# yliess86/TorchBooster

Hardware: AMD Instinct MI355X
Metric: images/sec (whole node) ResNet-50 224px bf16 DDP (higher is better)
Workload: dtype bf16; 1 GPU; model=resnet50, image=224, per_gpu_batch=256, global_batch=256, parallelism=dp1, hip_graph=False, mode=native, pg_world_size=1, optimizer=AdamW lr1e-3 wd1e-2 + clip 1.0 + CycleScheduler, loss=cross_entropy label_smoothing=0.1

## Files before the change

### csrc/bind_conv.cpp

```cpp
#include "bind_common.h"

namespace {
using namespace tbbind;

const auto kNHWC = at::MemoryFormat::ChannelsLast;

Tensor f32_work(int64_t n, const Tensor& like) {
  return n > 0 ? at::empty({n}, like.options().dtype(at::kFloat)) : Tensor();
}

Tensor conv2d_stem_pad(const Tensor& x_) {
  const at::DeviceGuard guard = on_device_of(x_, "x");
  TORCH_CHECK(x_.scalar_type() == at::kBFloat16 && x_.dim() == 4 && x_.size(1) == 3, "conv2d_stem_pad: bf16 [N,3,H,W]");
  Tensor x = nhwc(x_);
  const int N = (int)x.size(0), H = (int)x.size(2), W = (int)x.size(3);
  int P, Q, Hp, Wp;
  tbamd::stem_geometry(H, W, &P, &Q, &Hp, &Wp);
  Tensor xp = at::empty({N, Hp, Wp, 4}, x.options());
  if (N > 0) tbamd::conv_stem_pad(x.data_ptr(), xp.data_ptr(), N, H, W, cur_stream());
  return xp;
}

std::vector<Tensor> conv2d_stem_fwd(const Tensor& xp, const Tensor& wp_, int64_t H, int64_t W, bool want_stats) {
  const at::DeviceGuard guard = on_device_of(xp, "xp");
// ... 67 lines not shown
  const at::DeviceGuard guard = on_device_of(dy_, "dy");
  TORCH_CHECK(dy_.scalar_type() == at::kBFloat16 && wt_.scalar_type() == at::kBFloat16, "conv2d_dgrad_s2: bf16 only");
  const int cs = (int)stride;
  Tensor dy = nhwc(dy_);
  Tensor wt = nhwc(wt_);
  const int N = (int)dy.size(0), Kf = (int)dy.size(1), P = (int)dy.size(2), Q = (int)dy.size(3);
  const int Cf = (int)wt.size(0);
  TORCH_CHECK(wt.dim() == 4 && wt.size(1) == Kf && wt.size(2) == R && wt.size(3) == S,
              "conv2d_dgrad_s2: wt must be the flip-transposed [Cf, Kf, R, S] weight");
  TORCH_CHECK(tbamd::conv_fwd_supported(Kf, Cf) && tbamd::conv_dgrad_s2_supported((int)R, (int)S, cs),
              "conv2d_dgrad_s2: channels % 64, stride 2 or 3, <= 16 taps per phase class");
  TORCH_CHECK(pad >= 0 && P == (H + 2 * pad - R) / cs + 1 && Q == (W + 2 * pad - S) / cs + 1,
              "conv2d_dgrad_s2: geometry");
  Tensor dx = at::empty({N, Cf, H, W}, dy.options().memory_format(kNHWC));
  const int64_t NHW = (int64_t)N * H * W;
  Tensor part;
  Bnb bnb;
  if (bnb_mode != 0) {
    TORCH_CHECK(bnb_mode >= 1 && bnb_mode <= 3, "conv2d_dgrad_s2: bnb_mode");
    bnb = bnb_operands(bnb_mode, bnb_x, bnb_scale, bnb_shift, bnb_mean, bnb_bits, NHW, Cf, "conv2d_dgrad_s2");
    part = at::empty({tbamd::conv_dgrad_s2_tiles(N, (int)H, (int)W, Cf, cs), 2, Cf}, dy.options().dtype(at::kFloat));
  }
  if (NHW > 0)
    tbamd::conv_dgrad_s2(dy.data_ptr(), wt.data_ptr(), dx.data_ptr(), N, P, Q, Kf, Cf, (int)R, (int)S, (int)pad,
                         (int)H, (int)W, cur_stream(), (int)bnb_mode, bnb.x, bnb.scale, bnb.shift, bnb.mean, bnb.bits,
                         f32_or_null(part), cs);
  return {dx, part};
}

std::vector<Tensor> conv2d_fwd(const Tensor& x_, const Tensor& w_, const optional<Tensor>& bias, int64_t stride,
                               int64_t pad, bool relu, bool want_stats, const optional<Tensor>& addend,
                               const optional<Tensor>& addend_mask, int64_t bnb_mode, const optional<Tensor>& bnb_x,
                               const optional<Tensor>& bnb_scale, const optional<Tensor>& bnb_shift,
                               const optional<Tensor>& bnb_mean, const optional<Tensor>& bnb_bits, int64_t big) {
  check_cuda(x_, "x");
  struct BigScope {
    explicit BigScope(int64_t c) { if (c >= 0) tbamd::conv_big_set_call((int)c); }
    ~BigScope() { tbamd::conv_big_set_call(-1); }
  } big_scope(big);
  const at::DeviceGuard guard(x_.device());
  TORCH_CHECK(x_.scalar_type() == at::kBFloat16 && w_.scalar_type() == at::kBFloat16, "conv2d_fwd: bf16 only");
  TORCH_CHECK(x_.dim() == 4 && w_.dim() == 4 && x_.size(1) == w_.size(1), "conv2d_fwd: shape");
  Tensor x = nhwc(x_);
  Tensor w = nhwc(w_);
  ConvGeom g = ConvGeom::of(x, w);
  TORCH_CHECK(tbamd::conv_fwd_supported(g.C, g.K), "conv2d_fwd: needs C % 64 == 0 and K % 64 == 0");
  const auto [N, C, H, W, K, R, S, P, Q] = g.window(stride, pad, 1, false, 0, "conv2d_fwd");
  Tensor y = at::empty({N, K, P, Q}, x.options().memory_format(kNHWC));
  Tensor bf = f32_or_undef(bias);
  Tensor stats;
  const int64_t NPQ = g.NPQ();
  if (want_stats)
    stats = at::empty({tbamd::conv_fwd_stats_rows(NPQ, C, K, R, S, (int)stride, (int)pad), 2, K},
                      x.options().dtype(at::kFloat));
  Tensor add;
  if (given(addend)) {
    TORCH_CHECK(!want_stats && !bf.defined() && !relu, "conv2d_fwd: addend excludes bias / relu / stats");
    TORCH_CHECK(addend->sizes() == y.sizes() && addend->scalar_type() == at::kBFloat16, "conv2d_fwd: addend shape");
    add = nhwc(*addend);
  }
  const uint8_t* amask = nullptr;
  if (given(addend_mask)) {
    TORCH_CHECK(add.defined() && addend_mask->scalar_type() == at::kByte && addend_mask->numel() == NPQ * (K / 8),
                "conv2d_fwd: addend_mask must be [N*P*Q, K/8] bytes");
    amask = addend_mask->data_ptr<uint8_t>();
  }
  Tensor part;
  Bnb bnb;
  if (bnb_mode != 0) {
    TORCH_CHECK(bnb_mode >= 1 && bnb_mode <= 3 && !want_stats && !bf.defined() && !relu, "conv2d_fwd: bnb_mode");
    bnb = bnb_operands(bnb_mode, bnb_x, bnb_scale, bnb_shift, bnb_mean, bnb_bits, NPQ, K, "conv2d_fwd");
    part = at::empty({tbamd::conv_fwd_bnb_rows(NPQ, C, K, R, S, (int)stride, (int)pad), 2, K},
                     x.options().dtype(at::kFloat));
  }
  if (NPQ > 0)
    tbamd::conv_fwd(x.data_ptr(), w.data_ptr(), y.data_ptr(), f32_or_null(bf),
                    want_stats ? stats.data_ptr<float>() : nullptr, ptr_or_null(add), amask, relu, N,
                    H, W, C, K, R, S, P, Q, (int)stride, (int)pad, cur_stream(), (int)bnb_mode, bnb.x, bnb.scale,
                    bnb.shift, bnb.mean, bnb.bits, f32_or_null(part));
  return {y, bnb_mode != 0 ? part : stats};
}

std::vector<Tensor> conv2d_dgrad_gxf(const Tensor& g_, const Tensor& wt_, const optional<Tensor>& addend,
                                     const optional<Tensor>& addend_mask, int64_t bnb_mode,
                                     const optional<Tensor>& bnb_x, const optional<Tensor>& bnb_scale,
                                     const optional<Tensor>& bnb_shift, const optional<Tensor>& bnb_mean,
                                     const optional<Tensor>& bnb_bits, int64_t gxf, const Tensor& gx_x_,
                                     const optional<Tensor>& gx_bits, const optional<Tensor>& gx_scale,
                                     const optional<Tensor>& gx_shift, const Tensor& gx_coef, bool want_dz) {
  const at::DeviceGuard guard = on_device_of(g_, "g");
  TORCH_CHECK(g_.scalar_type() == at::kBFloat16 && wt_.scalar_type() == at::kBFloat16 &&
                  gx_x_.scalar_type() == at::kBFloat16, "conv2d_dgrad_gxf: bf16 only");
  TORCH_CHECK(g_.dim() == 4 && wt_.dim() == 4 && wt_.size(1) == g_.size(1) && wt_.size(2) == 1 && wt_.size(3) == 1,
              "conv2d_dgrad_gxf: 1x1 weight [K, C, 1, 1] over g [N, C, H, W]");
  TORCH_CHECK(gx_x_.sizes() == g_.sizes(), "conv2d_dgrad_gxf: gx_x must have g's shape");
  Tensor g = nhwc(g_);
  Tensor wt = nhwc(wt_);
  Tensor gx_x = nhwc(gx_x_);
  const int N = (int)g.size(0), C = (int)g.size(1), H = (int)g.size(2), W = (int)g.size(3);
  const int K = (int)wt.size(0);
  const int64_t NPQ = (int64_t)N * H * W;
  TORCH_CHECK(tbamd::conv_fwd_supported(C, K), "conv2d_dgrad_gxf: needs C % 64 == 0 and K % 64 == 0");
  TORCH_CHECK(gx_coef.scalar_type() == at::kFloat && gx_coef.is_contiguous() && gx_coef.numel() == 3 * C,
              "conv2d_dgrad_gxf: gx_coef [3, C] f32");
  const uint8_t* gbits = nullptr;
  const float *gsc = nullptr, *gsf = nullptr;
  if (gxf == 2) {
    TORCH_CHECK(gx_bits.has_value() && gx_bits->scalar_type() == at::kByte && gx_bits->numel() == NPQ * (C / 8),
                "conv2d_dgrad_gxf: gx_bits [N*H*W, C/8] bytes");
    gbits = gx_bits->data_ptr<uint8_t>();
  } else {
    TORCH_CHECK(gxf == 1 && gx_scale.has_value() && gx_shift.has_value() && gx_scale->numel() == C &&
                    gx_shift->numel() == C && gx_scale->scalar_type() == at::kFloat &&
                    gx_shift->scalar_type() == at::kFloat && gx_scale->is_contiguous() && gx_shift->is_contiguous(),
                "conv2d_dgrad_gxf: gxf 1 needs f32 [C] scale / shift");
    gsc = gx_scale->data_ptr<float>();
    gsf = gx_shift->data_ptr<float>();
  }
  Tensor y = at::empty({N, K, H, W}, g.options().memory_format(kNHWC));
  Tensor add;
  const uint8_t* amask = nullptr;
  if (given(addend)) {
    TORCH_CHECK(addend->sizes() == y.sizes() && addend->scalar_type() == at::kBFloat16, "conv2d_dgrad_gxf: addend");
    add = nhwc(*addend);
    if (given(addend_mask)) {
      TORCH_CHECK(addend_mask->scalar_type() == at::kByte && addend_mask->numel() == NPQ * (K / 8),
                  "conv2d_dgrad_gxf: addend_mask [N*H*W, K/8] bytes");
      amask = addend_mask->data_ptr<uint8_t>();
    }
  }
  const int add_code = add.defined() ? (amask ? 2 : 1) : 0;
  TORCH_CHECK(tbamd::conv_dgrad_gxf_supported((int)gxf, add_code, (int)bnb_mode),
              "conv2d_dgrad_gxf: unsupported (gxf, addend, bnb_mode) combination");
  Tensor part;
  Bnb bnb;
  if (bnb_mode != 0) {
    bnb = bnb_operands(bnb_mode, bnb_x, bnb_scale, bnb_shift, bnb_mean, bnb_bits, NPQ, K, "conv2d_dgrad_gxf");
    part = at::empty({tbamd::conv_gxf_bnb_rows(NPQ, K), 2, K}, g.options().dtype(at::kFloat));
  }
  Tensor dz;
  if (want_dz) dz = at::empty_like(g);
  if (NPQ > 0)
    tbamd::conv_dgrad_gxf(g.data_ptr(), wt.data_ptr(), y.data_ptr(), ptr_or_null(add), amask,
                          N, H, W, C, K, cur_stream(), (int)bnb_mode, bnb.x, bnb.scale, bnb.shift, bnb.mean, bnb.bits,
                          f32_or_null(part), (int)gxf, gx_x.data_ptr(), gbits, gsc,
                          gsf, gx_coef.data_ptr<float>(), ptr_or_null(dz));
  return {y, part, dz};
}

bool conv_dgrad_gxf_supported(int64_t gxf, int64_t add, int64_t bnb_mode) {
  return tbamd::conv_dgrad_gxf_supported((int)gxf, (int)add, (int)bnb_mode);
}

void check_xf_coeffs(const Tensor& scale, const Tensor& shift, int C, const char* op) {
  TORCH_CHECK(scale.scalar_type() == at::kFloat && shift.scalar_type() == at::kFloat && scale.numel() == C &&
                  shift.numel() == C && scale.is_contiguous() && shift.is_contiguous(),
              op, ": scale / shift [C] f32");
}

std::vector<Tensor> conv2d_fwd_xf(const Tensor& x_, const Tensor& w_, const Tensor& scale, const Tensor& shift,
                                  int64_t stride, int64_t pad, bool want_stats) {
  const at::DeviceGuard guard = on_device_of(x_, "x");
  TORCH_CHECK(x_.scalar_type() == at::kBFloat16 && w_.scalar_type() == at::kBFloat16, "conv2d_fwd_xf: bf16 only");
  Tensor x = nhwc(x_);
  Tensor w = nhwc(w_);
  ConvGeom g = ConvGeom::of(x, w);
  TORCH_CHECK(w.size(1) == g.C && tbamd::conv_fwd_supported(g.C, g.K), "conv2d_fwd_xf: needs C % 64 == 0 and K % 64 == 0");
  TORCH_CHECK(g.C <= tbamd::kXfMaxC, "conv2d_fwd_xf: at most ", tbamd::kXfMaxC, " input channels (coefficients in LDS)");
  check_xf_coeffs(scale, shift, g.C, "conv2d_fwd_xf");
  const auto [N, C, H, W, K, R, S, P, Q] = g.window(stride, pad, 1, false, 0, "conv2d_fwd_xf");
  const int64_t NPQ = g.NPQ();
  TORCH_CHECK(tbamd::conv_fwd_xf_supported(NPQ, C, K, R, S, (int)stride, (int)pad),
              "conv2d_fwd_xf: the persistent 1x1 shapes only (C = 64 / 128, 1x1 stride 1, K % 128, enough pixels)");
  Tensor y = at::empty({N, K, P, Q}, x.options().memory_format(kNHWC));
  Tensor stats;
  if (want_stats)
    stats = at::empty({tbamd::conv_fwd_stats_rows_tiled(NPQ, C, K, R, S, (int)stride, (int)pad), 2, K},
                      x.options().dtype(at::kFloat));
  if (NPQ > 0)
    tbamd::conv_fwd_xf(x.data_ptr(), w.data_ptr(), y.data_ptr(), want_stats ? stats.data_ptr<float>() : nullptr,
                       scale.data_ptr<float>(), shift.data_ptr<float>(), N, H, W, C, K, R, S, P, Q, (int)stride,
                       (int)pad, cur_stream());
  return {y, stats};
}

Tensor conv_flip_weight(const Tensor& w_) {
  const at::DeviceGuard guard(w_.device());
  Tensor w = nhwc(w_);
  const int K = (int)w.size(0), C = (int)w.size(1), R = (int)w.size(2), S = (int)w.size(3);
  Tensor wt = at::empty({C, K, R, S}, w.options().memory_format(kNHWC));
  tbamd::conv_flip_transpose_weight(w.data_ptr(), K, R, S, C, wt.data_ptr(), cur_stream());
  return wt;
}

Tensor dw_slot_or_new(const optional<Tensor>& out, const ConvGeom& g, const Tensor& x, const char* op) {
  if (!given(out)) return at::empty({g.K, g.C, g.R, g.S}, x.options().memory_format(kNHWC));
  TORCH_CHECK(out->dim() == 4 && out->size(0) == g.K && out->size(1) == g.C && out->size(2) == g.R &&
                  out->size(3) == g.S && out->scalar_type() == at::kBFloat16 && out->is_contiguous(kNHWC),
              op, ": out must be a channels_last bf16 [K, C, R, S] tensor");
  return *out;
}

Tensor conv2d_wgrad(const Tensor& dy_, const Tensor& x_, int64_t R_, int64_t S_, int64_t stride, int64_t pad,
                    const optional<Tensor>& out) {
  const at::DeviceGuard guard = on_device_of(x_, "x");
  TORCH_CHECK(x_.scalar_type() == at::kBFloat16 && dy_.scalar_type() == at::kBFloat16, "conv2d_wgrad: bf16 only");
  Tensor x = nhwc(x_);
  Tensor dy = nhwc(dy_);
  ConvGeom g = ConvGeom::of(x, dy, R_, S_);
  const auto [N, C, H, W, K, R, S, P, Q] = g.window(stride, pad, 1, false, 0, "conv2d_wgrad");
  TORCH_CHECK(g.fits(dy), "conv2d_wgrad: dy shape does not match x / kernel / stride / pad");
  const int64_t NPQ = g.NPQ();
  TORCH_CHECK(tbamd::conv_wgrad_supported(C, K, NPQ), "conv2d_wgrad: needs C % 64 == 0 and K % 64 == 0");
  Tensor dw = dw_slot_or_new(out, g, x, "conv2d_wgrad");
  if (NPQ == 0) return dw.zero_();
  Tensor work = f32_work(tbamd::conv_wgrad_workspace(N, H, W, C, K, R, S, P, Q, (int)stride, (int)pad), x);
  tbamd::conv_wgrad(dy.data_ptr(), x.data_ptr(), dw.data_ptr(), f32_or_null(work), N, H, W, C, K, R, S, P, Q,
                    (int)stride, (int)pad, cur_stream());
  return dw;
}

Tensor conv2d_wgrad_xf(const Tensor& dy_, const Tensor& x_, const Tensor& scale, const Tensor& shift, int64_t R_,
                       int64_t S_, int64_t stride, int64_t pad, const optional<Tensor>& out) {
  const at::DeviceGuard guard = on_device_of(x_, "x");
  TORCH_CHECK(x_.scalar_type() == at::kBFloat16 && dy_.scalar_type() == at::kBFloat16, "conv2d_wgrad_xf: bf16 only");
  Tensor x = nhwc(x_);
  Tensor dy = nhwc(dy_);
  ConvGeom g = ConvGeom::of(x, dy, R_, S_);
  TORCH_CHECK(tbamd::conv_wgrad_supported(g.C, g.K, (int64_t)g.N * dy.size(2) * dy.size(3)), "conv2d_wgrad_xf: shape");
  check_xf_coeffs(scale, shift, g.C, "conv2d_wgrad_xf");
  const auto [N, C, H, W, K, R, S, P, Q] = g.window(stride, pad, 1, false, 0, "conv2d_wgrad_xf");
  TORCH_CHECK(dy.size(2) == P && dy.size(3) == Q, "conv2d_wgrad_xf: dy shape");
  Tensor dw = dw_slot_or_new(out, g, x, "conv2d_wgrad_xf");
  Tensor work = f32_work(tbamd::conv_wgrad_workspace(N, H, W, C, K, R, S, P, Q, (int)stride, (int)pad), x);
  tbamd::conv_wgrad_xf(dy.data_ptr(), x.data_ptr(), dw.data_ptr(), f32_or_null(work), scale.data_ptr<float>(),
                       shift.data_ptr<float>(), N, H, W, C, K, R, S, P, Q, (int)stride, (int)pad, cur_stream());
  return dw;
}

Tensor conv2d_wgrad_tinyin(const Tensor& T_, const Tensor& G_) {
  check_cuda(T_, "T");
  check_cuda(G_, "G");
  const at::DeviceGuard guard(T_.device());
  TORCH_CHECK(T_.scalar_type() == at::kBFloat16 && G_.scalar_type() == at::kBFloat16, "conv2d_wgrad_tinyin: bf16");
  TORCH_CHECK(T_.dim() == 4 && G_.dim() == 4 && T_.size(0) == G_.size(0), "conv2d_wgrad_tinyin: NCHW shapes");
  Tensor T = nhwc(T_), G = nhwc(G_);
  const int N = (int)T.size(0), C = (int)T.size(1), H = (int)T.size(2), W = (int)T.size(3);
  const int K = (int)G.size(1), P = (int)G.size(2), Q = (int)G.size(3);
  TORCH_CHECK(tbamd::wgrad_tinyin_supported(C, K, 4, 4, 2, 1, P, Q, H, W),
              "conv2d_wgrad_tinyin: needs C = 3, K = 64, Q = 64, H = 2P, W = 2Q");
  Tensor part = at::empty({(int64_t)tbamd::wgrad_tinyin_parts(N, P) * K * 48}, T.options().dtype(at::kFloat));
  Tensor dw = at::empty({K, C, 4, 4}, T.options().memory_format(kNHWC));
  tbamd::wgrad_tinyin(T.data_ptr(), G.data_ptr(), dw.data_ptr(), part.data_ptr<float>(), N, P, H, W, cur_stream());
  return dw;
}

Tensor conv2d_fwd_virtual(const Tensor& x_, const Tensor& w_, const optional<Tensor>& bias, int64_t stride,
                          int64_t pad, int64_t up, bool reflect) {
  const at::DeviceGuard guard = on_device_of(x_, "x");
  TORCH_CHECK(x_.scalar_type() == at::kBFloat16 && w_.scalar_type() == at::kBFloat16, "conv2d_fwd_virtual: bf16 only");
  TORCH_CHECK(x_.dim() == 4 && w_.dim() == 4 && x_.size(1) == w_.size(1), "conv2d_fwd_virtual: shape");
  TORCH_CHECK(tbamd::conv_fwd_supported((int)x_.size(1), (int)w_.size(0)),
              "conv2d_fwd_virtual: needs C % 64 == 0 and K % 64 == 0");
  TORCH_CHECK(up == 1 || up == 2 || up == 4, "conv2d_fwd_virtual: up must be 1, 2 or 4");
  Tensor x = nhwc(x_);
  Tensor w = nhwc(w_);
  const auto [N, C, H, W, K, R, S, P, Q] = ConvGeom::of(x, w).window(
      stride, pad, up, reflect, ConvGeom::kReflectFits | ConvGeom::kNonEmpty, "conv2d_fwd_virtual");
  Tensor y = at::empty({N, K, P, Q}, x.options().memory_format(kNHWC));
  Tensor bf = f32_or_undef(bias);
  tbamd::conv_fwd_virtual(x.data_ptr(), w.data_ptr(), y.data_ptr(), f32_or_null(bf), N,
                          H, W, C, K, R, S, P, Q, (int)stride, (int)pad, (int)up, reflect ? 1 : 0, cur_stream());
  return y;
}

Tensor conv2d_wgrad_virtual(const Tensor& dy_, const Tensor& x_, int64_t R_, int64_t S_, int64_t stride, int64_t pad,
                            int64_t up, bool reflect) {
  const at::DeviceGuard guard = on_device_of(x_, "x");
  Tensor x = nhwc(x_);
  Tensor dy = nhwc(dy_);
  ConvGeom g = ConvGeom::of(x, dy, R_, S_);
  TORCH_CHECK(dy.scalar_type() == at::kBFloat16 && x.scalar_type() == at::kBFloat16, "conv2d_wgrad_virtual: bf16");
  TORCH_CHECK(g.C % 64 == 0 && g.K % 32 == 0 && (up == 1 || up == 2 || up == 4), "conv2d_wgrad_virtual: channels / up");
  const auto [N, C, H, W, K, R, S, P, Q] = g.window(stride, pad, up, reflect, 0, "conv2d_wgrad_virtual");
  TORCH_CHECK(g.fits(dy), "conv2d_wgrad_virtual: dy shape");
  Tensor dw = at::empty({K, C, R, S}, x.options().memory_format(kNHWC));
  Tensor work = f32_work(tbamd::conv_wgrad_workspace(N, H, W, C, K, R, S, P, Q, (int)stride, (int)pad), x);
  tbamd::conv_wgrad_virtual(dy.data_ptr(), x.data_ptr(), dw.data_ptr(), f32_or_null(work), N, H, W, C, K, R, S, P, Q,
                            (int)stride, (int)pad, (int)up, reflect ? 1 : 0, cur_stream());
  return dw;
}

Tensor conv2d_dgrad_virtual(const Tensor& dy_, const Tensor& wt_, int64_t H, int64_t W, int64_t stride, int64_t pad,
                            int64_t up, bool reflect) {
  const at::DeviceGuard guard = on_device_of(dy_, "dy");
  Tensor dy = nhwc(dy_);
  Tensor wt = nhwc(wt_);
  TORCH_CHECK(dy.scalar_type() == at::kBFloat16 && wt.scalar_type() == at::kBFloat16, "conv2d_dgrad_virtual: bf16");
  const int N = (int)dy.size(0), K = (int)dy.size(1), P = (int)dy.size(2), Q = (int)dy.size(3);
  const int C = (int)wt.size(0), R = (int)wt.size(2), S = (int)wt.size(3);
  TORCH_CHECK(wt.size(1) == K && tbamd::conv_fwd_supported(K, C), "conv2d_dgrad_virtual: wt [C, K, R, S], % 64");
  TORCH_CHECK(stride == 1 || (stride == 2 && tbamd::conv_dgrad_s2_supported(R, S, 2)),
              "conv2d_dgrad_virtual: stride 1, or 2 with <= 16 taps per phase class");
  const int Hp = (int)(H * up + 2 * pad), Wp = (int)(W * up + 2 * pad);
  TORCH_CHECK(P == (Hp - R) / (int)stride + 1 && Q == (Wp - S) / (int)stride + 1, "conv2d_dgrad_virtual: geometry");
  Tensor dxp = at::empty({N, C, Hp, Wp}, dy.options().memory_format(kNHWC));
  if (stride == 1) {
    TORCH_CHECK(R == S, "conv2d_dgrad_virtual: square taps");
    tbamd::conv_fwd(dy.data_ptr(), wt.data_ptr(), dxp.data_ptr(), nullptr, nullptr, nullptr, nullptr, false, N, P, Q, K,
                    C, R, S, Hp, Wp, 1, R - 1, cur_stream());
  } else {
    tbamd::conv_dgrad_s2(dy.data_ptr(), wt.data_ptr(), dxp.data_ptr(), N, P, Q, K, C, R, S, 0, Hp, Wp, cur_stream());
  }
  const tbamd::ConvAnyShape fwd{N, (int)H, (int)W, C, K, R, S, P, Q, (int)stride, (int)pad, (int)up, 1, reflect ? 1 : 0};
  Tensor dx = at::empty({N, C, H, W}, dy.options().memory_format(kNHWC));
  tbamd::conv_any_fold(0, dxp.data_ptr(), Hp, Wp, dx.data_ptr(), fwd, cur_stream());
  return dx;
}

std::vector<Tensor> split_bf16(const Tensor& t_) {
  const at::DeviceGuard guard = on_device_of(t_, "t");
  TORCH_CHECK(t_.scalar_type() == at::kFloat, "split_bf16: fp32");
  const bool cl = t_.dim() == 4 && !t_.is_contiguous() && t_.is_contiguous(kNHWC);
  Tensor t = cl ? t_ : t_.contiguous();
  TORCH_CHECK(t.numel() % 4 == 0, "split_bf16: numel % 4");
  Tensor hi = at::empty_like(t, t.options().dtype(at::kBFloat16));
  Tensor lo = at::empty_like(t, t.options().dtype(at::kBFloat16));
  tbamd::split_bf16(t.data_ptr<float>(), t.numel(), (uint16_t*)hi.data_ptr(), (uint16_t*)lo.data_ptr(), cur_stream());
  return {hi, lo};
}

Tensor bias_k(const optional<Tensor>& bias, int K, const char* op) {
  Tensor b = f32_or_undef(bias);
  TORCH_CHECK(!b.defined() || b.numel() == K, op, ": bias");
  return b;
}

Tensor conv2d_fwd_split32(const Tensor& xh, const Tensor& xl, const Tensor& wh, const Tensor& wl,
                          const optional<Tensor>& bias, int64_t stride, int64_t pad, bool relu) {
  const at::DeviceGuard guard = on_device_of(xh, "xh");
  for (const Tensor* t : {&xh, &xl, &wh, &wl})
    TORCH_CHECK(t->scalar_type() == at::kBFloat16 && t->is_contiguous(kNHWC),
                "conv2d_fwd_split32: bf16 channels_last operands");
  ConvGeom g = ConvGeom::of(xh, wh);
  TORCH_CHECK(wh.size(1) == g.C && g.C % 64 == 0 && g.K % 64 == 0 && xl.sizes() == xh.sizes() &&
                  wl.sizes() == wh.sizes(),
              "conv2d_fwd_split32: shapes");
  const auto [N, C, H, W, K, R, S, P, Q] = g.window(stride, pad, 1, false, 0, "conv2d_fwd_split32");
  Tensor y = at::empty({N, K, P, Q}, xh.options().dtype(at::kFloat).memory_format(kNHWC));
  Tensor b = bias_k(bias, K, "conv2d_fwd_split32");
  const int ns = tbamd::conv_fwd_split32_ksplit(N, C, K, R, S, P, Q);
  Tensor part;
  if (ns > 1) part = at::empty({(int64_t)ns * N * P * Q * K}, y.options().memory_format(at::MemoryFormat::Contiguous));
  tbamd::conv_fwd_split32(xh.data_ptr(), xl.data_ptr(), wh.data_ptr(), wl.data_ptr(), y.data_ptr<float>(),
                          f32_or_null(b), relu, N, H, W, C, K, R, S, P, Q, (int)stride,
                          (int)pad, cur_stream(), ns > 1 ? part.data_ptr<float>() : nullptr);
  return y;
}

Tensor conv2d_fwd_splitk(const Tensor& x_, const Tensor& w_, const optional<Tensor>& bias, int64_t stride, int64_t pad,
                         bool relu) {
  const at::DeviceGuard guard = on_device_of(x_, "x");
  Tensor x = nhwc(x_), w = nhwc(w_);
  TORCH_CHECK(x.scalar_type() == at::kBFloat16 && w.scalar_type() == at::kBFloat16, "conv2d_fwd_splitk: bf16");
  ConvGeom g = ConvGeom::of(x, w);
  TORCH_CHECK(w.size(1) == g.C && g.C % 64 == 0 && g.K % 128 == 0 && stride >= 1 && pad >= 0,
              "conv2d_fwd_splitk: shapes");
  const auto [N, C, H, W, K, R, S, P, Q] = g.window(stride, pad, 1, false, ConvGeom::kNonEmpty, "conv2d_fwd_splitk");
  Tensor y = at::empty({N, K, P, Q}, x.options().memory_format(kNHWC));
  Tensor b = bias_k(bias, K, "conv2d_fwd_splitk");
  const int ns = std::max(1, tbamd::conv_fwd_splitk_bf16_ksplit(N, C, K, R, S, P, Q));
  Tensor part = at::empty({(int64_t)ns * N * P * Q * K}, x.options().dtype(at::kFloat));
  tbamd::conv_fwd_splitk_bf16(x.data_ptr(), w.data_ptr(), y.data_ptr(), f32_or_null(b),
                              relu, N, H, W, C, K, R, S, P, Q, (int)stride, (int)pad, part.data_ptr<float>(), ns,
                              cur_stream());
  return y;
}

Tensor conv2d_wgrad_split32(const Tensor& dy_, const Tensor& x_, int64_t R_, int64_t S_, int64_t stride, int64_t pad,
                            int64_t up, bool reflect) {
  const at::DeviceGuard guard = on_device_of(x_, "x");
  Tensor x = nhwc(x_);
  Tensor dy = nhwc(dy_);
  ConvGeom g = ConvGeom::of(x, dy, R_, S_);
  TORCH_CHECK(dy.scalar_type() == at::kFloat && x.scalar_type() == at::kFloat, "conv2d_wgrad_split32: fp32");
  TORCH_CHECK(g.C % 64 == 0 && g.K % 64 == 0 && (up == 1 || up == 2 || up == 4), "conv2d_wgrad_split32: channels / up");
  const auto [N, C, H, W, K, R, S, P, Q] = g.window(stride, pad, up, reflect, 0, "conv2d_wgrad_split32");
  TORCH_CHECK(g.fits(dy), "conv2d_wgrad_split32: dy shape");
  TORCH_CHECK(g.NPQ() < (1ll << 31), "conv2d_wgrad_split32: too many output pixels");
  Tensor dw = at::empty({K, C, R, S}, x.options().memory_format(kNHWC));
  auto bf = x.options().dtype(at::kBFloat16);
  Tensor dyh = at::empty({dy.numel()}, bf), dyl = at::empty({dy.numel()}, bf);
  Tensor xh = at::empty({x.numel()}, bf), xl = at::empty({x.numel()}, bf);
  Tensor work = at::empty({tbamd::conv_wgrad_split32_workspace(N, H, W, C, K, R, S, P, Q, (int)stride, (int)pad)},
                          x.options());
  tbamd::conv_wgrad_split32(dy.data_ptr<float>(), x.data_ptr<float>(), dw.data_ptr<float>(),
                            (uint16_t*)dyh.data_ptr(), (uint16_t*)dyl.data_ptr(), (uint16_t*)xh.data_ptr(),
                            (uint16_t*)xl.data_ptr(), work.data_ptr<float>(), N, H, W, C, K, R, S, P, Q,
                            (int)stride, (int)pad, (int)up, reflect ? 1 : 0, cur_stream());
  return dw;
}

Tensor im2col(const Tensor& x, int64_t R, int64_t S, int64_t P, int64_t Q, int64_t stride, int64_t pad, int64_t up,
              bool reflect) {
  TORCH_CHECK(x.is_cuda() && x.dtype() == at::kBFloat16 && x.dim() == 4 && x.is_contiguous(kNHWC),
              "im2col: expected bf16 channels_last [N, C, H, W]");
  TORCH_CHECK(up == 1 || up == 2 || up == 4, "im2col: upsample 1, 2 or 4");
  const int64_t N = x.size(0), C = x.size(1), H = x.size(2), W = x.size(3);
  const int64_t KP = (R * S * C + 7) / 8 * 8;
  Tensor col = at::empty({N * P * Q, KP}, x.options().memory_format(at::MemoryFormat::Contiguous));
  tbamd::im2col_nhwc(x.data_ptr(), col.data_ptr(), (int)N, (int)H, (int)W, (int)C, (int)R, (int)S, (int)P, (int)Q,
                     (int)stride, (int)pad, (int)up, reflect ? 1 : 0, (int)KP, cur_stream());
  return col;
}

Tensor col2im(const Tensor& col, int64_t N, int64_t C, int64_t H, int64_t W, int64_t R, int64_t S, int64_t P,
              int64_t Q, int64_t stride, int64_t pad, const optional<Tensor>& bias) {
  TORCH_CHECK(col.is_cuda() && col.dtype() == at::kBFloat16 && col.dim() == 2 && col.is_contiguous(),
              "col2im: expected contiguous bf16 [M, KP]");
  const int64_t KP = col.size(1);
  TORCH_CHECK(col.size(0) == N * P * Q && KP >= R * S * C, "col2im: col shape");
  Tensor b;
  if (given(bias)) {
    b = bias->to(at::kBFloat16).contiguous();
    TORCH_CHECK(b.numel() == C, "col2im: bias size");
  }
  Tensor dx = at::empty({N, C, H, W}, col.options().memory_format(kNHWC));
  tbamd::col2im_nhwc(col.data_ptr(), dx.data_ptr(), ptr_or_null(b), (int)N, (int)H, (int)W,
                     (int)C, (int)R, (int)S, (int)P, (int)Q, (int)stride, (int)pad, (int)KP, cur_stream());
  return dx;
}

}

void register_conv(pybind11::module& m) {
  m.def("conv2d_stem_pad", &conv2d_stem_pad);
  m.def("conv2d_stem_fwd", &conv2d_stem_fwd);
  m.def("conv2d_stem_wgrad", &conv2d_stem_wgrad);
  m.def("conv2d_dgrad_s2", &conv2d_dgrad_s2, py::arg("dy"), py::arg("wt"), py::arg("R"), py::arg("S"), py::arg("pad"),
        py::arg("H"), py::arg("W"), py::arg("bnb_mode") = 0, py::arg("bnb_x") = py::none(),
        py::arg("bnb_scale") = py::none(), py::arg("bnb_shift") = py::none(), py::arg("bnb_mean") = py::none(),
        py::arg("bnb_bits") = py::none(), py::arg("stride") = 2);
  m.def("conv_dgrad_s2_supported", &tbamd::conv_dgrad_s2_supported);
  m.def("conv2d_fwd", &conv2d_fwd, py::arg("x"), py::arg("w"), py::arg("bias"), py::arg("stride"), py::arg("pad"),
        py::arg("relu"), py::arg("want_stats"), py::arg("addend") = py::none(), py::arg("addend_mask") = py::none(),
        py::arg("bnb_mode") = 0, py::arg("bnb_x") = py::none(), py::arg("bnb_scale") = py::none(),
        py::arg("bnb_shift") = py::none(), py::arg("bnb_mean") = py::none(), py::arg("bnb_bits") = py::none(),
        py::arg("big") = -1);
  m.def("conv2d_dgrad_gxf", &conv2d_dgrad_gxf, py::arg("g"), py::arg("wt"), py::arg("addend"),
        py::arg("addend_mask"), py::arg("bnb_mode"), py::arg("bnb_x"), py::arg("bnb_scale"), py::arg("bnb_shift"),
        py::arg("bnb_mean"), py::arg("bnb_bits"), py::arg("gxf"), py::arg("gx_x"), py::arg("gx_bits"),
        py::arg("gx_scale"), py::arg("gx_shift"), py::arg("gx_coef"), py::arg("want_dz"));
  m.def("conv_dgrad_gxf_supported", &conv_dgrad_gxf_supported);
  m.def("conv_fwd_xf_supported", &tbamd::conv_fwd_xf_supported);
  m.def("conv2d_fwd_xf", &conv2d_fwd_xf, py::arg("x"), py::arg("w"), py::arg("scale"), py::arg("shift"),
        py::arg("stride"), py::arg("pad"), py::arg("want_stats") = true);
  m.def("conv_flip_weight", &conv_flip_weight);
  m.def("conv2d_wgrad", &conv2d_wgrad, py::arg("dy"), py::arg("x"), py::arg("R"), py::arg("S"), py::arg("stride"),
        py::arg("pad"), py::arg("out") = py::none());
  m.def("conv2d_wgrad_xf", &conv2d_wgrad_xf, py::arg("dy"), py::arg("x"), py::arg("scale"), py::arg("shift"),
        py::arg("R"), py::arg("S"), py::arg("stride"), py::arg("pad"), py::arg("out") = py::none());
  m.def("conv2d_wgrad_tinyin", &conv2d_wgrad_tinyin, py::arg("T"), py::arg("G"));
  m.def("conv2d_fwd_virtual", &conv2d_fwd_virtual, py::arg("x"), py::arg("w"), py::arg("bias"), py::arg("stride"),
        py::arg("pad"), py::arg("up") = 1, py::arg("reflect") = false);
  m.def("conv2d_wgrad_virtual", &conv2d_wgrad_virtual, py::arg("dy"), py::arg("x"), py::arg("R"), py::arg("S"),
        py::arg("stride"), py::arg("pad"), py::arg("up") = 1, py::arg("reflect") = false);
  m.def("conv2d_dgrad_virtual", &conv2d_dgrad_virtual, py::arg("dy"), py::arg("wt"), py::arg("H"), py::arg("W"),
        py::arg("stride"), py::arg("pad"), py::arg("up") = 1, py::arg("reflect") = false);
  m.def("split_bf16", &split_bf16);
  m.def("conv2d_fwd_split32", &conv2d_fwd_split32, py::arg("xh"), py::arg("xl"), py::arg("wh"), py::arg("wl"),
        py::arg("bias") = py::none(), py::arg("stride") = 1, py::arg("pad") = 0, py::arg("relu") = false);
  m.def("conv2d_fwd_splitk", &conv2d_fwd_splitk, py::arg("x"), py::arg("w"), py::arg("bias") = py::none(),
        py::arg("stride") = 1, py::arg("pad") = 0, py::arg("relu") = false);
  m.def("conv_fwd_splitk_ksplit", [](int64_t N, int64_t C, int64_t K, int64_t R, int64_t S, int64_t P, int64_t Q) {
    return tbamd::conv_fwd_splitk_bf16_ksplit((int)N, (int)C, (int)K, (int)R, (int)S, (int)P, (int)Q);
  });
  m.def("conv2d_wgrad_split32", &conv2d_wgrad_split32);
  m.def("im2col", &im2col);
  m.def("col2im", &col2im, py::arg("col"), py::arg("N"), py::arg("C"), py::arg("H"), py::arg("W"), py::arg("R"),
        py::arg("S"), py::arg("P"), py::arg("Q"), py::arg("stride"), py::arg("pad"), py::arg("bias") = py::none());
  m.def("conv_set_stages", &tbamd::conv_set_stages);
  m.def("conv_set_big", &tbamd::conv_set_big);
  m.def("conv_get_big", &tbamd::conv_get_big);
  m.def("conv_big_encode", &tbamd::conv_big_encode);
  m.def("conv_big_choice", &tbamd::conv_big_choice);
  m.def("conv_set_persistent_1x1", &tbamd::conv_set_persistent_1x1);
  m.def("conv_set_occupancy", &tbamd::conv_set_occupancy);
  m.def("conv_wgrad_set_occupancy", &tbamd::conv_wgrad_set_occupancy);
}
```

### csrc/conv.hip

```cpp
#include <cstdlib>
#include <mutex>
#include <stdexcept>
#include <type_traits>

#include "common.h"
#include "tbamd.h"
#include "xf.h"

namespace tbamd {

typedef __bf16 bf16x8_t __attribute__((ext_vector_type(8)));
typedef float f32x4_t __attribute__((ext_vector_type(4)));

struct ConvGeom {
  int N, H, W, C, K, R, S, P, Q, st, pad;
  int upsh, reflect, Hv, Wv;
};

constexpr int kConvBK = 64;
constexpr int kStemKT = 4;
constexpr int kConvThreads = 256;

__device__ __forceinline__ int swz(int row, int chunk) { return chunk ^ ((row >> 1) & 7); }

__device__ __attribute__((aligned(64))) uint4 g_conv_zero_page[16];

typedef __attribute__((address_space(3))) void lds_void_t;
typedef const __attribute__((address_space(1))) void gbl_void_t;

__device__ __forceinline__ void glds16(const void* src, void* lds_wave_base) {
  __builtin_amdgcn_global_load_lds((gbl_void_t*)src, (lds_void_t*)lds_wave_base, 16, 0, 0);
}

__device__ __forceinline__ uint32_t add_bf16x2(uint32_t a, uint32_t b) {
  const float lo = bf2f((uint16_t)(a & 0xffff)) + bf2f((uint16_t)(b & 0xffff));
  const float hi = bf2f((uint16_t)(a >> 16)) + bf2f((uint16_t)(b >> 16));
  return (uint32_t)f2bf(lo) | ((uint32_t)f2bf(hi) << 16);
}

struct BnBwdEpi {
  const uint16_t* xb;
  const float* scale;
  const float* shift;
  const float* mean;
  const uint8_t* bits;
  float* part;
};

struct GxfArgs {
  const uint16_t* xb;
  const uint8_t* bits;
  const float* scale;
  const float* shift;
  const float* coef;
  uint16_t* out;
};

struct S2Cls {
  int a, b, ntap, st;
  int dr[16], ds[16], wrs[16];
  int H, W;
  int tile_base;
};

constexpr int kS2MaxCls = 9;
struct S2Set {
  int ncls;
  int wg_start[kS2MaxCls + 1];
  ConvGeom g[kS2MaxCls];
  S2Cls c[kS2MaxCls];
};

__device__ __forceinline__ int p_virt_h(int v, const ConvGeom& g) {
  return g.reflect ? (v < 0 ? -v : (v >= g.Hv ? 2 * g.Hv - 2 - v : v)) : v;
}
__device__ __forceinline__ int p_virt_w(int v, const ConvGeom& g) {
  return g.reflect ? (v < 0 ? -v : (v >= g.Wv ? 2 * g.Wv - 2 - v : v)) : v;
}

template <int BM, int BN, bool STATS, bool BIAS, bool RELU, int STAGES, int ADD, int OCC = 2, int BNB = 0,
          bool STEM = false, bool S2D = false, bool VIRT = false, int PRIO = 3, int GXF = 0>
__global__ __launch_bounds__(kConvThreads, OCC) void conv_fwd_k(const uint16_t* __restrict__ x,
                                                              const uint16_t* __restrict__ w,
                                                              uint16_t* __restrict__ y,
                                                              const float* __restrict__ bias,
                                                              float* __restrict__ stats,
                                                              const uint16_t* __restrict__ addend,
                                                              const uint8_t* __restrict__ amask, ConvGeom g_in,
                                                              BnBwdEpi bnb = BnBwdEpi{},
                                                              std::conditional_t<S2D, S2Set, S2Cls> s2arg = {},
                                                              GxfArgs gxa = GxfArgs{}) {
  static_assert(!S2D || (ADD == 0 && !STATS && !STEM), "S2D: dgrad epilogue (optionally BN partials) only");
  static_assert(!VIRT || (!S2D && !STEM), "VIRT: plain forward addressing only");
  static_assert(GXF == 0 || (STAGES == 1 && !S2D && !STEM && !VIRT && !STATS),
                "GXF: single-stage 1x1 dgrad addressing only (host: R = S = 1, stride 1, pad 0)");
  constexpr int BK = kConvBK;
  constexpr int A_PASSES = BM / 32, B_PASSES = BN / 32;
  constexpr int WM = BM / 2, WN = BN / 2;
  constexpr int TM = WM / 16, TN = WN / 16;
  constexpr int STAGE = (BM + BN) * BK / 8;
  constexpr int OUT_U4 = BN * BM / 8 + (STATS ? BM : 0);
  constexpr int LDS_U4 = STAGES * STAGE > OUT_U4 ? STAGES * STAGE : OUT_U4;
  __shared__ __attribute__((aligned(16))) uint4 lds[LDS_U4];

  const int tid = threadIdx.x, lane = tid & 63, wave = tid >> 6;
  const int wm = wave >> 1, wn = wave & 1;
  ConvGeom g = g_in;
  int bid = blockIdx.x;
  int kcls = 0;
  if constexpr (S2D) {
    while (kcls + 1 < s2arg.ncls && bid >= s2arg.wg_start[kcls + 1]) ++kcls;
    bid -= s2arg.wg_start[kcls];
    g = s2arg.g[kcls];
  }
  const S2Cls& cls = [&]() -> const S2Cls& {
    if constexpr (S2D) return s2arg.c[kcls];
    else return s2arg;
  }();
  const int64_t NPQ = (int64_t)g.N * g.P * g.Q;
  const int ntm = g.K / BM;
  const int ntn = (int)((NPQ + BN - 1) / BN);
  {
    const int nwg = ntm * ntn;
    if constexpr (S2D) {
      if (bid >= nwg) return;
    }
    const int q8 = nwg / 8, r8 = nwg % 8, xcd = bid % 8;
    bid = (xcd < r8 ? xcd * (q8 + 1) : r8 * (q8 + 1) + (xcd - r8) * q8) + bid / 8;
  }
  const int tile_m = bid % ntm;
  const int tile_n = bid / ntm;
  const int m0 = tile_m * BM;
  const int64_t n0 = (int64_t)tile_n * BN;

  const int Kred = g.R * g.S * g.C;
  const int cblocks = g.C / BK;
  const int KT = STEM ? kStemKT : (S2D ? cls.ntap * cblocks : g.R * g.S * cblocks);
  const int lrow = wave * 8 + (lane >> 3);
  const int slot = lane & 7;

  int64_t pix_base[B_PASSES];
  int pix_h[B_PASSES], pix_w[B_PASSES], pix_n[B_PASSES];
#pragma unroll
  for (int i = 0; i < B_PASSES; ++i) {
    const int64_t pix = n0 + lrow + 32 * i;
    const bool ok = pix < NPQ;
    const int64_t pp = ok ? pix : 0;
    const int q = (int)(pp % g.Q);
    const int64_t t = pp / g.Q;
    const int p = (int)(t % g.P);
    const int n = (int)(t / g.P);
    pix_n[i] = ok ? n : -1;
    pix_h[i] = ok ? p * g.st - g.pad : -(1 << 20);
    pix_w[i] = q * g.st - g.pad;
    pix_base[i] = (((int64_t)n * g.H + pix_h[i]) * g.W + pix_w[i]) * g.C;
    if constexpr (STEM) pix_base[i] = ok ? (((int64_t)n * g.H + p * g.st) * g.W + q * g.st) * g.C : 0;
  }
  const uint16_t* wsrc0 = w + (int64_t)(m0 + lrow) * Kred + (slot ^ swz(lrow, 0)) * 8;
  const int64_t wpass = (int64_t)32 * Kred;

  const int cbl = STEM ? 1 : cblocks;
  const void* zpage = pin_sgpr(g_conv_zero_page);
  uint4 gx_v[GXF ? B_PASSES : 1];
  uint32_t gx_m[GXF == 2 ? B_PASSES : 1];
  extern __shared__ __attribute__((aligned(16))) float gx_lds[];
  auto issue = [&](int kt, int buf) {
    const int rs = kt / cbl, cb = kt - rs * cbl;
    int r = rs / g.S, s = rs - r * g.S;
    int wofs = kt * BK;
    if constexpr (S2D) {
      r = cls.dr[rs];
      s = cls.ds[rs];
      wofs = (cls.wrs[rs] * cbl + cb) * BK;
    }
    uint4* A = lds + buf * STAGE;
    uint4* B = A + BM * BK / 8;
#pragma unroll
    for (int i = 0; i < A_PASSES; ++i) {
      const uint16_t* wsrc = wsrc0 + i * wpass;
      const bool wok = TB_BOUNDS_OK(wsrc + wofs + 8 <= w + (int64_t)g.K * Kred, kBndConvW);
      glds16(wok ? (const void*)(wsrc + wofs) : zpage, A + (32 * i + wave * 8) * 8);
    }
    if constexpr (STEM) {
#pragma unroll
      for (int i = 0; i < B_PASSES; ++i) {
        const int row = lrow + 32 * i;
        const int lc = slot ^ swz(row, 0);
        const int64_t off = (int64_t)(2 * kt + (lc >> 2)) * g.W * g.C + (lc & 3) * 8;
        const void* src = pix_h[i] >= 0 ? (const void*)(x + pix_base[i] + off) : zpage;
        glds16(src, B + (32 * i + wave * 8) * 8);
      }
    } else if constexpr (VIRT) {
#pragma unroll
      for (int i = 0; i < B_PASSES; ++i) {
        const int row = lrow + 32 * i;
        int vh = p_virt_h(pix_h[i] + r, g), vw = p_virt_w(pix_w[i] + s, g);
        bool ok = pix_n[i] >= 0 && (unsigned)vh < (unsigned)g.Hv && (unsigned)vw < (unsigned)g.Wv;
        const int64_t off = (((int64_t)(ok ? pix_n[i] : 0) * g.H + (vh >> g.upsh)) * g.W + (vw >> g.upsh)) * g.C +
                            cb * BK + (slot ^ swz(row, 0)) * 8;
        ok = ok && TB_BOUNDS_OK(off >= 0 && off + 8 <= (int64_t)g.N * g.H * g.W * g.C, kBndConvSrc);
        glds16(ok ? (const void*)(x + off) : zpage, B + (32 * i + wave * 8) * 8);
      }
    } else {
    const int64_t tap = ((int64_t)r * g.W + s) * g.C + cb * BK;
#pragma unroll
    for (int i = 0; i < B_PASSES; ++i) {
      const int row = lrow + 32 * i;
      const int ih = pix_h[i] + r, iw = pix_w[i] + s;
      bool ok = (unsigned)ih < (unsigned)g.H && (unsigned)iw < (unsigned)g.W;
      const int64_t off = pix_base[i] + tap + (slot ^ swz(row, 0)) * 8;
      ok = ok && TB_BOUNDS_OK(off >= 0 && off + 8 <= (int64_t)g.N * g.H * g.W * g.C, kBndConvSrc);
      const void* src = ok ? (const void*)(x + off) : zpage;
      glds16(src, B + (32 * i + wave * 8) * 8);
      if constexpr (GXF != 0) {
        gx_v[i] = ok ? *reinterpret_cast<const uint4*>(gxa.xb + off) : make_uint4(0u, 0u, 0u, 0u);
        if constexpr (GXF == 2) gx_m[i] = ok ? (uint32_t)gxa.bits[off >> 3] : 0u;
      }
    }
    }
  };
  auto gxf_stage_coef = [&]() {
    if constexpr (GXF != 0) {
      const int C4 = g.C >> 2;
      float4* d = reinterpret_cast<float4*>(gx_lds);
      const float4* cf = reinterpret_cast<const float4*>(gxa.coef);
      for (int i = tid; i < 3 * C4; i += kConvThreads) d[i] = cf[i];
      if constexpr (GXF == 1) {
        const float4* sc = reinterpret_cast<const float4*>(gxa.scale);
        const float4* sf = reinterpret_cast<const float4*>(gxa.shift);
        for (int i = tid; i < C4; i += kConvThreads) {
          d[3 * C4 + i] = sc[i];
          d[4 * C4 + i] = sf[i];
        }
      }
    }
  };
  auto gxf_apply = [&](int kt) {
    if constexpr (GXF != 0) {
      uint4* B = lds + BM * BK / 8;
      const int c0 = kt * BK + (slot ^ swz(lrow, 0)) * 8;
      float ka[8], k0[8], k1[8], sc[8], sf[8];
      auto ld8 = [&](int row, float (&v)[8]) {
        const float4 a = *reinterpret_cast<const float4*>(gx_lds + row * g.C + c0);
        const float4 b = *reinterpret_cast<const float4*>(gx_lds + row * g.C + c0 + 4);
        v[0] = a.x; v[1] = a.y; v[2] = a.z; v[3] = a.w; v[4] = b.x; v[5] = b.y; v[6] = b.z; v[7] = b.w;
      };
      ld8(0, ka);
      ld8(1, k0);
      ld8(2, k1);
      if constexpr (GXF == 1) {
        ld8(3, sc);
        ld8(4, sf);
      }
      const bool wr = gxa.out != nullptr && tile_m == 0;
#pragma unroll
      for (int i = 0; i < B_PASSES; ++i) {
        if (pix_n[i] < 0) continue;
        uint4* p = B + (32 * i + lrow) * 8 + slot;
        const uint4 gv = *p, xv = gx_v[i];
        const uint32_t gw[4] = {gv.x, gv.y, gv.z, gv.w}, xw[4] = {xv.x, xv.y, xv.z, xv.w};
        uint32_t ow[4];
#pragma unroll
        for (int e = 0; e < 4; ++e) {
          float d[2];
#pragma unroll
          for (int h = 0; h < 2; ++h) {
            const int k = 2 * e + h;
            const float xf = bf2f((uint16_t)(xw[e] >> (16 * h)));
            const float gf = bf2f((uint16_t)(gw[e] >> (16 * h)));
            bool keep;
            if constexpr (GXF == 1) keep = __builtin_fmaf(xf, sc[k], sf[k]) > 0.f;
            else keep = (gx_m[i] >> k) & 1u;
            const float dz = keep ? gf : 0.f;
            d[h] = ka[k] * dz + k0[k] + k1[k] * xf;
          }
          ow[e] = (uint32_t)f2bf(d[0]) | ((uint32_t)f2bf(d[1]) << 16);
        }
        const uint4 o = make_uint4(ow[0], ow[1], ow[2], ow[3]);
        *p = o;
        if (wr) *reinterpret_cast<uint4*>(gxa.out + pix_base[i] + c0) = o;
      }
    }
  };
  f32x4_t acc[TM][TN];
#pragma unroll
  for (int i = 0; i < TM; ++i)
#pragma unroll
    for (int j = 0; j < TN; ++j) acc[i][j] = f32x4_t{0.f, 0.f, 0.f, 0.f};

  const int fr = lane & 15, fq = lane >> 4;
  auto compute = [&](int cur) {
    const uint4* A = lds + cur * STAGE;
    const uint4* B = A + BM * BK / 8;
#pragma unroll
    for (int ks = 0; ks < BK / 32; ++ks) {
      bf16x8_t af[TM], bfr[TN];
      const int ch = ks * 4 + fq;
#pragma unroll
      for (int i = 0; i < TM; ++i) {
        const int row = wm * WM + i * 16 + fr;
        af[i] = __builtin_bit_cast(bf16x8_t, A[row * 8 + swz(row, ch)]);
      }
#pragma unroll
      for (int j = 0; j < TN; ++j) {
        const int row = wn * WN + j * 16 + fr;
        bfr[j] = __builtin_bit_cast(bf16x8_t, B[row * 8 + swz(row, ch)]);
      }
#pragma unroll
      for (int i = 0; i < TM; ++i)
#pragma unroll
        for (int j = 0; j < TN; ++j)
          acc[i][j] = __builtin_amdgcn_mfma_f32_16x16x32_bf16(af[i], bfr[j], acc[i][j], 0, 0, 0);
    }
  };

  if constexpr (STAGES >= 2) {
    constexpr int LPT = A_PASSES + B_PASSES;
#pragma unroll
    for (int t = 0; t < STAGES - 1; ++t)
      if (t < KT) issue(t, t);
    int cur = 0, nxt = STAGES - 1;
    for (int kt = 0; kt < KT; ++kt) {
      if (kt + STAGES - 2 < KT) asm volatile("s_waitcnt vmcnt(%0)" ::"n"((STAGES - 2) * LPT) : "memory");
      else asm volatile("s_waitcnt vmcnt(0)" ::: "memory");
      __builtin_amdgcn_s_barrier();
      asm volatile("" ::: "memory");
      if (kt + STAGES - 1 < KT) issue(kt + STAGES - 1, nxt);
      compute(cur);
      cur = cur + 1 == STAGES ? 0 : cur + 1;
      nxt = nxt + 1 == STAGES ? 0 : nxt + 1;
    }
    __syncthreads();
  } else {
  issue(0, 0);
  if constexpr (GXF != 0) {
    gxf_stage_coef();
    asm volatile("s_waitcnt vmcnt(0)" ::: "memory");
    __syncthreads();
    gxf_apply(0);
  } else {
    asm volatile("s_waitcnt vmcnt(0)" ::: "memory");
  }
  __syncthreads();
  for (int kt = 0; kt < KT; ++kt) {
    const int cur = 0;
    const uint4* A = lds + cur * STAGE;
    const uint4* B = A + BM * BK / 8;
    if constexpr (PRIO > 0) __builtin_amdgcn_s_setprio(PRIO);
#pragma unroll
    for (int ks = 0; ks < BK / 32; ++ks) {
      bf16x8_t af[TM], bfr[TN];
      const int ch = ks * 4 + fq;
#pragma unroll
      for (int i = 0; i < TM; ++i) {
        const int row = wm * WM + i * 16 + fr;
        af[i] = __builtin_bit_cast(bf16x8_t, A[row * 8 + swz(row, ch)]);
      }
#pragma unroll
      for (int j = 0; j < TN; ++j) {
        const int row = wn * WN + j * 16 + fr;
        bfr[j] = __builtin_bit_cast(bf16x8_t, B[row * 8 + swz(row, ch)]);
      }
#pragma unroll
      for (int i = 0; i < TM; ++i)
#pragma unroll
        for (int j = 0; j < TN; ++j)
          acc[i][j] = __builtin_amdgcn_mfma_f32_16x16x32_bf16(af[i], bfr[j], acc[i][j], 0, 0, 0);
    }
    if constexpr (PRIO > 0) __builtin_amdgcn_s_setprio(0);
    if (kt + 1 < KT) {
      __syncthreads();
      issue(kt + 1, 0);
    }
    asm volatile("s_waitcnt vmcnt(0)" ::: "memory");
    if constexpr (GXF != 0) {
      if (kt + 1 < KT) gxf_apply(kt + 1);
    }
    __syncthreads();
  }
  }

  constexpr int CPR = BM / 8;
  uint16_t* ot = reinterpret_cast<uint16_t*>(lds);
  float ssum[TM][4], ssq[TM][4];
#pragma unroll
  for (int i = 0; i < TM; ++i)
#pragma unroll
    for (int e = 0; e < 4; ++e) ssum[i][e] = ssq[i][e] = 0.f;
#pragma unroll
  for (int i = 0; i < TM; ++i) {
    const int cl = wm * WM + i * 16 + fq * 4;
    float bv[4] = {0.f, 0.f, 0.f, 0.f};
    if constexpr (BIAS) {
#pragma unroll
      for (int e = 0; e < 4; ++e) bv[e] = bias[m0 + cl + e];
    }
#pragma unroll
    for (int j = 0; j < TN; ++j) {
      const int pl = wn * WN + j * 16 + fr;
      const bool pv = n0 + pl < NPQ;
      uint16_t hv[4];
#pragma unroll
      for (int e = 0; e < 4; ++e) {
        float v = acc[i][j][e] + bv[e];
        if constexpr (RELU) v = fmaxf(v, 0.f);
        hv[e] = f2bf(v);
        if constexpr (STATS) {
          if (pv) {
            const float vr = bf2f(hv[e]);
            ssum[i][e] += vr;
            ssq[i][e] += vr * vr;
          }
        }
      }
      const int chunk = (cl >> 3) ^ (pl & (CPR - 1));
      *reinterpret_cast<uint2*>(ot + pl * BM + chunk * 8 + (cl & 7)) =
          make_uint2((uint32_t)hv[0] | ((uint32_t)hv[1] << 16), (uint32_t)hv[2] | ((uint32_t)hv[3] << 16));
    }
  }
  __syncthreads();
  float bsc[8], bsf[8], bmu[8], bdb[8], bdg[8];
  if constexpr (BNB != 0) {
    const int c0 = m0 + (tid % CPR) * 8;
#pragma unroll
    for (int e = 0; e < 8; ++e) {
      bmu[e] = bnb.mean[c0 + e];
      if constexpr (BNB == 1) {
// ... 643 lines not shown
int conv_fwd_bnb_rows(int64_t NPQ, int C, int K, int R, int S, int stride, int pad) {
  if (const int big = conv_big_choice(NPQ, C, K, R, S, stride, pad)) {
    const int bn = conv_big_pixel_tile(big);
    return (int)((NPQ + bn - 1) / bn);
  }
  return conv_fwd_pixel_tiles(NPQ, K);
}

int conv_fwd_pixel_tiles(int64_t NPQ, int K) {
  const int BN = conv_big_pix(NPQ, K) ? 128 : 64;
  return (int)((NPQ + BN - 1) / BN);
}

static int g_conv_stages = [] {
  const char* e = getenv("TBAMD_CONV_STAGES");
  return e ? atoi(e) : 0;
}();
static int g_conv_occ = 0;
void conv_set_stages(int s) { g_conv_stages = s; }
void conv_set_occupancy(int o) { g_conv_occ = o; }

template <int BM, int BN, bool STATS, bool BIAS, bool RELU, int ADD = 0, int BNB = 0>
static void launch_conv(const uint16_t* x, const uint16_t* w, uint16_t* y, const float* bias, float* stats,
                        const uint16_t* addend, const uint8_t* amask, const ConvGeom& g, hipStream_t st,
                        const BnBwdEpi& bnb = BnBwdEpi{}) {
  const int64_t NPQ = (int64_t)g.N * g.P * g.Q;
  const int ntn = (int)((NPQ + BN - 1) / BN);
  const int ntm = g.K / BM;
  const dim3 grid(ntm * ntn);
  if constexpr (ADD != 0 || BNB != 0) {
    static const int epi_stages = [] {
      const char* e = getenv("TBAMD_CONV_EPI_STAGES");
      return e ? atoi(e) : 1;
    }();
    if (epi_stages == 2)
      conv_fwd_k<BM, BN, STATS, BIAS, RELU, 2, ADD, 2, BNB>
          <<<grid, kConvThreads, 0, st>>>(x, w, y, bias, stats, addend, amask, g, bnb, S2Cls{});
    else if (epi_stages == 3)
      conv_fwd_k<BM, BN, STATS, BIAS, RELU, 3, ADD, 2, BNB>
          <<<grid, kConvThreads, 0, st>>>(x, w, y, bias, stats, addend, amask, g, bnb, S2Cls{});
    else
      conv_fwd_k<BM, BN, STATS, BIAS, RELU, 1, ADD, 4, BNB>
          <<<grid, kConvThreads, 0, st>>>(x, w, y, bias, stats, addend, amask, g, bnb, S2Cls{});
  } else {
    int stages = g_conv_stages;
    if (stages == 0) stages = 1;
    switch (stages) {
      case 1:
        if (g_conv_occ == 2)
          conv_fwd_k<BM, BN, STATS, BIAS, RELU, 1, ADD, 2><<<grid, kConvThreads, 0, st>>>(x, w, y, bias, stats, addend, amask, g, bnb, S2Cls{});
        else if (g_conv_occ == 3)
          conv_fwd_k<BM, BN, STATS, BIAS, RELU, 1, ADD, 3><<<grid, kConvThreads, 0, st>>>(x, w, y, bias, stats, addend, amask, g, bnb, S2Cls{});
        else
          conv_fwd_k<BM, BN, STATS, BIAS, RELU, 1, ADD, 4><<<grid, kConvThreads, 0, st>>>(x, w, y, bias, stats, addend, amask, g, bnb, S2Cls{});
        break;
      case 3:
        conv_fwd_k<BM, BN, STATS, BIAS, RELU, 3, ADD><<<grid, kConvThreads, 0, st>>>(x, w, y, bias, stats, addend, amask, g, bnb, S2Cls{});
        break;
      case 4:
        conv_fwd_k<BM, BN, STATS, BIAS, RELU, 4, ADD><<<grid, kConvThreads, 0, st>>>(x, w, y, bias, stats, addend, amask, g, bnb, S2Cls{});
        break;
      default:
        conv_fwd_k<BM, BN, STATS, BIAS, RELU, 2, ADD><<<grid, kConvThreads, 0, st>>>(x, w, y, bias, stats, addend, amask, g, bnb, S2Cls{});
    }
  }
}

template <int BM, int BN, int ADD>
static void dispatch_bnb(const uint16_t* x, const uint16_t* w, uint16_t* y, const uint16_t* addend,
                         const uint8_t* amask, int bnb_mode, const BnBwdEpi& bnb, const ConvGeom& g,
                         hipStream_t st) {
  switch (bnb_mode) {
    case 1: launch_conv<BM, BN, false, false, false, ADD, 1>(x, w, y, nullptr, nullptr, addend, amask, g, st, bnb); break;
    case 2: launch_conv<BM, BN, false, false, false, ADD, 2>(x, w, y, nullptr, nullptr, addend, amask, g, st, bnb); break;
    default: launch_conv<BM, BN, false, false, false, ADD, 3>(x, w, y, nullptr, nullptr, addend, amask, g, st, bnb);
  }
}

template <int BM, int BN>
static void dispatch_epi(const uint16_t* x, const uint16_t* w, uint16_t* y, const float* bias, float* stats,
                         const uint16_t* addend, const uint8_t* amask, bool relu, const ConvGeom& g,
                         hipStream_t st, int bnb_mode = 0, const BnBwdEpi& bnb = BnBwdEpi{}) {
  if (bnb_mode != 0) {
    if (addend && amask) dispatch_bnb<BM, BN, 2>(x, w, y, addend, amask, bnb_mode, bnb, g, st);
    else if (addend) dispatch_bnb<BM, BN, 1>(x, w, y, addend, nullptr, bnb_mode, bnb, g, st);
    else dispatch_bnb<BM, BN, 0>(x, w, y, nullptr, nullptr, bnb_mode, bnb, g, st);
  } else if (addend) {
    if (amask) launch_conv<BM, BN, false, false, false, 2>(x, w, y, nullptr, nullptr, addend, amask, g, st);
    else launch_conv<BM, BN, false, false, false, 1>(x, w, y, nullptr, nullptr, addend, nullptr, g, st);
  } else if (stats) {
    if (bias) launch_conv<BM, BN, true, true, false>(x, w, y, bias, stats, nullptr, nullptr, g, st, bnb);
    else launch_conv<BM, BN, true, false, false>(x, w, y, bias, stats, nullptr, nullptr, g, st, bnb);
  } else if (bias) {
    if (relu) launch_conv<BM, BN, false, true, true>(x, w, y, bias, stats, nullptr, nullptr, g, st);
    else launch_conv<BM, BN, false, true, false>(x, w, y, bias, stats, nullptr, nullptr, g, st);
  } else {
    if (relu) launch_conv<BM, BN, false, false, true>(x, w, y, bias, stats, nullptr, nullptr, g, st);
    else launch_conv<BM, BN, false, false, false>(x, w, y, bias, stats, nullptr, nullptr, g, st);
  }
}

template <int BM, int BN, int ADD, int BNB, int GXF>
static void launch_gxf(const uint16_t* x, const uint16_t* w, uint16_t* y, const uint16_t* addend,
                       const uint8_t* amask, const ConvGeom& g, hipStream_t st, const BnBwdEpi& bnb,
                       const GxfArgs& gxa) {
  const int64_t NPQ = (int64_t)g.N * g.P * g.Q;
  const dim3 grid((g.K / BM) * (int)((NPQ + BN - 1) / BN));
  const size_t coef_bytes = (size_t)(GXF == 1 ? 5 : 3) * g.C * sizeof(float);
  conv_fwd_k<BM, BN, false, false, false, 1, ADD, 4, BNB, false, false, false, 3, GXF>
      <<<grid, kConvThreads, coef_bytes, st>>>(x, w, y, nullptr, nullptr, addend, amask, g, bnb, S2Cls{}, gxa);
}

template <int BM, int BN>
static bool dispatch_gxf(const uint16_t* x, const uint16_t* w, uint16_t* y, const uint16_t* addend,
                         const uint8_t* amask, const ConvGeom& g, hipStream_t st, int bnb_mode, const BnBwdEpi& bnb,
                         int gxf, const GxfArgs& gxa) {
  const int add = addend ? (amask ? 2 : 1) : 0;
  if (gxf == 2 && add == 0 && bnb_mode == 1) launch_gxf<BM, BN, 0, 1, 2>(x, w, y, addend, amask, g, st, bnb, gxa);
  else if (gxf == 1 && add == 2 && bnb_mode == 2) launch_gxf<BM, BN, 2, 2, 1>(x, w, y, addend, amask, g, st, bnb, gxa);
  else if (gxf == 1 && add == 1 && bnb_mode == 2) launch_gxf<BM, BN, 1, 2, 1>(x, w, y, addend, amask, g, st, bnb, gxa);
  else if (gxf == 1 && add == 1 && bnb_mode == 0) launch_gxf<BM, BN, 1, 0, 1>(x, w, y, addend, amask, g, st, bnb, gxa);
  else return false;
  return true;
}

bool conv_dgrad_gxf_supported(int gxf, int add, int bnb_mode) {
  return (gxf == 2 && add == 0 && bnb_mode == 1) || (gxf == 1 && add == 2 && bnb_mode == 2) ||
         (gxf == 1 && add == 1 && (bnb_mode == 2 || bnb_mode == 0));
}

int conv_gxf_bnb_rows(int64_t NPQ, int K) {
  (void)K;
  return (int)((NPQ + 63) / 64);
}

void conv_dgrad_gxf(const void* x, const void* w, void* y, const void* addend, const uint8_t* amask, int N, int H,
                    int W, int C, int K, hipStream_t st, int bnb_mode, const void* bnb_x, const float* bnb_scale,
                    const float* bnb_shift, const float* bnb_mean, const uint8_t* bnb_bits, float* bnb_part, int gxf,
                    const void* gx_x, const uint8_t* gx_bits, const float* gx_scale, const float* gx_shift,
                    const float* gx_coef, void* gx_out) {
  const BnBwdEpi bnb{(const uint16_t*)bnb_x, bnb_scale, bnb_shift, bnb_mean, bnb_bits, bnb_part};
  const GxfArgs gxa{(const uint16_t*)gx_x, gx_bits, gx_scale, gx_shift, gx_coef, (uint16_t*)gx_out};
  const ConvGeom g{N, H, W, C, K, 1, 1, H, W, 1, 0};
  const uint16_t* xx = (const uint16_t*)x;
  const uint16_t* ww = (const uint16_t*)w;
  uint16_t* yy = (uint16_t*)y;
  const uint16_t* aa = (const uint16_t*)addend;
  bool ok;
  if (K % 128 == 0) ok = dispatch_gxf<128, 64>(xx, ww, yy, aa, amask, g, st, bnb_mode, bnb, gxf, gxa);
  else ok = dispatch_gxf<64, 64>(xx, ww, yy, aa, amask, g, st, bnb_mode, bnb, gxf, gxa);
  if (!ok) throw std::runtime_error("conv_dgrad_gxf: unsupported (gxf, addend, bnb_mode) combination");
}

void conv_fwd(const void* x, const void* w, void* y, const float* bias, float* stats, const void* addend,
              const uint8_t* amask, bool relu, int N, int H, int W, int C, int K, int R, int S, int P, int Q,
              int stride, int pad, hipStream_t st, int bnb_mode, const void* bnb_x, const float* bnb_scale,
              const float* bnb_shift, const float* bnb_mean, const uint8_t* bnb_bits, float* bnb_part) {
  const BnBwdEpi bnb{(const uint16_t*)bnb_x, bnb_scale, bnb_shift, bnb_mean, bnb_bits, bnb_part};
  ConvGeom g{N, H, W, C, K, R, S, P, Q, stride, pad};
  const int64_t NPQ = (int64_t)N * P * Q;
  {
    const int big = bnb_mode != 0 || addend ? conv_big_choice(NPQ, C, K, R, S, stride, pad)
                                            : big_for(NPQ, C, K, R, S, stride, pad);
    if (big) {
      conv_big_fwd(x, w, y, bias, stats, addend, amask, relu, N, H, W, C, K, R, S, P, Q, stride, pad, st, bnb_mode,
                   bnb_x, bnb_scale, bnb_shift, bnb_mean, bnb_bits, bnb_part, big);
      return;
    }
  }

  const bool bigpix = conv_big_pix(NPQ, K);
  const uint16_t* xx = (const uint16_t*)x;
  const uint16_t* ww = (const uint16_t*)w;
  uint16_t* yy = (uint16_t*)y;
  const uint16_t* aa = (const uint16_t*)addend;
  if (!bias && !relu && !addend && bnb_mode == 0 && conv1x1p_eligible(C, K, R, S, stride, pad, NPQ)) {
    const int ns = conv1x1p_streams(NPQ, K, C);
    const dim3 grid((K / 128) * ns);
    if (C == 64) {
      if (stats) conv1x1_fwd_k<64, 128, true><<<grid, kConvThreads, 0, st>>>(xx, ww, yy, stats, NPQ, K, ns);
      else conv1x1_fwd_k<64, 128, false><<<grid, kConvThreads, 0, st>>>(xx, ww, yy, nullptr, NPQ, K, ns);
    } else {
      if (stats) conv1x1_fwd_k<128, 64, true><<<grid, kConvThreads, 0, st>>>(xx, ww, yy, stats, NPQ, K, ns);
      else conv1x1_fwd_k<128, 64, false><<<grid, kConvThreads, 0, st>>>(xx, ww, yy, nullptr, NPQ, K, ns);
    }
    return;
  }
  if (K % 128 == 0) {
    if (bigpix) dispatch_epi<128, 128>(xx, ww, yy, bias, stats, aa, amask, relu, g, st, bnb_mode, bnb);
    else dispatch_epi<128, 64>(xx, ww, yy, bias, stats, aa, amask, relu, g, st, bnb_mode, bnb);
  } else {
    if (bigpix) dispatch_epi<64, 128>(xx, ww, yy, bias, stats, aa, amask, relu, g, st, bnb_mode, bnb);
    else dispatch_epi<64, 64>(xx, ww, yy, bias, stats, aa, amask, relu, g, st, bnb_mode, bnb);
  }
}

bool conv_fwd_xf_supported(int64_t NPQ, int C, int K, int R, int S, int stride, int pad) {
  return conv1x1p_eligible(C, K, R, S, stride, pad, NPQ);
}

template <bool STATS>
static void launch_xf(const uint16_t* x, const uint16_t* w, uint16_t* y, float* stats, const ConvGeom& g,
                      const XfArgs& xf, hipStream_t st) {
  const int64_t NPQ = (int64_t)g.N * g.P * g.Q;
  if (conv1x1p_eligible(g.C, g.K, g.R, g.S, g.st, g.pad, NPQ)) {
    const int ns = conv1x1p_streams(NPQ, g.K, g.C);
    const dim3 grid((g.K / 128) * ns);
    if (g.C == 64)
      conv1x1_fwd_k<64, 128, STATS, true><<<grid, kConvThreads, 0, st>>>(x, w, y, stats, NPQ, g.K, ns, xf);
    else
      conv1x1_fwd_k<128, 64, STATS, true><<<grid, kConvThreads, 0, st>>>(x, w, y, stats, NPQ, g.K, ns, xf);
    return;
  }
  throw std::runtime_error("conv2d_fwd_xf: the BN-in-operand forward runs on the persistent 1x1 kernel only "
                           "(C = 64 / 128, 1x1 stride 1, enough pixels: conv_fwd_xf_supported)");
}

void conv_fwd_xf(const void* x, const void* w, void* y, float* stats, const float* scale, const float* shift, int N,
                 int H, int W, int C, int K, int R, int S, int P, int Q, int stride, int pad, hipStream_t st) {
  const ConvGeom g{N, H, W, C, K, R, S, P, Q, stride, pad};
  const XfArgs xf{scale, shift};
  if (stats) launch_xf<true>((const uint16_t*)x, (const uint16_t*)w, (uint16_t*)y, stats, g, xf, st);
  else launch_xf<false>((const uint16_t*)x, (const uint16_t*)w, (uint16_t*)y, nullptr, g, xf, st);
}

template <int BM, int BN>
static void launch_virt(const uint16_t* x, const uint16_t* w, uint16_t* y, const float* bias, const ConvGeom& g,
                        hipStream_t st) {
  const int64_t NPQ = (int64_t)g.N * g.P * g.Q;
  const dim3 grid((g.K / BM) * (int)((NPQ + BN - 1) / BN));
  if (bias)
    conv_fwd_k<BM, BN, false, true, false, 1, 0, 4, 0, false, false, true>
        <<<grid, kConvThreads, 0, st>>>(x, w, y, bias, nullptr, nullptr, nullptr, g);
  else
    conv_fwd_k<BM, BN, false, false, false, 1, 0, 4, 0, false, false, true>
        <<<grid, kConvThreads, 0, st>>>(x, w, y, nullptr, nullptr, nullptr, nullptr, g);
}

void conv_fwd_virtual(const void* x, const void* w, void* y, const float* bias, int N, int H, int W, int C, int K,
                      int R, int S, int P, int Q, int stride, int pad, int up, int reflect, hipStream_t st) {
  ConvGeom g{N, H, W, C, K, R, S, P, Q, stride, pad, up == 4 ? 2 : (up == 2 ? 1 : 0), reflect ? 1 : 0, H * up, W * up};
  const int64_t NPQ = (int64_t)N * P * Q;
  const bool bigpix = conv_big_pix(NPQ, K);
  const uint16_t* xx = (const uint16_t*)x;
  const uint16_t* ww = (const uint16_t*)w;
  uint16_t* yy = (uint16_t*)y;
  if (K % 128 == 0) {
    if (bigpix) launch_virt<128, 128>(xx, ww, yy, bias, g, st);
    else launch_virt<128, 64>(xx, ww, yy, bias, g, st);
  } else {
    if (bigpix) launch_virt<64, 128>(xx, ww, yy, bias, g, st);
    else launch_virt<64, 64>(xx, ww, yy, bias, g, st);
  }
}

__global__ __launch_bounds__(256) void stem_pad_k(const uint16_t* __restrict__ x, uint16_t* __restrict__ xp, int N,
                                                  int H, int W, int Hp, int Wp, int pad) {
  const int64_t total = (int64_t)N * Hp * Wp;
  for (int64_t i = (int64_t)blockIdx.x * 256 + threadIdx.x; i < total; i += (int64_t)gridDim.x * 256) {
    const int w = (int)(i % Wp);
    const int64_t t = i / Wp;
    const int h = (int)(t % Hp);
    const int n = (int)(t / Hp);
    const int ih = h - pad, iw = w - pad;
    uint32_t lo = 0, hi = 0;
    if ((unsigned)ih < (unsigned)H && (unsigned)iw < (unsigned)W) {
      const uint16_t* s = x + (((int64_t)n * H + ih) * W + iw) * 3;
      lo = (uint32_t)s[0] | ((uint32_t)s[1] << 16);
      hi = (uint32_t)s[2];
    }
    *reinterpret_cast<uint2*>(xp + i * 4) = make_uint2(lo, hi);
  }
}

static void stem_dims(int H, int W, int& P, int& Q, int& Hp, int& Wp) {
  P = (H - 1) / 2 + 1;
  Q = (W - 1) / 2 + 1;
  Hp = 2 * P + 6;
  Wp = 2 * Q + 6;
}

int64_t conv_stem_workspace(int N, int H, int W) {
  int P, Q, Hp, Wp;
  stem_dims(H, W, P, Q, Hp, Wp);
  return (int64_t)N * Hp * Wp * 4;
}

template <int BM, int BN, bool STATS>
static void launch_stem(const uint16_t* xp, const uint16_t* wp, uint16_t* y, float* stats, const ConvGeom& g,
                        hipStream_t st) {
  const int64_t NPQ = (int64_t)g.N * g.P * g.Q;
  const dim3 grid((g.K / BM) * (int)((NPQ + BN - 1) / BN));
  conv_fwd_k<BM, BN, STATS, false, false, 1, 0, 4, 0, true>
      <<<grid, kConvThreads, 0, st>>>(xp, wp, y, nullptr, stats, nullptr, nullptr, g);
}

void conv_stem_pad(const void* x, void* xp, int N, int H, int W, hipStream_t st) {
  int P, Q, Hp, Wp;
  stem_dims(H, W, P, Q, Hp, Wp);
  const int64_t tot = (int64_t)N * Hp * Wp;
  int64_t gs = (tot + 255) / 256;
  if (gs > 8192) gs = 8192;
  stem_pad_k<<<(int)gs, 256, 0, st>>>((const uint16_t*)x, (uint16_t*)xp, N, H, W, Hp, Wp, 3);
}

void stem_geometry(int H, int W, int* P, int* Q, int* Hp, int* Wp) { stem_dims(H, W, *P, *Q, *Hp, *Wp); }
// ... 174 lines not shown
```

### csrc/conv_wgrad.hip

```cpp
#include <algorithm>
#include <cstdlib>
#include <type_traits>

#include "common.h"
#include "tbamd.h"
#include "xf.h"

namespace tbamd {

namespace {

typedef __bf16 bf16x8_t __attribute__((ext_vector_type(8)));
typedef short s16x4_t __attribute__((ext_vector_type(4)));
typedef float f32x4_t __attribute__((ext_vector_type(4)));
typedef __attribute__((address_space(3))) void lds_void_t;
typedef const __attribute__((address_space(1))) void gbl_void_t;
typedef __attribute__((address_space(3))) s16x4_t lds_s16x4_t;

__device__ __attribute__((aligned(64))) uint4 g_wgrad_zero_page[16];

__device__ __forceinline__ void glds16(const void* src, void* lds_wave_base) {
  __builtin_amdgcn_global_load_lds((gbl_void_t*)src, (lds_void_t*)lds_wave_base, 16, 0, 0);
}

struct FastDiv {
  uint32_t mul;
  uint32_t shift;
  uint32_t d;
};

static FastDiv make_fastdiv(uint32_t d) {
  uint32_t l = 0;
  while ((1ull << l) < d) ++l;
  const uint64_t m = ((1ull << 32) * ((1ull << l) - d)) / d + 1;
  return FastDiv{(uint32_t)m, l, d};
}

__device__ __forceinline__ uint32_t fdiv(uint32_t n, const FastDiv& f) {
  return (__umulhi(n, f.mul) + n) >> f.shift;
}

struct WgradGeom {
  int N, H, W, C, K, R, S, P, Q, st, pad;
  int ncol;
  int npq;
  int pix_split;
  int splits;
  FastDiv fq, fp;
  int upsh, reflect, Hv, Wv;
};

template <int ROWB>
__device__ __forceinline__ int wz(int row) {
  if constexpr (ROWB == 256) return ((row & 3) | (((row >> 3) & 1) << 2)) << 1;
  else if constexpr (ROWB == 128) return ((((row >> 1) & 1) | (((row >> 3) & 1) << 1))) << 1;
  else return ((row >> 3) & 1) << 1;
}

template <int ROWB>
__device__ __forceinline__ bf16x8_t tr_frag(const char* base, int ks, int cb, int lane) {
  const int g = lane >> 4, q = (lane >> 2) & 3, p = lane & 3;
  const int lc = (cb >> 3) + (p >> 1);
  const int r0 = ks * 32 + 8 * g + q, r1 = r0 + 4;
  const int o0 = r0 * ROWB + ((lc ^ wz<ROWB>(r0)) << 4) + ((p & 1) << 3);
  const int o1 = r1 * ROWB + ((lc ^ wz<ROWB>(r1)) << 4) + ((p & 1) << 3);
  const s16x4_t v0 = __builtin_amdgcn_ds_read_tr16_b64_v4i16((lds_s16x4_t*)(base + o0));
  const s16x4_t v1 = __builtin_amdgcn_ds_read_tr16_b64_v4i16((lds_s16x4_t*)(base + o1));
  typedef short s16x8_t __attribute__((ext_vector_type(8)));
  const s16x8_t v = __builtin_shufflevector(v0, v1, 0, 1, 2, 3, 4, 5, 6, 7);
  return __builtin_bit_cast(bf16x8_t, v);
}

constexpr int kWgThreads = 256;
constexpr int kWgBK = 64;

template <int BM, int BN, bool FINAL, int OCC = 2, bool STEM = false, bool VIRT = false, bool XF = false>
__global__ __launch_bounds__(kWgThreads, OCC) void conv_wgrad_k(const uint16_t* __restrict__ dy,
                                                              const uint16_t* __restrict__ x,
                                                              float* __restrict__ part,
                                                              uint16_t* __restrict__ dw, WgradGeom g,
                                                              XfArgs xf = XfArgs{}) {
  static_assert(!XF || (!STEM && !VIRT), "XF: plain weight gradient");
  constexpr int BK = kWgBK;
  constexpr int ROWA = BM * 2, ROWB = BN * 2;
  constexpr int CPA = BM / 8, CPB = BN / 8;
  constexpr int A_PASSES = BK * CPA / kWgThreads, B_PASSES = BK * CPB / kWgThreads;
  constexpr int WM = BM / 2, WN = BN / 2, TM = WM / 16, TN = WN / 16;
  constexpr int STAGE = BK * (ROWA + ROWB);
  __shared__ __attribute__((aligned(16))) char lds[STAGE];

  const int tid = threadIdx.x, lane = tid & 63, wave = tid >> 6;
  const int wm = wave >> 1, wn = wave & 1;
  const int ntm = g.K / BM, ntn = g.ncol / BN, ntiles = ntm * ntn;
  const int nwg = ntiles * g.splits;
  int bid = blockIdx.x;
  {
    const int q8 = nwg / 8, r8 = nwg % 8, xcd = bid % 8;
    bid = (xcd < r8 ? xcd * (q8 + 1) : r8 * (q8 + 1) + (xcd - r8) * q8) + bid / 8;
  }
  const int split = bid / ntiles, tile = bid - split * ntiles;
  const int tile_m = tile % ntm, tile_n = tile / ntm;
  const int m0 = tile_m * BM, n0 = tile_n * BN;
  const int pb = split * g.pix_split;
  const int pe = min(pb + g.pix_split, g.npq);
  const int KT = (pe - pb + BK - 1) / BK;

  const uint16_t* asrc[A_PASSES];
  int arow[A_PASSES];
#pragma unroll
  for (int i = 0; i < A_PASSES; ++i) {
    const int row = i * (kWgThreads / CPA) + wave * (64 / CPA) + lane / CPA;
    const int lc = (lane % CPA) ^ wz<ROWA>(row);
    arow[i] = row;
    asrc[i] = dy + m0 + lc * 8;
  }
  int brow[B_PASSES], bdr[B_PASSES], bds[B_PASSES], bc[B_PASSES];
#pragma unroll
  for (int i = 0; i < B_PASSES; ++i) {
    const int row = i * (kWgThreads / CPB) + wave * (64 / CPB) + lane / CPB;
    const int lc = (lane % CPB) ^ wz<ROWB>(row);
    const int col = n0 + lc * 8;
    const int c = col % g.C, rs = col / g.C;
    brow[i] = row;
    bdr[i] = rs / g.S - g.pad;
    bds[i] = rs % g.S - g.pad;
    bc[i] = c;
    if constexpr (STEM) {
      bdr[i] = col >> 5;
      bds[i] = (col & 31) >> 2;
      bc[i] = 0;
    }
  }

  const void* zpage = pin_sgpr(g_wgrad_zero_page);
  uint32_t bvalid = 0u;
  float xsc[XF ? 8 : 1], xsh[XF ? 8 : 1];
  if constexpr (XF) {
    float sc8[8], sh8[8];
    xf_load(xf, bc[0], sc8, sh8);
#pragma unroll
    for (int e = 0; e < 8; ++e) {
      xsc[e] = sc8[e];
      xsh[e] = sh8[e];
    }
  }
  auto issue = [&](int kt, int buf) {
    char* A = lds + buf * STAGE;
    char* B = A + BK * ROWA;
    const int p0 = pb + kt * BK;
#pragma unroll
    for (int i = 0; i < A_PASSES; ++i) {
      const int pix = p0 + arow[i];
      const void* src = pix < pe ? (const void*)(asrc[i] + (int64_t)pix * g.K) : zpage;
      glds16(src, A + (i * kWgThreads + wave * 64) * 16);
    }
#pragma unroll
    for (int i = 0; i < B_PASSES; ++i) {
      const int pix = p0 + brow[i];
      const void* src = zpage;
      if (pix < pe) {
        const uint32_t t = fdiv((uint32_t)pix, g.fq);
        const int q = pix - (int)t * g.Q;
        const uint32_t n = fdiv(t, g.fp);
        const int p = (int)t - (int)n * g.P;
        const int h = p * g.st + bdr[i], w = q * g.st + bds[i];
        if constexpr (STEM) {
          src = x + (((int64_t)n * g.H + h) * g.W + w) * 4;
        } else if constexpr (VIRT) {
          const int vh = g.reflect ? (h < 0 ? -h : (h >= g.Hv ? 2 * g.Hv - 2 - h : h)) : h;
          const int vw = g.reflect ? (w < 0 ? -w : (w >= g.Wv ? 2 * g.Wv - 2 - w : w)) : w;
          if ((unsigned)vh < (unsigned)g.Hv && (unsigned)vw < (unsigned)g.Wv)
            src = x + (((int64_t)n * g.H + (vh >> g.upsh)) * g.W + (vw >> g.upsh)) * g.C + bc[i];
        } else if ((unsigned)h < (unsigned)g.H && (unsigned)w < (unsigned)g.W) {
          src = x + (((int64_t)n * g.H + h) * g.W + w) * g.C + bc[i];
        }
      }
      glds16(src, B + (i * kWgThreads + wave * 64) * 16);
      if constexpr (XF) {
        if (i == 0) bvalid = 0u;
        bvalid |= (uint32_t)(src != zpage) << i;
      }
    }
  };
  auto xform = [&](int buf) {
    if constexpr (XF) {
      char* B = lds + buf * STAGE + BK * ROWA;
      float sc8[8], sh8[8];
#pragma unroll
      for (int e = 0; e < 8; ++e) {
        sc8[e] = xsc[e];
        sh8[e] = xsh[e];
      }
#pragma unroll
      for (int i = 0; i < B_PASSES; ++i) {
        if (!((bvalid >> i) & 1u)) continue;
        uint4* p = reinterpret_cast<uint4*>(B + (i * kWgThreads + wave * 64) * 16) + lane;
        *p = xf_chunk(*p, sc8, sh8);
      }
    }
  };

  f32x4_t acc[TM][TN];
#pragma unroll
  for (int i = 0; i < TM; ++i)
#pragma unroll
    for (int j = 0; j < TN; ++j) acc[i][j] = f32x4_t{0.f, 0.f, 0.f, 0.f};

  for (int kt = 0; kt < KT; ++kt) {
    issue(kt, 0);
    asm volatile("s_waitcnt vmcnt(0)" ::: "memory");
    xform(0);
    __syncthreads();
#pragma unroll
    for (int ks = 0; ks < BK / 32; ++ks) {
      bf16x8_t af[TM], bfr[TN];
#pragma unroll
      for (int i = 0; i < TM; ++i) af[i] = tr_frag<ROWA>(lds, ks, wm * WM + i * 16, lane);
#pragma unroll
      for (int j = 0; j < TN; ++j) bfr[j] = tr_frag<ROWB>(lds + BK * ROWA, ks, wn * WN + j * 16, lane);
#pragma unroll
      for (int i = 0; i < TM; ++i)
#pragma unroll
        for (int j = 0; j < TN; ++j)
          acc[i][j] = __builtin_amdgcn_mfma_f32_16x16x32_bf16(af[i], bfr[j], acc[i][j], 0, 0, 0);
    }
    __syncthreads();
  }

  const int fr = lane & 15, fq = lane >> 4;
#pragma unroll
  for (int i = 0; i < TM; ++i)
#pragma unroll
    for (int e = 0; e < 4; ++e) {
      const int m = m0 + wm * WM + i * 16 + fq * 4 + e;
#pragma unroll
      for (int j = 0; j < TN; ++j) {
        const int n = n0 + wn * WN + j * 16 + fr;
        if constexpr (FINAL) dw[(int64_t)m * g.ncol + n] = f2bf(acc[i][j][e]);
        else part[((int64_t)split * g.K + m) * g.ncol + n] = acc[i][j][e];
      }
    }
}

constexpr int kRedCols = 16, kRedLanes = 16;
template <typename OutT>
__global__ __launch_bounds__(256) void wgrad_reduce_k(const float* __restrict__ part, int splits, int64_t total,
                                                      OutT* __restrict__ dw) {
  __shared__ float4 red[kRedLanes][kRedCols];
  const int tx = threadIdx.x % kRedCols, ty = threadIdx.x / kRedCols;
  const int64_t i4 = ((int64_t)blockIdx.x * kRedCols + tx) * 4;
  float4 s = make_float4(0.f, 0.f, 0.f, 0.f);
  if (i4 < total) {
    int k = ty;
#pragma unroll 1
    for (; k + 3 * kRedLanes < splits; k += 4 * kRedLanes) {
      float4 v[4];
#pragma unroll
      for (int u = 0; u < 4; ++u) v[u] = *reinterpret_cast<const float4*>(part + (int64_t)(k + u * kRedLanes) * total + i4);
#pragma unroll
      for (int u = 0; u < 4; ++u) {
        s.x += v[u].x;
        s.y += v[u].y;
        s.z += v[u].z;
        s.w += v[u].w;
      }
    }
    for (; k < splits; k += kRedLanes) {
      const float4 v = *reinterpret_cast<const float4*>(part + (int64_t)k * total + i4);
      s.x += v.x;
      s.y += v.y;
      s.z += v.z;
      s.w += v.w;
    }
  }
  red[ty][tx] = s;
  __syncthreads();
  if (ty == 0 && i4 < total) {
    for (int j = 1; j < kRedLanes; ++j) {
      const float4 v = red[j][tx];
      s.x += v.x;
      s.y += v.y;
      s.z += v.z;
      s.w += v.w;
    }
    if constexpr (sizeof(OutT) == 4) {
      *reinterpret_cast<float4*>(dw + i4) = s;
    } else {
      const uint32_t lo = (uint32_t)f2bf(s.x) | ((uint32_t)f2bf(s.y) << 16);
      const uint32_t hi = (uint32_t)f2bf(s.z) | ((uint32_t)f2bf(s.w) << 16);
      *reinterpret_cast<uint2*>(dw + i4) = make_uint2(lo, hi);
    }
  }
}

__global__ __launch_bounds__(256) void split_bf16_k(const float* __restrict__ v, int64_t n4, uint16_t* __restrict__ hi,
                                                    uint16_t* __restrict__ lo) {
  for (int64_t i = (int64_t)blockIdx.x * 256 + threadIdx.x; i < n4; i += (int64_t)gridDim.x * 256) {
    const float4 a = reinterpret_cast<const float4*>(v)[i];
    const float f[4] = {a.x, a.y, a.z, a.w};
    uint16_t h[4], l[4];
#pragma unroll
    for (int e = 0; e < 4; ++e) {
      h[e] = f2bf(f[e]);
      l[e] = f2bf(f[e] - bf2f(h[e]));
    }
    reinterpret_cast<uint2*>(hi)[i] = make_uint2((uint32_t)h[0] | ((uint32_t)h[1] << 16), (uint32_t)h[2] | ((uint32_t)h[3] << 16));
    reinterpret_cast<uint2*>(lo)[i] = make_uint2((uint32_t)l[0] | ((uint32_t)l[1] << 16), (uint32_t)l[2] | ((uint32_t)l[3] << 16));
  }
}

int g_wgrad_occ = 0;

template <int BM, int BN, int OCC>
void launch_wgrad_s(const uint16_t* dy, const uint16_t* x, float* part, uint16_t* dw, const WgradGeom& g,
                    hipStream_t st) {
  const int nwg = (g.K / BM) * (g.ncol / BN) * g.splits;
  if (g.splits == 1)
    conv_wgrad_k<BM, BN, true, OCC><<<nwg, kWgThreads, 0, st>>>(dy, x, part, dw, g);
  else
    conv_wgrad_k<BM, BN, false, OCC><<<nwg, kWgThreads, 0, st>>>(dy, x, part, dw, g);
}

template <int BM, int BN>
void launch_wgrad(const uint16_t* dy, const uint16_t* x, float* part, uint16_t* dw, const WgradGeom& g,
                  hipStream_t st) {
  switch (g_wgrad_occ) {
    case 3: launch_wgrad_s<BM, BN, 3>(dy, x, part, dw, g, st); break;
    case 4: launch_wgrad_s<BM, BN, 4>(dy, x, part, dw, g, st); break;
    default: launch_wgrad_s<BM, BN, 2>(dy, x, part, dw, g, st);
  }
}

WgradGeom plan_wgrad(int N, int H, int W, int C, int K, int R, int S, int P, int Q, int stride, int pad) {
  WgradGeom g{};
  g.N = N, g.H = H, g.W = W, g.C = C, g.K = K, g.R = R, g.S = S, g.P = P, g.Q = Q, g.st = stride, g.pad = pad;
  g.ncol = R * S * C;
  g.npq = N * P * Q;
  const int BM = K % 128 == 0 ? 128 : (K % 64 == 0 ? 64 : 32);
  const int BN = g.ncol % 128 == 0 ? 128 : 64;
  const int64_t tiles = (int64_t)(K / BM) * (g.ncol / BN);
  const int bk = kWgBK;
  const int64_t kiters = (g.npq + bk - 1) / bk;
  static const double waves = [] {
    const char* e = getenv("TBAMD_WGRAD_WAVES");
    const double v = e ? atof(e) : 1.0;
    return v > 0.0 && v <= 8.0 ? v : 1.0;
  }();
  const int64_t target = (int64_t)(((BM == 128 && BN == 128) ? 768 : 1024) * waves);
  int64_t splits = (target + tiles - 1) / tiles;
  splits = std::min<int64_t>(splits, std::max<int64_t>(g.npq / 1024, 1));
  static const int64_t cap_mb = [] {
    const char* e = getenv("TBAMD_WGRAD_CAP_MB");
    const int64_t v = e ? atoll(e) : 32;
    return v >= 1 && v <= 1024 ? v : 32;
  }();
  const int64_t cap = (cap_mb << 20) / ((int64_t)K * g.ncol * 4);
  splits = std::max<int64_t>(1, std::min(splits, std::max<int64_t>(cap, 1)));
  const int64_t per = ((kiters + splits - 1) / splits) * bk;
  g.pix_split = (int)per;
  g.splits = (int)((g.npq + per - 1) / per);
  g.fq = make_fastdiv((uint32_t)Q);
  g.fp = make_fastdiv((uint32_t)P);
  return g;
}

}

int64_t conv_stem_wgrad_workspace(int N, int Hp, int Wp, int K, int P, int Q) {
  const WgradGeom g = plan_wgrad(N, Hp, Wp, 4, K, 8, 8, P, Q, 2, 0);
  return g.splits > 1 ? (int64_t)g.splits * K * g.ncol : 0;
}

void conv_stem_wgrad(const void* dy, const void* xp, void* dwp, float* workspace, int N, int Hp, int Wp, int K,
                     int P, int Q, hipStream_t st) {
  const WgradGeom g = plan_wgrad(N, Hp, Wp, 4, K, 8, 8, P, Q, 2, 0);
  const uint16_t* d = (const uint16_t*)dy;
  const uint16_t* xx = (const uint16_t*)xp;
  uint16_t* o = (uint16_t*)dwp;
  const int nwg = (K / (K % 128 == 0 ? 128 : 64)) * (g.ncol / 128) * g.splits;
  if (K % 128 == 0) {
    if (g.splits == 1) conv_wgrad_k<128, 128, true, 3, true><<<nwg, kWgThreads, 0, st>>>(d, xx, workspace, o, g);
    else conv_wgrad_k<128, 128, false, 3, true><<<nwg, kWgThreads, 0, st>>>(d, xx, workspace, o, g);
  } else {
    if (g.splits == 1) conv_wgrad_k<64, 128, true, 3, true><<<nwg, kWgThreads, 0, st>>>(d, xx, workspace, o, g);
    else conv_wgrad_k<64, 128, false, 3, true><<<nwg, kWgThreads, 0, st>>>(d, xx, workspace, o, g);
  }
  if (g.splits > 1) {
    const int64_t total = (int64_t)K * g.ncol;
    wgrad_reduce_k<uint16_t><<<cdiv(total, 4 * kRedCols), kRedCols * kRedLanes, 0, st>>>(workspace, g.splits, total, o);
  }
}

void conv_wgrad_virtual(const void* dy, const void* x, void* dw, float* workspace, int N, int H, int W, int C, int K,
                        int R, int S, int P, int Q, int stride, int pad, int up, int reflect, hipStream_t st) {
  WgradGeom g = plan_wgrad(N, H, W, C, K, R, S, P, Q, stride, pad);
  g.upsh = up == 4 ? 2 : (up == 2 ? 1 : 0);
  g.reflect = reflect ? 1 : 0;
  g.Hv = H * up;
  g.Wv = W * up;
  const uint16_t* d = (const uint16_t*)dy;
  const uint16_t* xx = (const uint16_t*)x;
  uint16_t* o = (uint16_t*)dw;
  auto go = [&](auto bm, auto bn) {
    constexpr int BM = decltype(bm)::value, BN = decltype(bn)::value;
    const int nwg = (g.K / BM) * (g.ncol / BN) * g.splits;
    if (g.splits == 1)
      conv_wgrad_k<BM, BN, true, 3, false, true><<<nwg, kWgThreads, 0, st>>>(d, xx, workspace, o, g);
    else
      conv_wgrad_k<BM, BN, false, 3, false, true><<<nwg, kWgThreads, 0, st>>>(d, xx, workspace, o, g);
  };
  using std::integral_constant;
  const bool bm128 = K % 128 == 0, bn128 = g.ncol % 128 == 0;
  if (K % 64 != 0) go(integral_constant<int, 32>{}, integral_constant<int, 64>{});
  else if (bm128 && bn128) go(integral_constant<int, 128>{}, integral_constant<int, 128>{});
  else if (bm128) go(integral_constant<int, 128>{}, integral_constant<int, 64>{});
  else if (bn128) go(integral_constant<int, 64>{}, integral_constant<int, 128>{});
  else go(integral_constant<int, 64>{}, integral_constant<int, 64>{});
  if (g.splits > 1) {
    const int64_t total = (int64_t)K * g.ncol;
    wgrad_reduce_k<uint16_t><<<cdiv(total, 4 * kRedCols), kRedCols * kRedLanes, 0, st>>>(workspace, g.splits, total, o);
  }
}

void conv_wgrad_xf(const void* dy, const void* x, void* dw, float* workspace, const float* scale, const float* shift,
                   int N, int H, int W, int C, int K, int R, int S, int P, int Q, int stride, int pad,
                   hipStream_t st) {
  const WgradGeom g = plan_wgrad(N, H, W, C, K, R, S, P, Q, stride, pad);
  const XfArgs xf{scale, shift};
  const uint16_t* d = (const uint16_t*)dy;
  const uint16_t* xx = (const uint16_t*)x;
  uint16_t* o = (uint16_t*)dw;
  auto go = [&](auto bm, auto bn) {
    constexpr int BM = decltype(bm)::value, BN = decltype(bn)::value;
    const int nwg = (g.K / BM) * (g.ncol / BN) * g.splits;
    if (g_wgrad_occ == 3) {
      if (g.splits == 1)
        conv_wgrad_k<BM, BN, true, 3, false, false, true><<<nwg, kWgThreads, 0, st>>>(d, xx, workspace, o, g, xf);
      else
        conv_wgrad_k<BM, BN, false, 3, false, false, true><<<nwg, kWgThreads, 0, st>>>(d, xx, workspace, o, g, xf);
    } else if (g.splits == 1) {
      conv_wgrad_k<BM, BN, true, 2, false, false, true><<<nwg, kWgThreads, 0, st>>>(d, xx, workspace, o, g, xf);
    } else {
      conv_wgrad_k<BM, BN, false, 2, false, false, true><<<nwg, kWgThreads, 0, st>>>(d, xx, workspace, o, g, xf);
    }
  };
  using std::integral_constant;
  const bool bm128 = K % 128 == 0, bn128 = g.ncol % 128 == 0;
  if (bm128 && bn128) go(integral_constant<int, 128>{}, integral_constant<int, 128>{});
  else if (bm128) go(integral_constant<int, 128>{}, integral_constant<int, 64>{});
  else if (bn128) go(integral_constant<int, 64>{}, integral_constant<int, 128>{});
  else go(integral_constant<int, 64>{}, integral_constant<int, 64>{});
  if (g.splits > 1) {
    const int64_t total = (int64_t)K * g.ncol;
    wgrad_reduce_k<uint16_t><<<cdiv(total, 4 * kRedCols), kRedCols * kRedLanes, 0, st>>>(workspace, g.splits, total, o);
  }
}

void conv_wgrad_set_occupancy(int o) { g_wgrad_occ = o; }

int64_t conv_wgrad_split32_workspace(int N, int H, int W, int C, int K, int R, int S, int P, int Q, int stride,
                                     int pad) {
  const WgradGeom g = plan_wgrad(N, H, W, C, K, R, S, P, Q, stride, pad);
  return 3ll * g.splits * K * g.ncol;
}

void conv_wgrad_split32(const float* dy, const float* x, float* dw, uint16_t* dyh, uint16_t* dyl, uint16_t* xh,
                        uint16_t* xl, float* part, int N, int H, int W, int C, int K, int R, int S, int P, int Q,
                        int stride, int pad, int up, int reflect, hipStream_t st) {
  const int64_t ndy = (int64_t)N * P * Q * K, nx = (int64_t)N * H * W * C;
  auto grid4 = [](int64_t n4) { return (int)std::min<int64_t>((n4 + 255) / 256, 8192); };
  split_bf16_k<<<grid4(ndy / 4), 256, 0, st>>>(dy, ndy / 4, dyh, dyl);
  split_bf16_k<<<grid4(nx / 4), 256, 0, st>>>(x, nx / 4, xh, xl);
  WgradGeom g = plan_wgrad(N, H, W, C, K, R, S, P, Q, stride, pad);
  const bool virt = up != 1 || reflect;
  g.upsh = up == 4 ? 2 : (up == 2 ? 1 : 0);
  g.reflect = reflect ? 1 : 0;
  g.Hv = H * up;
  g.Wv = W * up;
  const int64_t slab = (int64_t)g.splits * K * g.ncol;
  const uint16_t* A[3] = {dyh, dyh, dyl};
  const uint16_t* B[3] = {xh, xl, xh};
  auto go = [&](auto bm, auto bn) {
    constexpr int BM = decltype(bm)::value, BN = decltype(bn)::value;
    const int nwg = (g.K / BM) * (g.ncol / BN) * g.splits;
    for (int t = 0; t < 3; ++t) {
      if (virt)
        conv_wgrad_k<BM, BN, false, 3, false, true><<<nwg, kWgThreads, 0, st>>>(A[t], B[t], part + t * slab, nullptr, g);
      else
        conv_wgrad_k<BM, BN, false, 3><<<nwg, kWgThreads, 0, st>>>(A[t], B[t], part + t * slab, nullptr, g);
    }
  };
  using std::integral_constant;
  const bool bm128 = K % 128 == 0, bn128 = g.ncol % 128 == 0;
  if (bm128 && bn128) go(integral_constant<int, 128>{}, integral_constant<int, 128>{});
  else if (bm128) go(integral_constant<int, 128>{}, integral_constant<int, 64>{});
  else if (bn128) go(integral_constant<int, 64>{}, integral_constant<int, 128>{});
  else go(integral_constant<int, 64>{}, integral_constant<int, 64>{});
  const int64_t total = (int64_t)K * g.ncol;
  wgrad_reduce_k<float><<<cdiv(total, 4 * kRedCols), kRedCols * kRedLanes, 0, st>>>(part, 3 * g.splits, total, dw);
}

void split_bf16(const float* v, int64_t n, uint16_t* hi, uint16_t* lo, hipStream_t st) {
  const int64_t n4 = n / 4;
  if (n4 == 0) return;
  split_bf16_k<<<(int)std::min<int64_t>((n4 + 255) / 256, 8192), 256, 0, st>>>(v, n4, hi, lo);
}

int conv_wgrad_supported(int C, int K, int64_t NPQ) {
  return C % 64 == 0 && K % 64 == 0 && NPQ < (1ll << 31);
}

int64_t conv_wgrad_workspace(int N, int H, int W, int C, int K, int R, int S, int P, int Q, int stride, int pad) {
  const WgradGeom g = plan_wgrad(N, H, W, C, K, R, S, P, Q, stride, pad);
  return g.splits > 1 ? (int64_t)g.splits * K * g.ncol : 0;
}

void conv_wgrad(const void* dy, const void* x, void* dw, float* workspace, int N, int H, int W, int C, int K, int R,
                int S, int P, int Q, int stride, int pad, hipStream_t st) {
  const WgradGeom g = plan_wgrad(N, H, W, C, K, R, S, P, Q, stride, pad);
  const uint16_t* d = (const uint16_t*)dy;
  const uint16_t* xx = (const uint16_t*)x;
  uint16_t* o = (uint16_t*)dw;
  const bool bm128 = K % 128 == 0, bn128 = g.ncol % 128 == 0;
  if (bm128 && bn128) launch_wgrad<128, 128>(d, xx, workspace, o, g, st);
  else if (bm128) launch_wgrad<128, 64>(d, xx, workspace, o, g, st);
  else if (bn128) launch_wgrad<64, 128>(d, xx, workspace, o, g, st);
  else launch_wgrad<64, 64>(d, xx, workspace, o, g, st);
  if (g.splits > 1) {
    const int64_t total = (int64_t)K * g.ncol;
    wgrad_reduce_k<uint16_t><<<cdiv(total, 4 * kRedCols), kRedCols * kRedLanes, 0, st>>>(workspace, g.splits, total, o);
  }
}

}
```

### csrc/tbamd.h

```cpp
#pragma once
#include <hip/hip_runtime.h>
#include <stdint.h>

#include <string>
#include <vector>


namespace tbamd {

enum DTypeCode : int { kF32 = 0, kBF16 = 1, kF16 = 2 };

int64_t conv_wgrad_split32_workspace(int N, int H, int W, int C, int K, int R, int S, int P, int Q, int stride,
                                     int pad);
void conv_wgrad_split32(const float* dy, const float* x, float* dw, uint16_t* dyh, uint16_t* dyl, uint16_t* xh,
                        uint16_t* xl, float* part, int N, int H, int W, int C, int K, int R, int S, int P, int Q,
                        int stride, int pad, int up, int reflect, hipStream_t st);

void split_bf16(const float* v, int64_t n, uint16_t* hi, uint16_t* lo, hipStream_t st);
void conv_fwd_split32(const void* xh, const void* xl, const void* wh, const void* wl, float* y, const float* bias,
                      bool relu, int N, int H, int W, int C, int K, int R, int S, int P, int Q, int stride, int pad,
                      hipStream_t st, float* part = nullptr);
int conv_fwd_splitk_bf16_ksplit(int N, int C, int K, int R, int S, int P, int Q);
void conv_fwd_splitk_bf16(const void* x, const void* w, void* y, const float* bias, bool relu, int N, int H, int W,
                          int C, int K, int R, int S, int P, int Q, int stride, int pad, float* part, int ns,
                          hipStream_t st);
int conv_fwd_split32_ksplit(int N, int C, int K, int R, int S, int P, int Q);

void act_forward(int dt, int act, const void* x, void* y, int64_t n, float slope, hipStream_t st);
void act_backward(int dt, int act, const void* x, const void* dy, void* dx, int64_t n, float slope, hipStream_t st);

int64_t stop_event_arm();
bool stop_event_disarm();
void stream_wait_stop_event(hipStream_t st, int64_t id);

int bn_partial_blocks(int64_t M, int C);
int bn_stats_rows(int dt, int nblk);
void bn_forward_train(int dt, const void* x, int64_t M, int C, const float* gamma, const float* beta,
                      float* running_mean, float* running_var, int64_t* nbt, float momentum, float eps,
                      float* psum, float* psq, int nblk, double* fin_ws, float* mean, float* invstd, float* scale,
                      float* shift, hipStream_t st);
int64_t colsum_workspace(int nrows, int C);
bool bn_backward_pool_ok(int H, int W, int C, int k, int s, int pad);
int bn_backward_pool_blocks(int N, int H, int W, int C);
void bn_backward_pool(int dt, const void* dyp, const uint8_t* idx, const void* x, int N, int H, int W, int C, int k,
                      int s, int pad, int act, float slope, const float* gamma, const float* mean,
                      const float* invstd, const float* scale, const float* shift, int training, float* pdb,
                      float* pdg, int nblk, double* fin_ws, float* coef, float* dgamma, float* dbeta, void* dx,
                      hipStream_t st);
void bn_backward_from_partials(int dt, const void* dy, const void* y, const void* x, int64_t M, int C, int act,
                               float slope, const float* gamma, const float* mean, const float* invstd,
                               const float* scale, const float* shift, int training, const float* part, int nrows,
                               double* fin_ws, float* coef, float* dgamma, float* dbeta, void* dx,
                               const uint8_t* maskin, hipStream_t st,
                               void* dres = nullptr,
                               const void* xds = nullptr, const float* mean_ds = nullptr, float* pds = nullptr);
void bn_backward_coef(const float* part, int nrows, int64_t M, int C, const float* gamma, const float* mean,
                      const float* invstd, int training, double* fin_ws, float* coef, float* dgamma, float* dbeta,
                      hipStream_t st);
void bn_backward_apply_coef(int dt, const void* dy, const void* x, int64_t M, int C, int act, float slope,
                            const float* scale, const float* shift, const float* coef, void* dx,
                            const uint8_t* maskin, hipStream_t st);
int bn_bwd_dsp_rows(int64_t M, int C);
void bn_eval_coeffs(int C, const float* gamma, const float* beta, const float* rm, const float* rv,
                    float eps, float* mean, float* invstd, float* scale, float* shift, hipStream_t st);
void bn_apply(int dt, const void* x, const void* res, const float* scale, const float* shift, int64_t M,
              int C, int act, float slope, void* y, uint8_t* mask, hipStream_t st, const float* rsc = nullptr,
              const float* rsh = nullptr);
void bn_backward(int dt, const void* dy, const void* y, const void* x, const void* res, int64_t M, int C,
                 int act, float slope, const float* gamma, const float* mean, const float* invstd,
                 const float* scale, const float* shift, int training, float* pdb, float* pdg, int nblk,
                 double* fin_ws, float* coef, float* dgamma, float* dbeta, void* dres, void* dx,
                 const uint8_t* maskin, hipStream_t st);

int norm_partial_blocks(int64_t M, int C, int S);
void norm_apply(int dt, const void* x, const void* res, const float* scale, const float* shift, int S,
                int64_t M, int C, int act, float slope, void* y, hipStream_t st);
void gn_forward_stats(int dt, const void* x, int N, int64_t HW, int C, int G, const float* gamma,
                      const float* beta, float eps, float* psum, float* psq, float* row0, int nblk, float* mean,
                      float* invstd, float* scale, float* shift, hipStream_t st);
void gn_backward(int dt, const void* dy, const void* y, const void* x, const void* res, int N, int64_t HW, int C,
                 int G, int act, float slope, const float* gamma, const float* mean, const float* invstd,
                 const float* scale, const float* shift, float* pdb, float* pdg, int nblk, float* coef,
                 float* dg_nc, float* db_nc, float* dgamma, float* dbeta, void* dres, void* dx, hipStream_t st);

int ln_bwd_blocks(int64_t M);
void ln_forward(int dt, const void* x, const void* res, const float* gamma, const float* beta, int64_t M, int C,
                float eps, void* y, void* xsum, float* mean, float* rstd, hipStream_t st);
void ln_backward(int dt, const void* dy, const void* x, const void* dadd, const float* gamma, const float* mean,
                 const float* rstd, int64_t M, int C, void* dx, float* pdg, float* pdb, int nblk, float* dgamma,
                 float* dbeta, hipStream_t st);
void rms_forward(int dt, const void* x, const void* res, const float* gamma, int64_t M, int C, float eps, void* y,
                 void* xsum, float* rstd, hipStream_t st);
void rms_backward(int dt, const void* dy, const void* x, const void* dadd, const float* gamma, const float* rstd,
                  int64_t M, int C, void* dx, float* pdg, int nblk, float* dgamma, hipStream_t st);

void swiglu_forward(int dt, const void* gu, int64_t sgu, int64_t M, int F, void* y, hipStream_t st);
void swiglu_backward(int dt, const void* gu, int64_t sgu, const void* dy, int64_t M, int F, void* dgu,
                     hipStream_t st);

void adamw_mt(int pdt, int gdt, bool master, bool ema, bool amsgrad, const void* chunks, int nchunks,
              const int64_t* table, float lr, float beta1, float beta2, float eps, float wd, float bc1,
              float bc2_sqrt, float ema_decay, const float* clip_coef, const float* inv_scale,
              const float* found_inf, hipStream_t st, const float* hyper = nullptr);
void sgd_mt(int pdt, int gdt, bool master, float momentum, float dampening, bool nesterov, float wd,
            float lr, int first_step, const void* chunks, int nchunks, const int64_t* table,
            const float* clip_coef, const float* inv_scale, const float* found_inf, hipStream_t st,
            const float* hyper = nullptr);
void grad_norm_mt(int gdt, const void* chunks, int nchunks, const int64_t* table, float max_norm,
                  const float* inv_scale, float* partial, float* out3, hipStream_t st);
void grad_norm_multi(int ngroups, const int* gdts, const void* const* chunks, const int* nchunks,
                     const int64_t* const* tables, float max_norm, const float* inv_scale, float* partial,
                     float* out3, hipStream_t st);
void scale_mt(int gdt, const void* chunks, int nchunks, const int64_t* table, const float* s,
              hipStream_t st);

void ce_forward(int dt, const void* logits, const int64_t* labels, int64_t N, int K, float smoothing,
                int64_t ignore_index, float* row_loss, float* row_lse, float* row_ok, float* out3,
                hipStream_t st);
void ce_backward(int dt, const void* logits, const int64_t* labels, const float* row_lse, const float* gout,
                 const float* stats3, int64_t N, int K, float smoothing, int64_t ignore_index,
                 void* dlogits, hipStream_t st);

int conv_fwd_supported(int C, int K);
void conv_set_stages(int s);
void conv_set_occupancy(int o);
int conv_fwd_pixel_tiles(int64_t NPQ, int K);
int conv_fwd_bnb_rows(int64_t NPQ, int C, int K, int R, int S, int stride, int pad);
bool conv_dgrad_gxf_supported(int gxf, int add, int bnb_mode);
int conv_gxf_bnb_rows(int64_t NPQ, int K);
void conv_dgrad_gxf(const void* x, const void* w, void* y, const void* addend, const uint8_t* amask, int N, int H,
                    int W, int C, int K, hipStream_t st, int bnb_mode, const void* bnb_x, const float* bnb_scale,
                    const float* bnb_shift, const float* bnb_mean, const uint8_t* bnb_bits, float* bnb_part, int gxf,
                    const void* gx_x, const uint8_t* gx_bits, const float* gx_scale, const float* gx_shift,
                    const float* gx_coef, void* gx_out);
int conv_big_choice(int64_t NPQ, int C, int K, int R, int S, int stride, int pad);
int conv_big_encode(int bm, int bn, int mf, int stages);
int conv_big_pixel_tile(int code);
void conv_set_big(int mode);
int conv_get_big();
void conv_big_set_call(int code);
int conv_big_mode_now();
void conv_big_fwd(const void* x, const void* w, void* y, const float* bias, float* stats, const void* addend,
                  const uint8_t* amask, bool relu, int N, int H, int W, int C, int K, int R, int S, int P, int Q,
                  int stride, int pad, hipStream_t st, int bnb_mode, const void* bnb_x, const float* bnb_scale,
                  const float* bnb_shift, const float* bnb_mean, const uint8_t* bnb_bits, float* bnb_part,
                  int code);
void conv_set_persistent_1x1(bool on);
int conv_fwd_stats_rows(int64_t NPQ, int C, int K, int R, int S, int stride, int pad);
int conv_fwd_stats_rows_tiled(int64_t NPQ, int C, int K, int R, int S, int stride, int pad);
int64_t conv_stem_workspace(int N, int H, int W);
void stem_geometry(int H, int W, int* P, int* Q, int* Hp, int* Wp);
void conv_stem_pad(const void* x, void* xp, int N, int H, int W, hipStream_t st);
void conv_stem_fwd(const void* xp, const void* wp, void* y, float* stats, int N, int H, int W, int K,
                   hipStream_t st);
int64_t conv_stem_wgrad_workspace(int N, int Hp, int Wp, int K, int P, int Q);
void conv_stem_wgrad(const void* dy, const void* xp, void* dwp, float* workspace, int N, int Hp, int Wp, int K,
                     int P, int Q, hipStream_t st);
void conv_dgrad_s2(const void* dy, const void* wt, void* dx, int N, int P, int Q, int Kf, int Cf, int R, int S,
                   int pad, int H, int W, hipStream_t st, int bnb_mode = 0, const void* bnb_x = nullptr,
                   const float* bnb_scale = nullptr, const float* bnb_shift = nullptr,
                   const float* bnb_mean = nullptr, const uint8_t* bnb_bits = nullptr, float* bnb_part = nullptr,
                   int cs = 2);
int conv_dgrad_s2_tiles(int N, int H, int W, int Cf, int st = 2);
bool conv_dgrad_s2_supported(int R, int S, int st);
constexpr int kXfMaxC = 512;
bool wgrad_tinyin_supported(int C, int K, int R, int S, int stride, int pad, int P, int Q, int H, int W);
int wgrad_tinyin_parts(int N, int P);
void wgrad_tinyin(const void* T, const void* G, void* dw, float* part, int N, int P, int H, int W, hipStream_t st);
void conv_wgrad_xf(const void* dy, const void* x, void* dw, float* workspace, const float* scale, const float* shift,
                   int N, int H, int W, int C, int K, int R, int S, int P, int Q, int stride, int pad,
                   hipStream_t st);
bool conv_fwd_xf_supported(int64_t NPQ, int C, int K, int R, int S, int stride, int pad);
void conv_fwd_xf(const void* x, const void* w, void* y, float* stats, const float* scale, const float* shift, int N,
                 int H, int W, int C, int K, int R, int S, int P, int Q, int stride, int pad, hipStream_t st);
void conv_fwd(const void* x, const void* w, void* y, const float* bias, float* stats, const void* addend,
              const uint8_t* addend_mask, bool relu, int N, int H, int W, int C, int K, int R, int S, int P, int Q,
              int stride, int pad, hipStream_t st, int bnb_mode = 0, const void* bnb_x = nullptr,
              const float* bnb_scale = nullptr, const float* bnb_shift = nullptr, const float* bnb_mean = nullptr,
              const uint8_t* bnb_bits = nullptr, float* bnb_part = nullptr);
void bn_finalize_from_conv(const float* part, int nblk, int64_t M, int C, const float* gamma, const float* beta,
                           float* running_mean, float* running_var, int64_t* nbt, float momentum, float eps,
                           double* fin_ws, float* mean, float* invstd, float* scale, float* shift, hipStream_t st);
void conv_flip_transpose_weights_mt(const void* chunks, int nchunks, const int64_t* table, hipStream_t st);
void conv_flip_transpose_weight(const void* w, int K, int R, int S, int C, void* wt, hipStream_t st);
int conv_wgrad_supported(int C, int K, int64_t NPQ);
void conv_wgrad_set_occupancy(int o);
int64_t conv_wgrad_workspace(int N, int H, int W, int C, int K, int R, int S, int P, int Q, int stride, int pad);
void conv_fwd_virtual(const void* x, const void* w, void* y, const float* bias, int N, int H, int W, int C, int K,
                      int R, int S, int P, int Q, int stride, int pad, int up, int reflect, hipStream_t st);
void conv_wgrad_virtual(const void* dy, const void* x, void* dw, float* workspace, int N, int H, int W, int C, int K,
                        int R, int S, int P, int Q, int stride, int pad, int up, int reflect, hipStream_t st);
void conv_wgrad(const void* dy, const void* x, void* dw, float* workspace, int N, int H, int W, int C, int K, int R,
                int S, int P, int Q, int stride, int pad, hipStream_t st);

struct AttnArgs {
  const uint16_t* q;
  const uint16_t* k;
  const uint16_t* v;
  uint16_t* o;
  float* lse;
  int B, H, N;
  float scale;
  int64_t sq[3], sk[3], sv[3], so[3];
  const uint16_t* dout;
  int64_t sdo[3];
  uint16_t* dq;
  uint16_t* dk;
  uint16_t* dv;
  int64_t sdq[3], sdk[3], sdv[3];
  float* delta;
  int causal;
  const int* klen;
  int window;
};
// ... 248 lines not shown
```

### torchbooster_amd/models/resnet.py

```python
from __future__ import annotations

import os
from typing import Tuple, Callable, List, Optional, Sequence, Type, Union

import torch
from torch import Tensor, nn

from torchbooster_amd.ops.conv import (conv2d_bn_stats, conv2d_xf_bn_stats, conv_stem, native_supported,
                                       stem_supported)
from torchbooster_amd.ops import _ext
from torchbooster_amd.ops._ext import native, use_native
from torchbooster_amd.ops.norm import BatchNormAct2d, BnBwdLink, BnGradXf, LazyAct, ResidualGradLink, gxf_enabled
from torchbooster_amd.ops.linear import Linear

__all__ = [
    "ConvBNAct",
    "conv_bn_act",
    "global_avgpool_flatten",
    "BasicBlock",
    "Bottleneck",
    "ResNet",
    "resnet18",
    "resnet34",
    "resnet50",
    "resnet101",
    "resnet152",
]


class ConvBNAct(nn.Module):

    def __init__(
        self,
        in_ch: int,
        out_ch: int,
        kernel_size: int,
        stride: int = 1,
        padding: Optional[int] = None,
        act: str = "relu",
        groups: int = 1,
    ) -> None:
        super().__init__()
        if padding is None:
            padding = kernel_size // 2
        self.conv = nn.Conv2d(in_ch, out_ch, kernel_size, stride, padding, groups=groups, bias=False)
        self.bn = BatchNormAct2d(out_ch, act=act)

    def native_ok(self, x: Tensor) -> bool:
        c = self.conv
        return (x.is_cuda and use_native(x) and
                native_supported(x, c.weight, c.stride, c.padding, c.dilation, c.groups))

    def forward(self, x: Tensor, residual: Optional[Tensor] = None, passthrough: bool = False,
                pool: Optional[Tuple[int, int, int]] = None, link: Optional[ResidualGradLink] = None,
                bn_in: Optional[BnBwdLink] = None, bn_out: Optional[BnBwdLink] = None,
                lazy_in: Optional[LazyAct] = None, lazy_out: Optional[LazyAct] = None, gx: Optional[BnGradXf] = None):
        return conv_bn_act(self.conv, self.bn, x, None, residual, passthrough, pool, link, bn_in, bn_out, lazy_in,
                           lazy_out, gx)


def conv_bn_act(conv: nn.Conv2d, bn: BatchNormAct2d, x: Tensor, act: Optional[str] = None,
                residual: Optional[Tensor] = None, passthrough: bool = False,
                pool: Optional[Tuple[int, int, int]] = None, link: Optional[ResidualGradLink] = None,
                bn_in: Optional[BnBwdLink] = None, bn_out: Optional[BnBwdLink] = None,
                lazy_in: Optional[LazyAct] = None, lazy_out: Optional[LazyAct] = None, gx: Optional[BnGradXf] = None):
    c = conv
    if lazy_in is not None and lazy_in.ready(x):
        assert not passthrough and pool is None
        y, stats = conv2d_xf_bn_stats(x, lazy_in.y, lazy_in.scale, lazy_in.shift, c.weight, c.stride[0],
                                      c.padding[0], bn_in, gx)
        outs = (y, stats, x)
    elif x.is_cuda and c.bias is None and native_supported(x, c.weight, c.stride, c.padding, c.dilation, c.groups):
        outs = conv2d_bn_stats(x, c.weight, c.stride[0], c.padding[0], passthrough,
                               link if passthrough else None, bn_in, gx)
        y, stats = outs[0], outs[1]
    elif x.is_cuda and c.bias is None and stem_supported(x, c.weight, c.stride, c.padding, c.dilation, c.groups):
        y, stats = conv_stem(x, c.weight)
        outs = (y, stats, x)
    else:
        y, stats = c(x), None
        outs = (y, None, x)
    if pool is not None:
        assert residual is None and not passthrough
        return bn.forward_maxpool(y, *pool, stats=stats, act=act)
    bn_link = link if residual is not None or (link is not None and link.carrier and not passthrough) else None
    y = bn(y, residual, stats, bn_link, bn_out, act=act, lazy=lazy_out, gx=gx if stats is not None else None)
    return (y, outs[2]) if passthrough else y


_LAZY_BN = os.environ.get("TBAMD_BN_XF", "1") != "0"
_RES_CARRIER = os.environ.get("TBAMD_RES_CARRIER", "1") != "0"
_LAZY_DS = os.environ.get("TBAMD_LAZY_DS", "1") != "0"


def _no_hooks(mods) -> bool:
    from torch.nn.modules import module as _mod

    if _mod._global_forward_hooks or _mod._global_forward_pre_hooks:
        return False
    return not any(m._forward_hooks or m._forward_pre_hooks for m in mods)


def _lazy_ds_ok(training: bool, down: Sequence[nn.Module], watch: Sequence[nn.Module]) -> bool:
    return _LAZY_DS and training and torch.is_grad_enabled() and _no_hooks(tuple(down) + tuple(watch))


def _lazy_ok(training: bool, convs: Sequence[nn.Conv2d], bns: Sequence[nn.Module],
             acts: Sequence[str], watch: Sequence[nn.Module]) -> bool:
    if not (_LAZY_BN and training and torch.is_grad_enabled()):
        return False
    if not _no_hooks((bns[0], convs[1], bns[1], convs[2]) + tuple(watch)):
        return False
    for i in (0, 1):
        if acts[i] != "relu" or convs[i].weight.dtype != torch.bfloat16 or convs[i].out_channels % 64:
            return False
    c2, c3 = convs[1], convs[2]
    return (c2.in_channels % 64 == 0 and c2.in_channels <= 512 and c3.in_channels <= 512 and c3.out_channels % 64 == 0
            and c2.groups == 1 and c3.groups == 1)


def _gxf_ok(training: bool, convs: Sequence[Optional[nn.Conv2d]], bns: Sequence[Optional[nn.Module]],
            watch: Sequence[nn.Module]) -> bool:
    if not (gxf_enabled() and training and torch.is_grad_enabled()):
        return False
    return _no_hooks(tuple(m for m in tuple(convs[:3]) + tuple(bns[:3]) if m is not None) + tuple(watch))


def _gxf_pair_ok(conv: nn.Conv2d, act: str) -> bool:
    return (act == "relu" and conv.bias is None and conv.kernel_size == (1, 1) and conv.stride == (1, 1)
            and conv.padding == (0, 0) and conv.groups == 1 and conv.weight.dtype == torch.bfloat16
            and conv.in_channels % 64 == 0 and conv.out_channels % 64 == 0)


def bottleneck_linked(x: Tensor, convs: Sequence[Optional[nn.Conv2d]], bns: Sequence[Optional[nn.Module]],
                      run: Callable, training: bool, bn_in: Optional[BnBwdLink] = None,
                      watch: Sequence[nn.Module] = (), acts: Sequence[str] = ("relu", "relu", "relu", "none")):
    c1 = convs[0]
    has_down = convs[3] is not None
    native = (x.is_cuda and use_native(x) and c1.bias is None and
              native_supported(x, c1.weight, c1.stride, c1.padding, c1.dilation, c1.groups))
    link = None
    if (native and _RES_CARRIER and has_down and convs[2].out_channels % 8 == 0
            and torch.is_grad_enabled() and bns[2].training and bns[3].training):
        link = ResidualGradLink(carrier=True)
    elif native and not has_down:
        link = ResidualGradLink()
    l1, l2, l3 = (BnBwdLink(), BnBwdLink(), BnBwdLink()) if native else (None, None, None)
    z2 = None
    if native and _lazy_ok(training, convs, bns, acts, watch):
        st = convs[1].stride[0]
        npq = x.shape[0] * (-(-x.shape[2] // st)) * (-(-x.shape[3] // st))
        c3 = convs[2]
        if _ext.native().conv_fwd_xf_supported(npq, c3.in_channels, c3.out_channels, 1, 1, 1, 0):
            z2 = LazyAct()
    g1 = g3 = None
    if native and _gxf_ok(training, convs, bns, watch):
        g1 = BnGradXf() if _gxf_pair_ok(convs[0], acts[0]) else None
        g3 = BnGradXf() if not has_down and link is not None and _gxf_pair_ok(convs[2], "relu") else None
    h, xp = run(0, x, passthrough=True, link=link if not has_down else None,
                bn_in=bn_in if native else None, bn_out=l1, gx=g1)
    if has_down:
        lz = LazyAct() if native and _lazy_ds_ok(training, (convs[3], bns[3]), watch) else None
        identity = run(3, xp, link=link, lazy_out=lz)
    else:
        identity = xp
    h = run(1, h, bn_in=l1, bn_out=l2, lazy_out=z2)
    return run(2, h, residual=identity, link=link, bn_in=l2, bn_out=l3, lazy_in=z2, gx=g3), l3


class BasicBlock(nn.Module):
    expansion = 1

    def __init__(self, in_ch: int, ch: int, stride: int = 1) -> None:
        super().__init__()
        out_ch = ch * self.expansion
        self.c1 = ConvBNAct(in_ch, ch, 3, stride)
        self.c2 = ConvBNAct(ch, out_ch, 3, 1, act="relu")
        self.down = None
        if stride != 1 or in_ch != out_ch:
            self.down = ConvBNAct(in_ch, out_ch, 1, stride, 0, act="none")

    def forward(self, x: Tensor) -> Tensor:
        h, xp = self.c1(x, passthrough=True)
        identity = xp if self.down is None else self.down(xp)
        return self.c2(h, identity)


class Bottleneck(nn.Module):
    expansion = 4

    def __init__(self, in_ch: int, ch: int, stride: int = 1) -> None:
        super().__init__()
        out_ch = ch * self.expansion
        self.c1 = ConvBNAct(in_ch, ch, 1, 1, 0)
        self.c2 = ConvBNAct(ch, ch, 3, stride)
        self.c3 = ConvBNAct(ch, out_ch, 1, 1, 0, act="relu")
        self.down = None
        if stride != 1 or in_ch != out_ch:
            self.down = ConvBNAct(in_ch, out_ch, 1, stride, 0, act="none")

    def forward(self, x: Tensor) -> Tensor:
        return self.forward_linked(x)[0]

    def forward_linked(self, x: Tensor, bn_in: Optional[BnBwdLink] = None):
        mods = (self.c1, self.c2, self.c3, self.down)

        def run(i, t, residual=None, **kw):
            return mods[i](t, residual, **kw)

        d = self.down
        return bottleneck_linked(
            x, tuple(m.conv if m is not None else None for m in mods),
            tuple(m.bn if m is not None else None for m in mods), run, self.training, bn_in,
            watch=(self.c2, self.c3) + ((d,) if d is not None else ()),
            acts=tuple(m.bn.act if m is not None else "none" for m in mods))


Block = Union[Type[BasicBlock], Type[Bottleneck]]


class ResNet(nn.Module):

    def __init__(
        self,
        block: Block,
        layers: Sequence[int],
        num_classes: int = 1000,
        in_ch: int = 3,
        small_input: bool = False,
        zero_init_residual: bool = False,
    ) -> None:
        super().__init__()
        self.block = block
        if small_input:
            self.stem = ConvBNAct(in_ch, 64, 3, 1, 1)
            self.pool = nn.Identity()
        else:
            self.stem = ConvBNAct(in_ch, 64, 7, 2, 3)
            self.pool = nn.MaxPool2d(3, 2, 1)
        ch = 64
        stages: List[nn.Module] = []
        for i, n in enumerate(layers):
            width = 64 * 2**i
            blocks = []
            for j in range(n):
                stride = 2 if (j == 0 and i > 0) else 1
                blocks.append(block(ch, width, stride))
                ch = width * block.expansion
            stages.append(nn.Sequential(*blocks))
        self.layer1, self.layer2, self.layer3, self.layer4 = stages
        self.avgpool = nn.AdaptiveAvgPool2d(1)
        self.fc = Linear(ch, num_classes)
        self.reset_parameters(zero_init_residual)

    def reset_parameters(self, zero_init_residual: bool = False) -> None:
        for m in self.modules():
            if isinstance(m, nn.Conv2d):
                nn.init.kaiming_normal_(m.weight, mode="fan_out", nonlinearity="relu")
            elif isinstance(m, BatchNormAct2d):
                nn.init.ones_(m.weight)
                nn.init.zeros_(m.bias)
        if zero_init_residual:
            for m in self.modules():
                if isinstance(m, Bottleneck):
                    nn.init.zeros_(m.c3.bn.weight)
                elif isinstance(m, BasicBlock):
                    nn.init.zeros_(m.c2.bn.weight)

    def features(self, x: Tensor) -> Tensor:
        if isinstance(self.pool, nn.MaxPool2d):
            p = self.pool
            x = self.stem(x, pool=(p.kernel_size, p.stride, p.padding))
        else:
            x = self.pool(self.stem(x))
        link = None
        for stage in (self.layer1, self.layer2, self.layer3, self.layer4):
            for blk in stage:
                if isinstance(blk, Bottleneck):
                    x, link = blk.forward_linked(x, link)
                else:
                    x, link = blk(x), None
        return x

    def forward(self, x: Tensor) -> Tensor:
        x = self.features(x)
        return self.fc(global_avgpool_flatten(x, self.avgpool))


def global_avgpool_flatten(x: Tensor, avgpool: nn.Module) -> Tensor:
    if x.is_cuda and x.is_contiguous(memory_format=torch.channels_last):
        return _GlobalAvgPoolNHWC.apply(x)
    return torch.flatten(avgpool(x), 1)


class _GlobalAvgPoolNHWC(torch.autograd.Function):

    @staticmethod
    def forward(ctx, x):
        ctx.shape = x.shape
        if x.shape[1] % 8 == 0:
            return native().global_avgpool(x)
        return x.mean((2, 3))

    @staticmethod
    def backward(ctx, dy):
        N, C, H, W = ctx.shape
        if C % 8 == 0:
            return native().global_avgpool_backward(dy.contiguous(), H, W)
        g = (dy * (1.0 / (H * W))).view(N, 1, 1, C).expand(N, H, W, C).contiguous()
        return g.permute(0, 3, 1, 2)

# ... 20 lines not shown
```

### torchbooster_amd/ops/conv.py

```python
from __future__ import annotations

import math
import os
from typing import Callable, Dict, Optional, Tuple

from torchbooster_amd.ops import conv_route as RT
from torchbooster_amd.ops import convgemm as CG
from torchbooster_amd.ops import streams

import torch
from torch.autograd.function import once_differentiable
import torch.nn.functional as F
from torch import Tensor

from torchbooster_amd.ops._ext import native, slot_alias, slot_in_use, take_slot, use_native
from torchbooster_amd.ops.conv_route import (_FORCE, _ROUTE_NAMES, _route, autotune_table,
                                             load_routes, save_routes)
from torchbooster_amd.ops.flipcache import _FLIP_CACHE, _FlipCache, _flipped, transposed_linear_weight

__all__ = ["conv2d_any", "conv_any_supported", "PadConv2d", "conv2d", "conv2d_bn_stats", "conv_stem", "stem_supported", "native_supported", "conv2d_forward", "conv2d_wgrad", "autotune_table",
           "Conv2d", "ConvTranspose2d", "conv_transpose2d", "conv_transpose_supported"]

_DIAG_SKIP_WGRAD = os.environ.get("TBAMD_DIAG_SKIP_WGRAD", "0") == "1"
_DISABLE_T = os.environ.get("TBAMD_NATIVE_CONVT", "1") == "0"
# ... 118 lines not shown
    return _route("fwd", key, cands)


def _add_residual(dx: Optional[Tensor], addend: Optional[Tensor], amask: Optional[Tensor],
                  inplace: bool = False) -> Optional[Tensor]:
    if addend is None:
        return dx
    if amask is not None:
        from torchbooster_amd.ops.norm import unpack_mask

        addend = addend * unpack_mask(amask, addend)
    if dx is None:
        return addend
    return dx.add_(addend) if inplace else dx + addend


def _dgrad(dy: Tensor, x: Tensor, w: Tensor, stride: int, pad: int, addend: Optional[Tensor],
           amask: Optional[Tensor] = None, bn_in=None, wparam: Optional[Tensor] = None) -> Tensor:
    R = w.shape[2]
    if addend is not None:
        addend = addend.contiguous(memory_format=torch.channels_last)
    use_bnb = bn_in is not None and bn_in.ready()

    def mio():
        return _add_residual(_miopen_bwd(dy, x, w, stride, pad, 0), addend, amask, inplace=True)

    if stride in (2, 3) and amask is None and native().conv_dgrad_s2_supported(R, w.shape[3], stride):
        bnb_ok = use_bnb and addend is None

        def nat_s2():
            wt = _flipped(w, wparam)
            if bnb_ok:
                b = bn_in
                dx, part = native().conv2d_dgrad_s2(dy, wt, R, w.shape[3], pad, x.shape[2], x.shape[3], b.mode, b.xb,
                                                    b.scale, b.shift, b.mean, b.bits, stride=stride)
                b.part, b.dx_ptr = part, dx.data_ptr()
                return dx
            dx = native().conv2d_dgrad_s2(dy, wt, R, w.shape[3], pad, x.shape[2], x.shape[3], stride=stride)[0]
            return _add_residual(dx, addend, None, inplace=True)

        pen = 2 * x.numel() * x.element_size() / _STATS_PASS_BW * 1e3 if bnb_ok else 0.0
        key = (tuple(x.shape), tuple(w.shape), stride, pad, addend is not None, False, bnb_ok)
        cands = [("native", nat_s2, 0.0), ("miopen", mio, pen)]
        return _route("dgrad", key, cands)
    if not (stride == 1 and pad <= R - 1):
        def gen():
            dx = native().conv_any_dgrad(dy, w, x.shape[2], x.shape[3], stride, pad, 1, False, _dgrad_weight(w, wparam))
            return _add_residual(dx, addend, amask, inplace=True)

        key = ("generic", tuple(x.shape), tuple(w.shape), stride, pad, addend is not None, amask is not None)
        return _route("dgrad", key, [("native", gen, 0.0), ("miopen", mio, 0.0)])

    def nat(big=-1):
        wt = _flipped(w, wparam)
        if use_bnb:
            b = bn_in
            dx, part = native().conv2d_fwd(dy, wt, None, 1, R - 1 - pad, False, False, addend, amask, b.mode, b.xb,
                                           b.scale, b.shift, b.mean, b.bits, big=big)
            b.part, b.dx_ptr = part, dx.data_ptr()
            return dx
        return native().conv2d_fwd(dy, wt, None, 1, R - 1 - pad, False, False, addend, amask, big=big)[0]

    pen = 2 * x.numel() * x.element_size() / _STATS_PASS_BW * 1e3 if use_bnb else 0.0
    key = (tuple(x.shape), tuple(w.shape), stride, pad, addend is not None, amask is not None, use_bnb)
    cands = [("native", nat, 0.0), ("miopen", mio, pen)]
    cands += _big_cands(x.shape[1], w.shape[0], lambda code: lambda: nat(big=code))
    return _route("dgrad", key, cands)


def _wgrad(dy: Tensor, x: Tensor, w: Tensor, stride: int, pad: int, slot: Optional[Tensor] = None) -> Tensor:
    R = w.shape[2]

    def nat():
        if slot is not None:
            native().conv2d_wgrad(dy, x, R, R, stride, pad, slot)
            return slot_alias(slot)
        return native().conv2d_wgrad(dy, x, R, R, stride, pad)

    def mio():
        return _miopen_bwd(dy, x, w, stride, pad, 1)

    cands = [("native", nat, 0.0), ("miopen", mio, 0.0)]
    K, C = w.shape[0], w.shape[1]
    if (R == 1 and w.shape[3] == 1 and stride == 1 and pad == 0 and K % 8 == 0 and C % 8 == 0
            and dy.is_contiguous(memory_format=torch.channels_last)
            and x.is_contiguous(memory_format=torch.channels_last)):
        def gemm():
            from torchbooster_amd.ops.gemm import mm_tn

            d2 = dy.permute(0, 2, 3, 1).reshape(-1, K)
            x2 = x.permute(0, 2, 3, 1).reshape(-1, C)
            if slot is not None:
                mm_tn(d2, x2, out=slot.permute(0, 2, 3, 1).reshape(K, C))
                return slot_alias(slot)
            return mm_tn(d2, x2).view(K, 1, 1, C).permute(0, 3, 1, 2)

        cands.insert(1, ("gemm", gemm, 0.0))
    key = (tuple(x.shape), tuple(w.shape), stride, pad)
    return _route("wgrad", key, cands)


def _gxf_conv_ok(x: Tensor, w: Tensor, stride: int, pad: int) -> bool:
    return (w.shape[2] == 1 and w.shape[3] == 1 and stride == 1 and pad == 0 and x.dtype == torch.bfloat16
            and w.dtype == torch.bfloat16 and x.dim() == 4 and w.shape[0] % 64 == 0 and w.shape[1] % 64 == 0
            and not f32_exact())


def _dgrad_gxf(gx, w: Tensor, wparam: Optional[Tensor], addend: Optional[Tensor], amask: Optional[Tensor], bn_in,
               want_dz: bool):
    g, xb, bits, scale, shift, coef, mode = gx.take()
    wt = _flipped(w, wparam)
    if addend is not None:
        addend = addend.contiguous(memory_format=torch.channels_last)
    b = bn_in
    dx, part, dz = native().conv2d_dgrad_gxf(
        g, wt, addend, amask, b.mode if b is not None else 0, b.xb if b is not None else None,
        b.scale if b is not None else None, b.shift if b is not None else None, b.mean if b is not None else None,
        b.bits if b is not None else None, mode, xb, bits, scale, shift, coef, want_dz)
    if b is not None:
        b.part, b.dx_ptr = part, dx.data_ptr()
    return dx, (dz if want_dz else None)


def _cl_slot(wparam: Tensor, w: Tensor) -> Optional[Tensor]:
    slot = take_slot(wparam)
    if slot is not None and (slot.dtype != w.dtype or not slot.is_contiguous(memory_format=torch.channels_last)):
        return None
    return slot


def _wgrad_side(wparam: Tensor, w: Tensor, run: Callable[[Tensor, Optional[Tensor]], Tensor], reads,
                after: Optional[Tensor]) -> Tensor:
    dy = reads[0]
    slot = _cl_slot(wparam, w)
    if slot is not None and _DIAG_SKIP_WGRAD:
        return slot_alias(slot)
    if slot is not None and streams.usable(dy):
        side = streams.fork(dy.device, after)
        with torch.cuda.stream(side):
            dw = run(dy, slot)
            if dw.data_ptr() != slot.data_ptr():
                slot.copy_(dw)
                dw.record_stream(side)
                dw = slot_alias(slot)
        for t in reads:
            t.record_stream(side)
        return dw
    dw = run(dy, slot)
    if slot is None and slot_in_use(wparam) and streams.pending(dy.device):
        torch.cuda.current_stream(dy.device).wait_stream(streams.side_stream(dy.device))
    return dw


def _deferred_apply(ctx, dy: Tensor, x: Tensor, w: Tensor, stride: int, pad: int, ok: bool,
                    addend: Optional[Tensor], amask: Optional[Tensor], want_dw: bool,
                    wgrad: Callable[[Tensor, Optional[Tensor]], Tensor], reads: tuple):
    gx, ctx.gx = ctx.gx, None
    if gx is None:
        return dy
    if not gx.ready(dy):
        return gx.materialize() if gx.mode else dy
    b = ctx.bn_in if (ctx.bn_in is not None and ctx.bn_in.ready()) else None
    add = 0 if addend is None else (2 if amask is not None else 1)
    if not (ctx.needs_input_grad[0] and ok and _gxf_conv_ok(x, w, stride, pad)
            and native().conv_dgrad_gxf_supported(gx.mode, add, b.mode if b is not None else 0)):
        return gx.materialize()
    dx, dz = _dgrad_gxf(gx, w, ctx.wparam, addend, amask, b, want_dz=want_dw)
    dw = _wgrad_side(ctx.wparam, w, wgrad, (dz,) + reads, None) if want_dw else None
    return dx, dw


def _recompute_grads(ctx, has_bias: bool, dy: Tensor, conv: Callable) -> list:
    needs = (ctx.needs_input_grad[0], ctx.needs_input_grad[1], has_bias and ctx.needs_input_grad[2])
    operands = (*ctx.saved_tensors[:2], ctx.bias_ref if has_bias else None)
    ins = [t for t, need in zip(operands, needs) if need]
    out = [None, None, None]
    if ins:
        y = conv(*operands)
        got = list(torch.autograd.grad(y, ins, dy.to(y.dtype), create_graph=True, allow_unused=True))
        for i, need in enumerate(needs):
            if need:
                out[i] = got.pop(0)
    return out


class _ConvFn(torch.autograd.Function):
    @staticmethod
    def forward(ctx, x, w, bias, stride, pad, want_stats, passthrough, link=None, bn_in=None, relu=False, gx=None):
        assert not (relu and (want_stats or passthrough)), "fused ReLU excludes stats / passthrough"
        y, stats = _fwd(x, w, bias, stride, pad, want_stats, relu)
        ctx.set_materialize_grads(False)
        ctx.relu = relu
        if relu:
            ctx.save_for_backward(x, w, y)
        else:
            ctx.save_for_backward(x, w)
        ctx.cfg = (stride, pad, bias is not None)
        ctx.wparam = w
        ctx.bias_ref = bias
        ctx.link = link
        ctx.bn_in = bn_in
        ctx.gx = gx
        if stats is not None:
            ctx.mark_non_differentiable(stats)
        if passthrough:
            return y, stats, x.view_as(x)
        return y, stats

    @staticmethod
    def backward(ctx, dy, dstats, dpass=None):
        if ctx.relu and dy is not None:
            dy = dy * (ctx.saved_tensors[2] > 0).to(dy.dtype)
        if torch.is_grad_enabled():
            return _ConvFn._backward_differentiable(ctx, dy, dpass)
        with torch.no_grad():
            return _ConvFn._backward_native(ctx, dy, dpass)

    @staticmethod
    def _backward_differentiable(ctx, dy, dpass):
        stride, pad, has_bias = ctx.cfg
        if ctx.link is not None:
            dpass = _add_residual(dpass, *ctx.link.take())
        ctx.gx = None
        grads = [None, None, None]
        if dy is not None:
            grads = _recompute_grads(ctx, has_bias, dy, lambda x, w, b: F.conv2d(x, w, b, stride, pad))
        grads[0] = _add_residual(grads[0], dpass, None)
        return (*grads, None, None, None, None, None, None, None, None)

    @staticmethod
    def _backward_native(ctx, dy, dpass):
        x, w = ctx.saved_tensors[:2]
        stride, pad, has_bias = ctx.cfg
        amask = None
        if ctx.link is not None:
            ldy, lmask = ctx.link.take()
            if ldy is not None and dpass is not None:
                dpass = _add_residual(dpass, ldy, lmask)
            elif ldy is not None:
                dpass, amask = ldy, lmask
        if dy is None:
            return _add_residual(None, dpass, amask), None, None, None, None, None, None, None, None, None, None

        def wgrad(g, slot):
            return _wgrad(g, x, w, stride, pad, slot)

        dy = _deferred_apply(ctx, dy, x, w, stride, pad, not has_bias and not ctx.relu, dpass, amask,
                             ctx.needs_input_grad[1], wgrad, (x,))
        if isinstance(dy, tuple):
            return (*dy, None, None, None, None, None, None, None, None, None)
        dy_in = dy
        dy = dy.contiguous(memory_format=torch.channels_last)
        dx = dw = db = None
        if ctx.needs_input_grad[1]:
            dw = _wgrad_side(ctx.wparam, w, wgrad, (dy, x), dy if dy is dy_in else None)
        if ctx.needs_input_grad[0]:
            dx = _dgrad(dy, x, w, stride, pad, dpass, amask, ctx.bn_in, ctx.wparam)
        if has_bias and ctx.needs_input_grad[2]:
            db = _bias_grad(dy, w.dtype)
        return dx, dw, db, None, None, None, None, None, None, None, None


class _ConvXfFn(torch.autograd.Function):

    @staticmethod
    def forward(ctx, a_ph, y, scale, shift, w, stride, pad, bn_in=None, gx=None):
        out, stats = native().conv2d_fwd_xf(y, w, scale, shift, stride, pad, True)
        ctx.set_materialize_grads(False)
        ctx.save_for_backward(y, scale, shift, w)
        ctx.cfg = (stride, pad)
        ctx.wparam = w
        ctx.bn_in = bn_in
        ctx.gx = gx
        ctx.mark_non_differentiable(stats)
        return out, stats

    @staticmethod
    @once_differentiable
    def backward(ctx, dy, dstats):
        if dy is None:
            return (None,) * 9
        y, scale, shift, w = ctx.saved_tensors
        stride, pad = ctx.cfg
        R = w.shape[2]

        def wgrad(g, slot):
            if slot is not None:
                native().conv2d_wgrad_xf(g, y, scale, shift, R, R, stride, pad, slot)
                return slot_alias(slot)
            return native().conv2d_wgrad_xf(g, y, scale, shift, R, R, stride, pad)

        dy = _deferred_apply(ctx, dy, y, w, stride, pad, True, None, None, ctx.needs_input_grad[4], wgrad,
                             (y, scale, shift))
        if isinstance(dy, tuple):
            return dy[0], None, None, None, dy[1], None, None, None, None
        dy_in = dy
        dy = dy.contiguous(memory_format=torch.channels_last)
        da = dw = None
        if ctx.needs_input_grad[4]:
            dw = _wgrad_side(ctx.wparam, w, wgrad, (dy, y, scale, shift), dy if dy is dy_in else None)
        if ctx.needs_input_grad[0]:
            da = _dgrad(dy, y, w, stride, pad, None, None, ctx.bn_in, ctx.wparam)
        return da, None, None, None, dw, None, None, None, None


def xf_supported(y: Tensor, w: Tensor, stride, padding) -> bool:
    return (y.is_cuda and y.dim() == 4 and y.dtype == torch.bfloat16 and w.dtype == torch.bfloat16
            and y.shape[1] % 64 == 0 and y.shape[1] <= 512 and w.shape[0] % 64 == 0 and w.shape[1] == y.shape[1]
            and w.shape[2] == w.shape[3] and _pair(stride) >= 1 and _pair(padding) >= 0 and not RT._DISABLE
            and use_native(y))


def conv2d_xf_bn_stats(a_ph: Tensor, y: Tensor, scale: Tensor, shift: Tensor, w: Tensor, stride: int, padding: int,
                       bn_in=None, gx=None):
    w = w.contiguous(memory_format=torch.channels_last)
    return _ConvXfFn.apply(a_ph, y.contiguous(memory_format=torch.channels_last), scale, shift, w, _pair(stride),
                           _pair(padding), bn_in, gx)


def conv2d(x: Tensor, w: Tensor, bias: Optional[Tensor] = None, stride=1, padding=0, dilation=1,
           groups=1, relu: bool = False) -> Tensor:
    if use_native(x) and native_supported(x, w, stride, padding, dilation, groups):
        x = x.contiguous(memory_format=torch.channels_last)
        w = w.contiguous(memory_format=torch.channels_last)
        return _ConvFn.apply(x, w, bias, _pair(stride), _pair(padding), False, False, None, None, relu)[0]
    y = F.conv2d(x, w, bias, stride, padding, dilation, groups)
    return F.relu(y) if relu else y


def stem_supported(x: Tensor, w: Tensor, stride, padding, dilation=1, groups=1) -> bool:
    return (x.is_cuda and x.dim() == 4 and x.shape[1] == 3 and x.dtype == torch.bfloat16
            and w.dtype == torch.bfloat16 and tuple(w.shape[1:]) == (3, 7, 7) and w.shape[0] % 64 == 0
            and _pair(stride) == 2 and _pair(padding) == 3 and _pair(dilation) == 1 and groups == 1
            and not RT._DISABLE and use_native(x))


def _pack_stem_w(w: Tensor) -> Tensor:
    K = w.shape[0]
    wp = w.new_zeros(K, 8, 8, 4)
    wp[:, :7, :7, :3] = w.permute(0, 2, 3, 1)
    return wp.reshape(K, 256)


class _StemConvFn(torch.autograd.Function):

    @staticmethod
    def forward(ctx, x, w, want_stats):
        H, W = x.shape[2], x.shape[3]
        keep = {}

        def nat():
            xp = native().conv2d_stem_pad(x)
            keep["xp"] = xp
            y, st = native().conv2d_stem_fwd(xp, _pack_stem_w(w), H, W, want_stats)
            return y, (st if want_stats else None)

        def mio():
            return F.conv2d(x, w, None, 2, 3).contiguous(memory_format=torch.channels_last), None

        pen = 0.0
        if want_stats:
            p, q = _out_hw(H, W, 7, 7, 2, 3)
            pen = x.shape[0] * p * q * w.shape[0] * 2 / _STATS_PASS_BW * 1e3
        y, stats = _route("fwd", ("stem", tuple(x.shape), tuple(w.shape), want_stats),
                          [("native", nat, 0.0), ("miopen", mio, pen)])
        ctx.set_materialize_grads(False)
        ctx.save_for_backward(x, w)
        ctx.xp = keep.get("xp")
        if stats is not None:
            ctx.mark_non_differentiable(stats)
        return y, stats

    @staticmethod
    @once_differentiable
    def backward(ctx, dy, dstats):
        x, w = ctx.saved_tensors
        dx = dw = None
        if dy is None:
            return None, None, None
        if ctx.needs_input_grad[0]:
            dx = _miopen_bwd(dy, x, w, 2, 3, 0)
        if ctx.needs_input_grad[1]:
            K, H, W = w.shape[0], x.shape[2], x.shape[3]
            cl = w.is_contiguous(memory_format=torch.channels_last)

            def nat():
                xp = ctx.xp if ctx.xp is not None else native().conv2d_stem_pad(x)
                g = native().conv2d_stem_wgrad(dy, xp, H, W).view(K, 8, 8, 4)[:, :7, :7, :3].permute(0, 3, 1, 2)
                return g.contiguous(memory_format=torch.channels_last if cl else torch.contiguous_format)

            def mio():
                return _miopen_bwd(dy, x, w, 2, 3, 1)

            dw = _route("wgrad", ("stem", tuple(x.shape), tuple(w.shape)), [("native", nat, 0.0), ("miopen", mio, 0.0)])
        ctx.xp = None
        return dx, dw, None


def conv_stem(x: Tensor, w: Tensor, want_stats: bool = True):
    x = x.contiguous(memory_format=torch.channels_last)
    return _StemConvFn.apply(x, w, want_stats)


def conv2d_bn_stats(x: Tensor, w: Tensor, stride: int, padding: int, passthrough: bool = False, link=None,
                    bn_in=None, gx=None):
    if use_native(x) and native_supported(x, w, stride, padding):
        x = x.contiguous(memory_format=torch.channels_last)
        w = w.contiguous(memory_format=torch.channels_last)
        return _ConvFn.apply(x, w, None, _pair(stride), _pair(padding), True, passthrough, link, bn_in, False, gx)
    y = F.conv2d(x, w, None, stride, padding)
    return (y, None, x) if passthrough else (y, None)


def conv_any_supported(x: Tensor, w: Tensor, stride, padding, dilation=1, groups=1) -> bool:
    if RT._DISABLE or not x.is_cuda or x.dim() != 4 or x.dtype not in (torch.bfloat16, torch.float32):
        return False
    if w.dtype != x.dtype or groups != 1 or _pair(dilation) != 1 or w.shape[2] != w.shape[3]:
        return False
    return _pair(stride) >= 1 and _pair(padding) >= 0 and use_native(x)


def _virtual(x: Tensor, pad: int, up: int, reflect: bool) -> Tensor:
    if up > 1:
        x = F.interpolate(x, scale_factor=up, mode="nearest")
    if pad:
        x = F.pad(x, (pad,) * 4, mode="reflect" if reflect else "constant")
    return x


def _bias_grad(dy: Tensor, dtype: torch.dtype) -> Tensor:
    C = dy.shape[1]
    rows = dy.permute(0, 2, 3, 1)
    if dy.is_cuda and rows.is_contiguous() and dy.dtype in (torch.bfloat16, torch.float32) and not RT._DISABLE:
        G = 8 // math.gcd(C, 8)
        M = rows.numel() // C
        if M % G == 0 and M > 0:
            s = native().colsum(rows.reshape(M // G, G * C), None)
            return (s.view(G, C).float().sum(0) if G > 1 else s).to(dtype)
    return dy.float().sum(dim=(0, 2, 3)).to(dtype)


def _dgrad_weight(w: Tensor, owner: Optional[Tensor]) -> Optional[Tensor]:
    if w.dtype != torch.bfloat16 or not w.is_contiguous(memory_format=torch.channels_last):
        return None
    return _flipped(w, owner)

# ... 444 lines not shown
```

### torchbooster_amd/ops/norm.py

```python
from __future__ import annotations

import os
import weakref
from typing import Optional

import torch
from torch.autograd.function import once_differentiable
import torch.nn.functional as F
from torch import Tensor, nn

from torchbooster_amd.ops import streams
from torchbooster_amd.ops._ext import DTYPE_CODE, slot_alias, take_slot, native, use_native

ACT_CODES = {"none": 0, "identity": 0, None: 0, "relu": 1, "gelu": 2, "silu": 3, "leaky_relu": 4}


def act_ref(z: Tensor, act: str, slope: float = 0.01) -> Tensor:
    if act in ("none", "identity", None):
        return z
    if act == "relu":
        return F.relu(z)
    if act == "gelu":
        return F.gelu(z)
    if act == "silu":
        return F.silu(z)
    if act == "leaky_relu":
        return F.leaky_relu(z, slope)
    raise ValueError(f"unknown activation {act}")


def _to_rows(x: Tensor):
    if x.dim() == 2:
        return x.contiguous(), lambda r: r
    N, C = x.shape[0], x.shape[1]
    if x.dim() == 4:
        xc = x.contiguous(memory_format=torch.channels_last)
        H, W = x.shape[2], x.shape[3]
        rows = xc.permute(0, 2, 3, 1).reshape(N * H * W, C)
        return rows, lambda r: r.view(N, H, W, C).permute(0, 3, 1, 2)
    spatial = x.shape[2:]
    perm = [0] + list(range(2, x.dim())) + [1]
    rows = x.permute(*perm).contiguous().reshape(-1, C)
    inv = [0, x.dim() - 1] + list(range(1, x.dim() - 1))
    return rows, lambda r: r.view(N, *spatial, C).permute(*inv)


class ResidualGradLink:

    __slots__ = ("dy", "mask", "carrier", "ver", "ds_x", "ds_mean", "ds_part")

    def __init__(self, carrier: bool = False) -> None:
        self.dy: Optional[Tensor] = None
        self.mask: Optional[Tensor] = None
        self.carrier = carrier
        self.ver = None
        self.ds_x = self.ds_mean = self.ds_part = None

    def put(self, dy: Tensor, mask: Tensor) -> None:
        self.dy, self.mask, self.ver = dy, mask, dy._version

    def take(self):
        out = (self.dy, self.mask)
        self.dy = self.mask = self.ver = None
        return out

    def take_carried(self, g: Tensor):
        dy, mask, ver, part = self.dy, self.mask, self.ver, self.ds_part
        self.dy = self.mask = self.ver = self.ds_part = self.ds_x = self.ds_mean = None
        if dy is None or mask is None or g.data_ptr() != dy.data_ptr() or g._version != ver or g.shape != dy.shape:
            raise RuntimeError("ResidualGradLink(carrier): the downsample branch received a gradient other than "
                               "the block output's dy (tensor hook or second consumer); build the block without "
                               "the carrier link for this use")
        return mask, part


class BnBwdLink:

    __slots__ = ("xb", "mean", "scale", "shift", "bits", "mode", "part", "dx_ptr")

    def __init__(self) -> None:
        self.mode = 0
        self.xb = self.mean = self.scale = self.shift = self.bits = self.part = None
        self.dx_ptr = None

    def ready(self) -> bool:
        return self.mode != 0 and self.xb is not None

    def take(self, dy: Tensor):
        part, ptr = self.part, self.dx_ptr
        self.part = self.dx_ptr = None
        if part is None or ptr != dy.data_ptr():
            return None
        return part


class BnGradXf:

    __slots__ = ("g", "xb", "bits", "scale", "shift", "coef", "mode", "ph", "restore", "__weakref__")

    def __init__(self) -> None:
        self.g = self.xb = self.bits = self.scale = self.shift = self.coef = self.ph = self.restore = None
        self.mode = 0

    def ready(self, dy: Optional[Tensor]) -> bool:
        return (self.mode != 0 and dy is not None and self.ph is not None and dy.data_ptr() == self.ph.data_ptr()
                and dy.shape == self.ph.shape and dy.stride() == self.ph.stride())

    def take(self):
        out = (self.g, self.xb, self.bits, self.scale, self.shift, self.coef, self.mode)
        self.g = self.xb = self.bits = self.scale = self.shift = self.coef = self.ph = self.restore = None
        self.mode = 0
        return out

    def materialize(self) -> Tensor:
        restore = self.restore
        g, xb, bits, scale, shift, coef, mode = self.take()
        dx = native().bn_backward_apply_coef(_to_rows(g)[0], _to_rows(xb)[0], coef, scale, shift, 1, 0.0,
                                             bits if mode == 2 else None)
        return restore(dx)


_GXF = os.environ.get("TBAMD_BN_GXF", "0") == "1"


def gxf_enabled() -> bool:
    return _GXF


class LazyAct:

    __slots__ = ("y", "scale", "shift", "ph", "__weakref__")

    def __init__(self) -> None:
        self.y = self.scale = self.shift = self.ph = None

    def ready(self, a: Tensor) -> bool:
        return self.y is not None and a is self.ph


def unpack_mask(mask: Tensor, shape_like: Tensor) -> Tensor:
    bits = (mask.unsqueeze(-1) >> torch.arange(8, device=mask.device, dtype=torch.uint8)) & 1
    rows, restore = _to_rows(shape_like)
    return restore(bits.reshape(rows.shape).bool())


class _BNActFn(torch.autograd.Function):
    @staticmethod
    def forward(ctx, x, weight, bias, running_mean, running_var, residual, training, momentum, eps, act,
                slope, stats=None, nbt=None, link=None, bn_out=None, lazy=None, gx=None):
        C = native()
        rows, restore = _to_rows(x)
        ctx.gx = gx if (gx is not None and training and x.dim() == 4) else None
        if (lazy is not None and training and stats is not None and residual is None and ACT_CODES[act] == 0
                and bn_out is None and x.dim() == 4 and rows.shape[1] % 8 == 0):
            mean, invstd, scale, shift = C.bn_stats(rows, stats, weight, bias, running_mean, running_var, True,
                                                    momentum, eps, nbt)
            ctx.save_for_backward(rows, None, None, weight, mean, invstd, scale, shift, None)
            ctx.link = None
            ctx.carried = link if link is not None and link.carrier else None
            if ctx.carried is not None:
                link.ds_x, link.ds_mean = rows, mean
            ctx.bn_out = None
            ctx.cfg = (training, 0, slope, False, x.dim(), x.shape)
            ctx.restore = restore
            ctx.w_dtype = weight.dtype if weight is not None else None
            ctx.params = (weight, bias)
            ctx.orig = (x, None, eps)
            lazy.y, lazy.scale, lazy.shift = x, scale.contiguous(), shift.contiguous()
            lazy.ph = x.new_empty(1).as_strided(tuple(x.shape), (0,) * x.dim())
            lazy.ph._tb_lazy_affine = weakref.ref(lazy)
            return lazy.ph
        if (lazy is not None and training and stats is not None and residual is None and ACT_CODES[act] == 1
                and bn_out is not None and x.dim() == 4 and rows.shape[1] % 8 == 0):
            mean, invstd, scale, shift = C.bn_stats(rows, stats, weight, bias, running_mean, running_var, True,
                                                    momentum, eps, nbt)
            ctx.save_for_backward(rows, None, None, weight, mean, invstd, scale, shift, None)
            ctx.link = None
            ctx.carried = None
            bn_out.mode, bn_out.xb, bn_out.mean, bn_out.scale, bn_out.shift = 1, rows, mean, scale, shift
            bn_out.bits = None
            ctx.bn_out = bn_out
            ctx.cfg = (training, 1, slope, False, x.dim(), x.shape)
            ctx.restore = restore
            ctx.w_dtype = weight.dtype if weight is not None else None
            ctx.params = (weight, bias)
            ctx.orig = (x, None, eps)
            lazy.y, lazy.scale, lazy.shift = x, scale.contiguous(), shift.contiguous()
            lazy.ph = x.new_empty(1).as_strided(tuple(x.shape), (0,) * x.dim())
            return lazy.ph
        code = ACT_CODES[act]
        if link is not None and link.carrier and residual is not None and link.ds_x is None:
            link = None
        want_mask = ((link is not None or (bn_out is not None and training)) and residual is not None and code == 1
                     and rows.shape[1] % 8 == 0)
        res_rows = res_aff = None
        if residual is not None:
            lz = getattr(residual, "_tb_lazy_affine", None)
            lz = lz() if lz is not None else None
            if lz is not None and lz.ready(residual):
                lrows, _ = _to_rows(lz.y)
                if stats is not None and training and want_mask and lrows.dtype == x.dtype:
                    res_rows, res_aff = lrows, (lz.scale, lz.shift)
                else:
                    coeff = torch.stack([lz.scale, lz.scale, lz.scale, lz.shift]).contiguous()
                    res_rows = C.bn_apply_coeff(lrows, coeff, None, 0, 0.0, False)[0].to(x.dtype)
            else:
                res_rows, _ = _to_rows(residual.to(x.dtype))
        if stats is not None and training:
            y, mean, invstd, scale, shift, mask = C.bn_forward_from_stats(
                rows, stats, weight, bias, running_mean, running_var, momentum, eps, res_rows, code, slope, nbt,
                want_mask, *(res_aff if res_aff is not None else (None, None)))
        else:
            y, mean, invstd, scale, shift, mask = C.bn_forward(rows, weight, bias, running_mean, running_var,
                                                               training, momentum, eps, res_rows, code, slope,
                                                               nbt if training else None, want_mask)
        keep_res = res_rows if (residual is not None and code not in (0, 1)) else None
        ctx.save_for_backward(rows, y, keep_res, weight, mean, invstd, scale, shift, mask)
        ctx.link = link if mask is not None else None
        ctx.carried = (link if link is not None and link.carrier and residual is None and code == 0 and training
                       and rows.shape[1] % 8 == 0 and x.dim() == 4 else None)
        if ctx.carried is not None:
            link.ds_x, link.ds_mean = rows, mean
        ctx.bn_out = None
        if bn_out is not None and training and rows.shape[1] % 8 == 0 and x.dim() == 4:
            mode = 0
            if code == 1 and residual is None:
                mode = 1
            elif code == 1 and mask is not None and residual is not None:
                mode = 2
            elif code == 0 and residual is None:
                mode = 3
            if mode:
                bn_out.mode, bn_out.xb, bn_out.mean, bn_out.scale, bn_out.shift = mode, rows, mean, scale, shift
                bn_out.bits = mask if mode == 2 else None
                ctx.bn_out = bn_out
        ctx.cfg = (training, code, slope, residual is not None, x.dim(), x.shape)
        ctx.restore = restore
        ctx.w_dtype = weight.dtype if weight is not None else None
        ctx.params = (weight, bias)
        ctx.orig = (x, residual, eps)
        out = restore(y)
        if not (code == 1 and residual is not None) and out._base is not None:
            out = out.new_empty(0).set_(y.untyped_storage(), out.storage_offset(), out.size(), out.stride())
        return out

    @staticmethod
    def backward(ctx, dy):
        if torch.is_grad_enabled():
            return _BNActFn._backward_differentiable(ctx, dy)
        with torch.no_grad():
            return _BNActFn._backward_native(ctx, dy)

    @staticmethod
    def _backward_differentiable(ctx, dy):
        rows, y, res_rows, weight, mean, invstd, scale, shift, mask = ctx.saved_tensors
        training, code, slope, has_res, _, _ = ctx.cfg
        x, residual, eps = ctx.orig
        wp, bp = ctx.params
        if ctx.link is not None:
            ctx.link = None
        if ctx.carried is not None:
            raise RuntimeError("ResidualGradLink(carrier) under create_graph: build the model without it")
        if ctx.bn_out is not None:
            ctx.bn_out.take(dy)
        shp = [1, -1] + [1] * (x.dim() - 2)
        xf = x.float()
        if training:
            dims = [0] + list(range(2, x.dim()))
            mu = xf.mean(dim=dims, keepdim=True)
            var = xf.var(dim=dims, unbiased=False, keepdim=True)
            xh = (xf - mu) * torch.rsqrt(var + eps)
        else:
            xh = (xf - mean.view(shp)) * invstd.view(shp)
        z = xh * (wp.float().view(shp) if wp is not None else 1.0) + (bp.float().view(shp) if bp is not None else 0.0)
        if residual is not None:
            z = z + residual.float()
        out = act_ref(z, {v: k for k, v in ACT_CODES.items() if isinstance(k, str)}[code], slope).to(x.dtype)
        want = [(x, ctx.needs_input_grad[0]), (wp, wp is not None and ctx.needs_input_grad[1]),
                (bp, bp is not None and ctx.needs_input_grad[2]), (residual, has_res and ctx.needs_input_grad[5])]
        ins = [t for t, need in want if need]
        grads = [None] * 17
        if ins:
            got = list(torch.autograd.grad(out, ins, dy.to(out.dtype), create_graph=True, allow_unused=True))
            for i, (t, need) in zip((0, 1, 2, 5), want):
                if need:
                    grads[i] = got.pop(0)
        return tuple(grads)

    @staticmethod
    def _backward_native(ctx, dy):
        C = native()
        rows, y, res_rows, weight, mean, invstd, scale, shift, mask = ctx.saved_tensors
        training, code, slope, has_res, _, _ = ctx.cfg
        if dy.dim() == 4:
            dy = dy.contiguous(memory_format=torch.channels_last)
        dy_rows, _ = _to_rows(dy)
        wp, bp = ctx.params
        f32 = ctx.w_dtype == torch.float32
        link = ctx.link
        part = ctx.bn_out.take(dy) if ctx.bn_out is not None else None
        gs = take_slot(wp) if f32 and ctx.needs_input_grad[1] else None
        bs = take_slot(bp) if f32 and ctx.needs_input_grad[2] else None
        ev = streams.arm(dy)
        if part is not None and _DIAG_SKIP_BN_BWD and (not has_res or _DIAG_SKIP_BN_BWD == "all"):
            dx = torch.empty_like(rows)
            dg = torch.zeros_like(mean) if weight is not None else None
            db = torch.zeros_like(mean) if weight is not None else None
            dx = ctx.restore(dx)
            dres_out = None
            if link is not None:
                link.put(dy, mask)
                dres_out = dy if link.carrier else None
            elif has_res:
                dres_out = dx
            dw = dg.to(ctx.w_dtype) if weight is not None and ctx.needs_input_grad[1] else None
            dbias = db.to(ctx.w_dtype) if weight is not None and ctx.needs_input_grad[2] else None
            return dx, dw, dbias, None, None, dres_out, None, None, None, None, None, None, None, None, None, None, None
        gx, ctx.gx = ctx.gx, None
        if part is not None and gx is not None and code == 1 and rows.shape[1] % 64 == 0:
            gmode = 0
            if not has_res and mask is None:
                gmode = 1
            elif has_res and mask is not None and link is not None and not link.carrier:
                gmode = 2
            if gmode:
                coef, dg, db = C.bn_backward_coef(part, weight, mean, invstd, rows.shape[0], training, gs, bs)
                gx.g, gx.xb, gx.bits = dy, ctx.restore(rows), (mask if gmode == 2 else None)
                gx.scale, gx.shift, gx.coef, gx.mode, gx.restore = scale, shift, coef, gmode, ctx.restore
                gx.ph = rows.new_empty(1).view(1, 1, 1, 1).expand(ctx.cfg[5])
                streams.tag(gx.ph, ev)
                if link is not None:
                    link.put(dy, mask)
                dw = dbias = None
                if weight is not None and ctx.needs_input_grad[1]:
                    dw = slot_alias(gs) if gs is not None else dg.to(ctx.w_dtype)
                if weight is not None and ctx.needs_input_grad[2]:
                    dbias = slot_alias(bs) if bs is not None else db.to(ctx.w_dtype)
                return (gx.ph, dw, dbias, None, None, None, None, None, None, None, None, None, None, None, None, None,
                        None)
        if part is not None:
            own_dres = link is None and has_res
            dsx = (link.ds_x if _DS_PARTIALS and link is not None and link.carrier and link.ds_x is not None
                   and link.ds_x.shape == rows.shape and link.ds_x.dtype == rows.dtype else None)
            dx, dg, db, dres, dsp = C.bn_backward_from_partials(
                dy_rows, rows, part, weight, mean, invstd, scale, shift, training, code, slope, gs, bs,
                mask if (link is not None or own_dres) else None, own_dres,
                dsx, link.ds_mean if dsx is not None else None)
            if dsx is not None:
                link.ds_part = dsp
            if not own_dres:
                dres = None
        else:
            if y is None and code == 0:
                y = rows
            elif y is None:
                y, _ = C.bn_apply_coeff(rows, torch.stack([mean, invstd, scale, shift]).contiguous(), None, code,
                                        slope, False)
            dsp = None
            if ctx.carried is not None:
                maskin, dsp = ctx.carried.take_carried(dy)
            else:
                maskin = mask if link is not None else None
            if dsp is not None:
                dx, dg, db, dres, _ = C.bn_backward_from_partials(dy_rows, rows, dsp, weight, mean, invstd, scale,
                                                                  shift, training, code, slope, gs, bs, maskin,
                                                                  False)
            else:
                dx, dg, db, dres = C.bn_backward(dy_rows, y, rows, res_rows, weight, mean, invstd, scale, shift,
                                                 training, code, slope, has_res, gs, bs, maskin)
        dx = ctx.restore(dx)
        streams.tag(dx, ev)
        if link is not None:
            link.put(dy, mask)
            dres_out = dy if link.carrier else None
        else:
            dres_out = ctx.restore(dres) if has_res else None
        dw = dbias = None
        if weight is not None and ctx.needs_input_grad[1]:
            dw = slot_alias(gs) if gs is not None else dg.to(ctx.w_dtype)
        if weight is not None and ctx.needs_input_grad[2]:
            dbias = slot_alias(bs) if bs is not None else db.to(ctx.w_dtype)
        return dx, dw, dbias, None, None, dres_out, None, None, None, None, None, None, None, None, None, None, None


_DIAG_SKIP_BN_BWD = os.environ.get("TBAMD_DIAG_SKIP_BN_BWD", "")

_DS_PARTIALS = os.environ.get("TBAMD_DS_PARTIALS", "1") == "1"

_POOL_FUSED_BWD = os.environ.get("TBAMD_POOL_FUSED_BWD", "1") == "1"


class _BNActPoolFn(torch.autograd.Function):

    @staticmethod
    def forward(ctx, x, weight, bias, running_mean, running_var, training, momentum, eps, act, slope, stats, nbt,
                k, s, p):
        C = native()
        rows, _ = _to_rows(x)
        code = ACT_CODES[act]
        mean, invstd, scale, shift = C.bn_stats(rows, stats if training else None, weight, bias, running_mean,
                                                running_var, training, momentum, eps, nbt if training else None)
        y, idx = C.bn_act_maxpool(x, scale, shift, code, slope, k, s, p)
        ctx.save_for_backward(rows, idx, weight, mean, invstd, scale, shift)
        ctx.cfg = (training, code, slope, k, s, p, x.shape[2], x.shape[3])
        ctx.w_dtype = weight.dtype if weight is not None else None
        ctx.params = (weight, bias)
        return y

    @staticmethod
    @once_differentiable
    def backward(ctx, dy):
        C = native()
        rows, idx, weight, mean, invstd, scale, shift = ctx.saved_tensors
        training, code, slope, k, s, p, H, W = ctx.cfg
        wp, bp = ctx.params
        f32 = ctx.w_dtype == torch.float32
        gs = take_slot(wp) if f32 and ctx.needs_input_grad[1] else None
        bs = take_slot(bp) if f32 and ctx.needs_input_grad[2] else None
        if _POOL_FUSED_BWD and C.bn_backward_pool_ok(H, W, rows.shape[1], k, s, p):
            N = dy.shape[0]
            dx, dg, db = C.bn_backward_pool(dy, idx, rows, N, H, W, k, s, p, weight, mean, invstd, scale, shift,
                                            training, code, slope, gs, bs)
            Cc = rows.shape[1]

            def restore(r):
                return r.view(N, H, W, Cc).permute(0, 3, 1, 2)
        else:
            dz = C.maxpool_backward(dy, idx, H, W, k, s, p)
            dz_rows, restore = _to_rows(dz)
            dx, dg, db, _ = C.bn_backward(dz_rows, rows, rows, None, weight, mean, invstd, scale, shift, training,
                                          code, slope, False, gs, bs)
        dw = dbias = None
        if weight is not None and ctx.needs_input_grad[1]:
            dw = slot_alias(gs) if gs is not None else dg.to(ctx.w_dtype)
        if weight is not None and ctx.needs_input_grad[2]:
            dbias = slot_alias(bs) if bs is not None else db.to(ctx.w_dtype)
        return (restore(dx), dw, dbias) + (None,) * 12


def batch_norm_act(
    x: Tensor,
    weight: Optional[Tensor],
    bias: Optional[Tensor],
    running_mean: Optional[Tensor],
    running_var: Optional[Tensor],
    training: bool,
    momentum: float = 0.1,
    eps: float = 1e-5,
    residual: Optional[Tensor] = None,
    act: str = "relu",
    slope: float = 0.01,
    stats: Optional[Tensor] = None,
    num_batches_tracked: Optional[Tensor] = None,
    link: Optional[ResidualGradLink] = None,
    bn_out: Optional[BnBwdLink] = None,
    lazy: Optional[LazyAct] = None,
    gx: Optional[BnGradXf] = None,
) -> Tensor:
    if use_native(x):
        return _BNActFn.apply(x, weight, bias, running_mean, running_var, residual, training, momentum, eps,
                              act, slope, stats, num_batches_tracked, link, bn_out, lazy, gx)
    if num_batches_tracked is not None and training:
        num_batches_tracked.add_(1)
    if running_mean is not None and running_mean.dtype != x.dtype and x.dtype != torch.float32:
        z = F.batch_norm(x.float(), running_mean, running_var, None if weight is None else weight.float(),
                         None if bias is None else bias.float(), training, momentum, eps).to(x.dtype)
    else:
        z = F.batch_norm(x, running_mean, running_var, weight, bias, training, momentum, eps)
    if residual is not None:
        z = z + residual
    return act_ref(z, act, slope)


class BatchNormAct2d(nn.BatchNorm2d):
# ... 300 lines not shown
```

Baseline: 13550 images/s.

## Fold BatchNorm backward input-term into 1x1 conv dgrad and wgrad via precomputed matrix

Adds a fold path for the bottleneck's third 1x1 conv followed by BN+residual. The BN backward's x-dependent term is folded algebraically: dgrad gets an extra reduction over K using a precomputed C×C matrix (W^T diag(c1) W) applied to the conv input, and wgrad gets a fused kernel. The aim is to avoid materializing the BN backward dx tensor and the separate pass over it. The cost is extra MMA work (a longer K reduction), a small per-step fold-matrix kernel, and a bf16 rounding of the folded matrix. It is enabled by default through TBAMD_BN_FOLD=1, for C≤128.

Result: no change. 13750 images/s, median of 6 (+1.4%).

```diff
diff --git a/csrc/bind_conv.cpp b/csrc/bind_conv.cpp
--- a/csrc/bind_conv.cpp
+++ b/csrc/bind_conv.cpp
@@ -243,6 +243,114 @@
   return tbamd::conv_dgrad_gxf_supported((int)gxf, (int)add, (int)bnb_mode);
 }
 
+void check_xf_coeffs(const Tensor& scale, const Tensor& shift, int C, const char* op);
+Tensor dw_slot_or_new(const optional<Tensor>& out, const ConvGeom& g, const Tensor& x, const char* op);
+
+struct FoldOps {
+  Tensor g, a;
+  int N, C, K, H, W;
+  int64_t NPQ;
+  const float *asc = nullptr, *ash = nullptr;
+};
+
+FoldOps fold_operands(const Tensor& g_, const Tensor& bits, const Tensor& coef, const Tensor& a_,
+                      const optional<Tensor>& a_scale, const optional<Tensor>& a_shift, const char* op) {
+  TORCH_CHECK(g_.scalar_type() == at::kBFloat16 && a_.scalar_type() == at::kBFloat16, op, ": bf16 only");
+  TORCH_CHECK(g_.dim() == 4 && a_.dim() == 4 && a_.size(0) == g_.size(0) && a_.size(2) == g_.size(2) &&
+                  a_.size(3) == g_.size(3), op, ": g [N, K, H, W], a [N, C, H, W]");
+  FoldOps f;
+  f.g = nhwc(g_), f.a = nhwc(a_);
+  f.N = (int)g_.size(0), f.K = (int)g_.size(1), f.H = (int)g_.size(2), f.W = (int)g_.size(3), f.C = (int)a_.size(1);
+  f.NPQ = (int64_t)f.N * f.H * f.W;
+  TORCH_CHECK(f.C % 64 == 0 && f.K % 128 == 0 && f.NPQ < (1ll << 31), op, ": needs C % 64 == 0 and K % 128 == 0");
+  TORCH_CHECK(coef.scalar_type() == at::kFloat && coef.is_contiguous() && coef.numel() == 3 * f.K, op,
+              ": coef [3, K] f32");
+  TORCH_CHECK(bits.scalar_type() == at::kByte && bits.is_contiguous() && bits.numel() == f.NPQ * (f.K / 8), op,
+              ": bits [N*H*W, K/8] bytes");
+  TORCH_CHECK(given(a_scale) == given(a_shift), op, ": a_scale and a_shift go together");
+  if (given(a_scale)) {
+    check_xf_coeffs(*a_scale, *a_shift, f.C, op);
+    f.asc = a_scale->data_ptr<float>();
+    f.ash = a_shift->data_ptr<float>();
+  }
+  return f;
+}
+
+Tensor conv_bn_fold_m(const Tensor& w_, const Tensor& coef) {
+  const at::DeviceGuard guard = on_device_of(w_, "w");
+  TORCH_CHECK(w_.scalar_type() == at::kBFloat16 && w_.dim() == 4 && w_.size(2) == 1 && w_.size(3) == 1,
+              "conv_bn_fold_m: w [K, C, 1, 1] bf16");
+  Tensor w = nhwc(w_);
+  const int K = (int)w.size(0), C = (int)w.size(1);
+  TORCH_CHECK(C % 16 == 0 && coef.scalar_type() == at::kFloat && coef.is_contiguous() && coef.numel() == 3 * K,
+              "conv_bn_fold_m: C % 16 == 0, coef [3, K] f32");
+  Tensor m = at::empty({C, C}, w.options());
+  tbamd::conv_bn_fold_m(w.data_ptr(), coef.data_ptr<float>(), K, C, m.data_ptr(), cur_stream());
+  return m;
+}
+
+std::vector<Tensor> conv2d_dgrad_fold(const Tensor& g_, const Tensor& wt_, const Tensor& wm, const Tensor& bits,
+                                      const Tensor& coef, const Tensor& a_, const optional<Tensor>& a_scale,
+                                      const optional<Tensor>& a_shift, const optional<Tensor>& addend,
+                                      const optional<Tensor>& addend_mask, int64_t bnb_mode,
+                                      const optional<Tensor>& bnb_x, const optional<Tensor>& bnb_scale,
+                                      const optional<Tensor>& bnb_shift, const optional<Tensor>& bnb_mean) {
+  const at::DeviceGuard guard = on_device_of(g_, "g");
+  TORCH_CHECK(wt_.dim() == 4 && wt_.size(0) == a_.size(1) && wt_.size(1) == g_.size(1) && wt_.size(2) == 1 &&
+                  wt_.size(3) == 1, "conv2d_dgrad_fold: wt [C, K, 1, 1]");
+  const FoldOps f = fold_operands(g_, bits, coef, a_, a_scale, a_shift, "conv2d_dgrad_fold");
+  Tensor wt = nhwc(wt_);
+  TORCH_CHECK(wt.scalar_type() == at::kBFloat16 && wm.scalar_type() == at::kBFloat16 && wm.is_contiguous() &&
+                  wm.numel() == (int64_t)f.C * f.C, "conv2d_dgrad_fold: wm [C, C] bf16");
+  Tensor y = at::empty({f.N, f.C, f.H, f.W}, f.g.options().memory_format(kNHWC));
+  Tensor add;
+  const uint8_t* amask = nullptr;
+  if (given(addend)) {
+    TORCH_CHECK(addend->sizes() == y.sizes() && addend->scalar_type() == at::kBFloat16, "conv2d_dgrad_fold: addend");
+    add = nhwc(*addend);
+    if (given(addend_mask)) {
+      TORCH_CHECK(addend_mask->scalar_type() == at::kByte && addend_mask->numel() == f.NPQ * (f.C / 8),
+                  "conv2d_dgrad_fold: addend_mask [N*H*W, C/8] bytes");
+      amask = addend_mask->data_ptr<uint8_t>();
+    }
+  }
+  const int add_code = add.defined() ? (amask ? 2 : 1) : 0;
+  TORCH_CHECK(tbamd::conv_dgrad_fold_combo_supported(add_code, (int)bnb_mode),
+              "conv2d_dgrad_fold: unsupported (addend, bnb_mode) combination");
+  Tensor part;
+  Bnb bnb;
+  if (bnb_mode != 0) {
+    bnb = bnb_operands(bnb_mode, bnb_x, bnb_scale, bnb_shift, bnb_mean, optional<Tensor>(), f.NPQ, f.C,
+                       "conv2d_dgrad_fold");
+    part = at::empty({tbamd::conv_fold_bnb_rows(f.NPQ, f.C), 2, f.C}, f.g.options().dtype(at::kFloat));
+  }
+  if (f.NPQ > 0)
+    tbamd::conv_dgrad_fold(f.g.data_ptr(), wt.data_ptr(), wm.data_ptr(), y.data_ptr(), ptr_or_null(add), amask, f.N,
+                           f.H, f.W, f.K, f.C, cur_stream(), (int)bnb_mode, bnb.x, bnb.scale, bnb.shift, bnb.mean,
+                           f32_or_null(part), bits.data_ptr<uint8_t>(), coef.data_ptr<float>(), f.a.data_ptr(), f.asc,
+                           f.ash);
+  return {y, part};
+}
+
+std::vector<Tensor> conv2d_wgrad_fold(const Tensor& g_, const Tensor& bits, const Tensor& coef, const Tensor& a_,
+                                      const optional<Tensor>& a_scale, const optional<Tensor>& a_shift,
+                                      const Tensor& w_, const optional<Tensor>& out) {
+  const at::DeviceGuard guard = on_device_of(g_, "g");
+  TORCH_CHECK(w_.scalar_type() == at::kBFloat16 && w_.dim() == 4 && w_.size(0) == g_.size(1) &&
+                  w_.size(1) == a_.size(1) && w_.size(2) == 1 && w_.size(3) == 1, "conv2d_wgrad_fold: w [K, C, 1, 1]");
+  const FoldOps f = fold_operands(g_, bits, coef, a_, a_scale, a_shift, "conv2d_wgrad_fold");
+  Tensor w = nhwc(w_);
+  ConvGeom cg = ConvGeom::of(f.a, f.g, 1, 1);
+  Tensor dw = dw_slot_or_new(out, cg, f.a, "conv2d_wgrad_fold");
+  if (f.NPQ == 0) return {dw.zero_(), Tensor()};
+  const int64_t rows = tbamd::conv_wgrad_fold_rows(f.C, f.K);
+  Tensor work = f32_work(tbamd::conv_wgrad_fold_workspace(f.N, f.H, f.W, f.C, f.K), f.a);
+  tbamd::conv_wgrad_fold(f.g.data_ptr(), bits.data_ptr<uint8_t>(), coef.data_ptr<float>(), f.a.data_ptr(), f.asc,
+                         f.ash, w.data_ptr(), dw.data_ptr(), work.data_ptr<float>(), f.N, f.H, f.W, f.C, f.K,
+                         cur_stream());
+  return {dw, work.slice(0, work.numel() - rows * f.C).view({rows, (int64_t)f.C})};
+}
+
 void check_xf_coeffs(const Tensor& scale, const Tensor& shift, int C, const char* op) {
   TORCH_CHECK(scale.scalar_type() == at::kFloat && shift.scalar_type() == at::kFloat && scale.numel() == C &&
                   shift.numel() == C && scale.is_contiguous() && shift.is_contiguous(),
@@ -543,6 +651,20 @@
         py::arg("bnb_mean"), py::arg("bnb_bits"), py::arg("gxf"), py::arg("gx_x"), py::arg("gx_bits"),
         py::arg("gx_scale"), py::arg("gx_shift"), py::arg("gx_coef"), py::arg("want_dz"));
   m.def("conv_dgrad_gxf_supported", &conv_dgrad_gxf_supported);
+  m.def("conv_bwd_fold_supported", [](int64_t NPQ, int64_t C, int64_t K, bool xf) {
+    return tbamd::conv_bwd_fold_supported(NPQ, (int)C, (int)K, xf);
+  });
+  m.def("conv_dgrad_fold_combo_supported", [](int64_t add, int64_t bnb_mode) {
+    return tbamd::conv_dgrad_fold_combo_supported((int)add, (int)bnb_mode);
+  });
+  m.def("conv_bn_fold_m", &conv_bn_fold_m, py::arg("w"), py::arg("coef"));
+  m.def("conv2d_dgrad_fold", &conv2d_dgrad_fold, py::arg("g"), py::arg("wt"), py::arg("wm"), py::arg("bits"),
+        py::arg("coef"), py::arg("a"), py::arg("a_scale") = py::none(), py::arg("a_shift") = py::none(),
+        py::arg("addend") = py::none(), py::arg("addend_mask") = py::none(), py::arg("bnb_mode") = 0,
+        py::arg("bnb_x") = py::none(), py::arg("bnb_scale") = py::none(), py::arg("bnb_shift") = py::none(),
+        py::arg("bnb_mean") = py::none());
+  m.def("conv2d_wgrad_fold", &conv2d_wgrad_fold, py::arg("g"), py::arg("bits"), py::arg("coef"), py::arg("a"),
+        py::arg("a_scale"), py::arg("a_shift"), py::arg("w"), py::arg("out") = py::none());
   m.def("conv_fwd_xf_supported", &tbamd::conv_fwd_xf_supported);
   m.def("conv2d_fwd_xf", &conv2d_fwd_xf, py::arg("x"), py::arg("w"), py::arg("scale"), py::arg("shift"),
         py::arg("stride"), py::arg("pad"), py::arg("want_stats") = true);
diff --git a/csrc/conv.hip b/csrc/conv.hip
--- a/csrc/conv.hip
+++ b/csrc/conv.hip
@@ -54,6 +54,7 @@
   const float* shift;
   const float* coef;
   uint16_t* out;
+  const uint16_t* wm = nullptr;
 };
 
 struct S2Cls {
@@ -94,6 +95,7 @@
   static_assert(!VIRT || (!S2D && !STEM), "VIRT: plain forward addressing only");
   static_assert(GXF == 0 || (STAGES == 1 && !S2D && !STEM && !VIRT && !STATS),
                 "GXF: single-stage 1x1 dgrad addressing only (host: R = S = 1, stride 1, pad 0)");
+  constexpr bool FOLD = GXF == 3;
   constexpr int BK = kConvBK;
   constexpr int A_PASSES = BM / 32, B_PASSES = BN / 32;
   constexpr int WM = BM / 2, WN = BN / 2;
@@ -135,7 +137,7 @@
 
   const int Kred = g.R * g.S * g.C;
   const int cblocks = g.C / BK;
-  const int KT = STEM ? kStemKT : (S2D ? cls.ntap * cblocks : g.R * g.S * cblocks);
+  const int KT = STEM ? kStemKT : (S2D ? cls.ntap * cblocks : g.R * g.S * cblocks) + (FOLD ? g.K / BK : 0);
   const int lrow = wave * 8 + (lane >> 3);
   const int slot = lane & 7;
 
@@ -158,11 +160,12 @@
   }
   const uint16_t* wsrc0 = w + (int64_t)(m0 + lrow) * Kred + (slot ^ swz(lrow, 0)) * 8;
   const int64_t wpass = (int64_t)32 * Kred;
+  const uint16_t* msrc0 = FOLD ? gxa.wm + (int64_t)(m0 + lrow) * g.K + (slot ^ swz(lrow, 0)) * 8 : nullptr;
 
   const int cbl = STEM ? 1 : cblocks;
   const void* zpage = pin_sgpr(g_conv_zero_page);
-  uint4 gx_v[GXF ? B_PASSES : 1];
-  uint32_t gx_m[GXF == 2 ? B_PASSES : 1];
+  uint4 gx_v[(GXF == 1 || GXF == 2) ? B_PASSES : 1];
+  uint32_t gx_m[GXF >= 2 ? B_PASSES : 1];
   extern __shared__ __attribute__((aligned(16))) float gx_lds[];
   auto issue = [&](int kt, int buf) {
     const int rs = kt / cbl, cb = kt - rs * cbl;
@@ -175,6 +178,25 @@
     }
     uint4* A = lds + buf * STAGE;
     uint4* B = A + BM * BK / 8;
+    if constexpr (FOLD) {
+      if (kt >= cblocks) {
+        const int ko = (kt - cblocks) * BK;
+#pragma unroll
+        for (int i = 0; i < A_PASSES; ++i) {
+          const uint16_t* msrc = msrc0 + (int64_t)i * 32 * g.K + ko;
+          const bool wok = TB_BOUNDS_OK(msrc + 8 <= gxa.wm + (int64_t)g.K * g.K, kBndConvW);
+          glds16(wok ? (const void*)msrc : zpage, A + (32 * i + wave * 8) * 8);
+        }
+#pragma unroll
+        for (int i = 0; i < B_PASSES; ++i) {
+          const int row = lrow + 32 * i;
+          const int64_t off = (n0 + row) * g.K + ko + (slot ^ swz(row, 0)) * 8;
+          const bool ok = pix_n[i] >= 0 && TB_BOUNDS_OK(off + 8 <= NPQ * g.K, kBndConvSrc);
+          glds16(ok ? (const void*)(gxa.xb + off) : zpage, B + (32 * i + wave * 8) * 8);
+        }
+        return;
+      }
+    }
 #pragma unroll
     for (int i = 0; i < A_PASSES; ++i) {
       const uint16_t* wsrc = wsrc0 + i * wpass;
@@ -213,8 +235,8 @@
       const void* src = ok ? (const void*)(x + off) : zpage;
       glds16(src, B + (32 * i + wave * 8) * 8);
       if constexpr (GXF != 0) {
-        gx_v[i] = ok ? *reinterpret_cast<const uint4*>(gxa.xb + off) : make_uint4(0u, 0u, 0u, 0u);
-        if constexpr (GXF == 2) gx_m[i] = ok ? (uint32_t)gxa.bits[off >> 3] : 0u;
+        if constexpr (!FOLD) gx_v[i] = ok ? *reinterpret_cast<const uint4*>(gxa.xb + off) : make_uint4(0u, 0u, 0u, 0u);
+        if constexpr (GXF >= 2) gx_m[i] = ok ? (uint32_t)gxa.bits[off >> 3] : 0u;
       }
     }
     }
@@ -224,6 +246,19 @@
       const int C4 = g.C >> 2;
       float4* d = reinterpret_cast<float4*>(gx_lds);
       const float4* cf = reinterpret_cast<const float4*>(gxa.coef);
+      if constexpr (FOLD) {
+        for (int i = tid; i < 2 * C4; i += kConvThreads) d[i] = cf[i];
+        if (gxa.scale != nullptr) {
+          const int K4 = g.K >> 2;
+          const float4* sc = reinterpret_cast<const float4*>(gxa.scale);
+          const float4* sf = reinterpret_cast<const float4*>(gxa.shift);
+          for (int i = tid; i < K4; i += kConvThreads) {
+            d[2 * C4 + i] = sc[i];
+            d[2 * C4 + K4 + i] = sf[i];
+          }
+        }
+        return;
+      }
       for (int i = tid; i < 3 * C4; i += kConvThreads) d[i] = cf[i];
       if constexpr (GXF == 1) {
         const float4* sc = reinterpret_cast<const float4*>(gxa.scale);
@@ -238,6 +273,26 @@
   auto gxf_apply = [&](int kt) {
     if constexpr (GXF != 0) {
       uint4* B = lds + BM * BK / 8;
+      if constexpr (FOLD) {
+        if (kt >= cblocks) {
+          if (gxa.scale == nullptr) return;
+          const int ca = (kt - cblocks) * BK + (slot ^ swz(lrow, 0)) * 8;
+          const float* sp = gx_lds + 2 * g.C + ca;
+          float s8[8], h8[8];
+#pragma unroll
+          for (int e = 0; e < 8; ++e) {
+            s8[e] = sp[e];
+            h8[e] = sp[g.K + e];
+          }
+#pragma unroll
+          for (int i = 0; i < B_PASSES; ++i) {
+            if (pix_n[i] < 0) continue;
+            uint4* p = B + (32 * i + lrow) * 8 + slot;
+            *p = xf_chunk(*p, s8, h8);
+          }
+          return;
+        }
+      }
       const int c0 = kt * BK + (slot ^ swz(lrow, 0)) * 8;
       float ka[8], k0[8], k1[8], sc[8], sf[8];
       auto ld8 = [&](int row, float (&v)[8]) {
@@ -247,17 +302,17 @@
       };
       ld8(0, ka);
       ld8(1, k0);
-      ld8(2, k1);
+      if constexpr (!FOLD) ld8(2, k1);
       if constexpr (GXF == 1) {
         ld8(3, sc);
         ld8(4, sf);
       }
-      const bool wr = gxa.out != nullptr && tile_m == 0;
+      const bool wr = !FOLD && gxa.out != nullptr && tile_m == 0;
 #pragma unroll
       for (int i = 0; i < B_PASSES; ++i) {
         if (pix_n[i] < 0) continue;
         uint4* p = B + (32 * i + lrow) * 8 + slot;
-        const uint4 gv = *p, xv = gx_v[i];
+        const uint4 gv = *p, xv = FOLD ? make_uint4(0u, 0u, 0u, 0u) : gx_v[FOLD ? 0 : i];
         const uint32_t gw[4] = {gv.x, gv.y, gv.z, gv.w}, xw[4] = {xv.x, xv.y, xv.z, xv.w};
         uint32_t ow[4];
 #pragma unroll
@@ -272,7 +327,8 @@
             if constexpr (GXF == 1) keep = __builtin_fmaf(xf, sc[k], sf[k]) > 0.f;
             else keep = (gx_m[i] >> k) & 1u;
             const float dz = keep ? gf : 0.f;
-            d[h] = ka[k] * dz + k0[k] + k1[k] * xf;
+            if constexpr (FOLD) d[h] = ka[k] * dz + k0[k];
+            else d[h] = ka[k] * dz + k0[k] + k1[k] * xf;
           }
           ow[e] = (uint32_t)f2bf(d[0]) | ((uint32_t)f2bf(d[1]) << 16);
         }
@@ -1222,6 +1278,88 @@
   if (!ok) throw std::runtime_error("conv_dgrad_gxf: unsupported (gxf, addend, bnb_mode) combination");
 }
 
+constexpr int kFoldT = 16, kFoldKS = 256;
+__global__ __launch_bounds__(kFoldT * kFoldT) void conv_bn_fold_m_k(const uint16_t* __restrict__ w,
+                                                                   const float* __restrict__ c1, int K, int C,
+                                                                   uint16_t* __restrict__ m) {
+  __shared__ float sa[kFoldKS][kFoldT + 1], sb[kFoldKS][kFoldT + 1];
+  const int tx = threadIdx.x % kFoldT, ty = threadIdx.x / kFoldT;
+  const int ca = blockIdx.y * kFoldT, cb = blockIdx.x * kFoldT;
+  float acc = 0.f;
+  for (int k0 = 0; k0 < K; k0 += kFoldKS) {
+    for (int r = ty; r < kFoldKS; r += kFoldT) {
+      const int k = k0 + r;
+      const bool ok = k < K;
+      sa[r][tx] = ok ? bf2f(w[(int64_t)k * C + ca + tx]) * c1[k] : 0.f;
+      sb[r][tx] = ok ? bf2f(w[(int64_t)k * C + cb + tx]) : 0.f;
+    }
+    __syncthreads();
+#pragma unroll 16
+    for (int r = 0; r < kFoldKS; ++r) acc = __builtin_fmaf(sa[r][ty], sb[r][tx], acc);
+    __syncthreads();
+  }
+  m[(int64_t)(ca + ty) * C + cb + tx] = f2bf(acc);
+}
+
+void conv_bn_fold_m(const void* w, const float* coef, int K, int C, void* m, hipStream_t st) {
+  conv_bn_fold_m_k<<<dim3(C / kFoldT, C / kFoldT), kFoldT * kFoldT, 0, st>>>((const uint16_t*)w, coef + 2 * (int64_t)K, K,
+                                                                           C, (uint16_t*)m);
+}
+
+bool conv_bwd_fold_supported(int64_t NPQ, int C, int K, bool xf) {
+  (void)xf;
+  return C % 64 == 0 && K % 64 == 0 && C <= 128 && NPQ > 0 && NPQ < (1ll << 31);
+}
+
+static int fold_pix_tile(int C) { return C % 128 == 0 ? 64 : 128; }
+
+int conv_fold_bnb_rows(int64_t NPQ, int C) {
+  const int bn = fold_pix_tile(C);
+  return (int)((NPQ + bn - 1) / bn);
+}
+
+template <int BM, int BN, int ADD, int BNB>
+static void launch_fold(const uint16_t* x, const uint16_t* w, uint16_t* y, const uint16_t* addend,
+                        const uint8_t* amask, const ConvGeom& g, hipStream_t st, const BnBwdEpi& bnb,
+                        const GxfArgs& gxa) {
+  const int64_t NPQ = (int64_t)g.N * g.P * g.Q;
+  const dim3 grid((g.K / BM) * (int)((NPQ + BN - 1) / BN));
+  const size_t coef_bytes = (size_t)(2 * g.C + 2 * g.K) * sizeof(float);
+  conv_fwd_k<BM, BN, false, false, false, 1, ADD, 4, BNB, false, false, false, 3, 3>
+      <<<grid, kConvThreads, coef_bytes, st>>>(x, w, y, nullptr, nullptr, addend, amask, g, bnb, S2Cls{}, gxa);
+}
+
+bool conv_dgrad_fold_combo_supported(int add, int bnb_mode) {
+  return (add == 0 || add == 2) && (bnb_mode == 0 || bnb_mode == 1);
+}
+
+void conv_dgrad_fold(const void* g_, const void* wt, const void* wm, void* y, const void* addend, const uint8_t* amask,
+                     int N, int H, int W, int K, int C, hipStream_t st, int bnb_mode, const void* bnb_x,
+                     const float* bnb_scale, const float* bnb_shift, const float* bnb_mean, float* bnb_part,
+                     const uint8_t* bits, const float* coef, const void* a, const float* a_scale,
+                     const float* a_shift) {
+  const BnBwdEpi bnb{(const uint16_t*)bnb_x, bnb_scale, bnb_shift, bnb_mean, nullptr, bnb_part};
+  const GxfArgs gxa{(const uint16_t*)a, bits, a_scale, a_shift, coef, nullptr, (const uint16_t*)wm};
+  const ConvGeom g{N, H, W, K, C, 1, 1, H, W, 1, 0};
+  const uint16_t* xx = (const uint16_t*)g_;
+  const uint16_t* ww = (const uint16_t*)wt;
+  uint16_t* yy = (uint16_t*)y;
+  const uint16_t* aa = (const uint16_t*)addend;
+  const int add = addend ? (amask ? 2 : 1) : 0;
+  if (!conv_dgrad_fold_combo_supported(add, bnb_mode))
+    throw std::runtime_error("conv_dgrad_fold: unsupported (addend, bnb_mode) combination");
+  auto go = [&](auto bm, auto bn) {
+    constexpr int BM = decltype(bm)::value, BN = decltype(bn)::value;
+    if (add == 0 && bnb_mode == 1) launch_fold<BM, BN, 0, 1>(xx, ww, yy, aa, amask, g, st, bnb, gxa);
+    else if (add == 0) launch_fold<BM, BN, 0, 0>(xx, ww, yy, aa, amask, g, st, bnb, gxa);
+    else if (bnb_mode == 1) launch_fold<BM, BN, 2, 1>(xx, ww, yy, aa, amask, g, st, bnb, gxa);
+    else launch_fold<BM, BN, 2, 0>(xx, ww, yy, aa, amask, g, st, bnb, gxa);
+  };
+  using std::integral_constant;
+  if (fold_pix_tile(C) == 64) go(integral_constant<int, 128>{}, integral_constant<int, 64>{});
+  else go(integral_constant<int, 64>{}, integral_constant<int, 128>{});
+}
+
 void conv_fwd(const void* x, const void* w, void* y, const float* bias, float* stats, const void* addend,
               const uint8_t* amask, bool relu, int N, int H, int W, int C, int K, int R, int S, int P, int Q,
               int stride, int pad, hipStream_t st, int bnb_mode, const void* bnb_x, const float* bnb_scale,
diff --git a/csrc/conv_wgrad.hip b/csrc/conv_wgrad.hip
--- a/csrc/conv_wgrad.hip
+++ b/csrc/conv_wgrad.hip
@@ -74,13 +74,20 @@
 constexpr int kWgThreads = 256;
 constexpr int kWgBK = 64;
 
-template <int BM, int BN, bool FINAL, int OCC = 2, bool STEM = false, bool VIRT = false, bool XF = false>
+struct FoldArgs {
+  const uint8_t* bits;
+  const float* coef;
+};
+
+template <int BM, int BN, bool FINAL, int OCC = 2, bool STEM = false, bool VIRT = false, bool XF = false,
+          bool FOLD = false>
 __global__ __launch_bounds__(kWgThreads, OCC) void conv_wgrad_k(const uint16_t* __restrict__ dy,
                                                               const uint16_t* __restrict__ x,
                                                               float* __restrict__ part,
                                                               uint16_t* __restrict__ dw, WgradGeom g,
-                                                              XfArgs xf = XfArgs{}) {
+                                                              XfArgs xf = XfArgs{}, FoldArgs fo = FoldArgs{}) {
   static_assert(!XF || (!STEM && !VIRT), "XF: plain weight gradient");
+  static_assert(!FOLD || (!STEM && !VIRT && !FINAL), "FOLD: plain 1x1 weight gradient into partials");
   constexpr int BK = kWgBK;
   constexpr int ROWA = BM * 2, ROWB = BN * 2;
   constexpr int CPA = BM / 8, CPB = BN / 8;
@@ -91,7 +98,8 @@
 
   const int tid = threadIdx.x, lane = tid & 63, wave = tid >> 6;
   const int wm = wave >> 1, wn = wave & 1;
-  const int ntm = g.K / BM, ntn = g.ncol / BN, ntiles = ntm * ntn;
+  const int ntk = g.K / BM;
+  const int ntm = ntk + (FOLD ? (g.C + BM - 1) / BM : 0), ntn = g.ncol / BN, ntiles = ntm * ntn;
   const int nwg = ntiles * g.splits;
   int bid = blockIdx.x;
   {
@@ -107,12 +115,24 @@
 
   const uint16_t* asrc[A_PASSES];
   int arow[A_PASSES];
+  const bool gtile = FOLD && tile_m >= ntk;
+  const int astride = gtile ? g.C : g.K;
+  bool acol_ok = true;
+  int achan = 0;
 #pragma unroll
   for (int i = 0; i < A_PASSES; ++i) {
     const int row = i * (kWgThreads / CPA) + wave * (64 / CPA) + lane / CPA;
     const int lc = (lane % CPA) ^ wz<ROWA>(row);
     arow[i] = row;
     asrc[i] = dy + m0 + lc * 8;
+    if constexpr (FOLD) {
+      achan = m0 + lc * 8;
+      if (gtile) {
+        achan -= g.K;
+        acol_ok = achan < g.C;
+        asrc[i] = x + (acol_ok ? achan : 0);
+      }
+    }
   }
   int brow[B_PASSES], bdr[B_PASSES], bds[B_PASSES], bc[B_PASSES];
 #pragma unroll
@@ -144,6 +164,19 @@
       xsh[e] = sh8[e];
     }
   }
+  float fta[FOLD ? 8 : 1], ftb[FOLD ? 8 : 1];
+  uint32_t amask[FOLD ? A_PASSES : 1];
+  uint32_t avalid = 0u;
+  if constexpr (FOLD) {
+    const float* ra = gtile ? xf.scale : fo.coef;
+    const float* rb = gtile ? xf.shift : fo.coef + g.K;
+    const bool have = (!gtile || XF) && acol_ok;
+#pragma unroll
+    for (int e = 0; e < 8; ++e) {
+      fta[e] = have ? ra[achan + e] : 0.f;
+      ftb[e] = have ? rb[achan + e] : 0.f;
+    }
+  }
   auto issue = [&](int kt, int buf) {
     char* A = lds + buf * STAGE;
     char* B = A + BK * ROWA;
@@ -151,8 +184,14 @@
 #pragma unroll
     for (int i = 0; i < A_PASSES; ++i) {
       const int pix = p0 + arow[i];
-      const void* src = pix < pe ? (const void*)(asrc[i] + (int64_t)pix * g.K) : zpage;
+      const bool aok = pix < pe && (!FOLD || acol_ok);
+      const void* src = aok ? (const void*)(asrc[i] + (int64_t)pix * (FOLD ? astride : g.K)) : zpage;
       glds16(src, A + (i * kWgThreads + wave * 64) * 16);
+      if constexpr (FOLD) {
+        if (i == 0) avalid = 0u;
+        avalid |= (uint32_t)aok << i;
+        amask[i] = (aok && !gtile) ? (uint32_t)fo.bits[(int64_t)pix * (g.K >> 3) + (achan >> 3)] : 0u;
+      }
     }
 #pragma unroll
     for (int i = 0; i < B_PASSES; ++i) {
@@ -183,6 +222,45 @@
     }
   };
   auto xform = [&](int buf) {
+    if constexpr (FOLD) {
+      char* A = lds + buf * STAGE;
+      if (!gtile) {
+#pragma unroll
+        for (int i = 0; i < A_PASSES; ++i) {
+          if (!((avalid >> i) & 1u)) continue;
+          uint4* p = reinterpret_cast<uint4*>(A + (i * kWgThreads + wave * 64) * 16) + lane;
+          const uint4 gv = *p;
+          const uint32_t gw[4] = {gv.x, gv.y, gv.z, gv.w};
+          uint32_t ow[4];
+#pragma unroll
+          for (int e = 0; e < 4; ++e) {
+            float d[2];
+#pragma unroll
+            for (int h = 0; h < 2; ++h) {
+              const int k = 2 * e + h;
+              const float gf = bf2f((uint16_t)(gw[e] >> (16 * h)));
+              const float dz = ((amask[i] >> k) & 1u) ? gf : 0.f;
+              d[h] = fta[k] * dz + ftb[k];
+            }
+            ow[e] = (uint32_t)f2bf(d[0]) | ((uint32_t)f2bf(d[1]) << 16);
+          }
+          *p = make_uint4(ow[0], ow[1], ow[2], ow[3]);
+        }
+      } else if constexpr (XF) {
+        float sc8[8], sh8[8];
+#pragma unroll
+        for (int e = 0; e < 8; ++e) {
+          sc8[e] = fta[e];
+          sh8[e] = ftb[e];
+        }
+#pragma unroll
+        for (int i = 0; i < A_PASSES; ++i) {
+          if (!((avalid >> i) & 1u)) continue;
+          uint4* p = reinterpret_cast<uint4*>(A + (i * kWgThreads + wave * 64) * 16) + lane;
+          *p = xf_chunk(*p, sc8, sh8);
+        }
+      }
+    }
     if constexpr (XF) {
       char* B = lds + buf * STAGE + BK * ROWA;
       float sc8[8], sh8[8];
@@ -237,7 +315,7 @@
       for (int j = 0; j < TN; ++j) {
         const int n = n0 + wn * WN + j * 16 + fr;
         if constexpr (FINAL) dw[(int64_t)m * g.ncol + n] = f2bf(acc[i][j][e]);
-        else part[((int64_t)split * g.K + m) * g.ncol + n] = acc[i][j][e];
+        else part[((int64_t)split * (FOLD ? ntm * BM : g.K) + m) * g.ncol + n] = acc[i][j][e];
       }
     }
 }
@@ -456,6 +534,62 @@
   }
 }
 
+__global__ __launch_bounds__(256) void wgrad_fold_finish_k(const float* __restrict__ sums,
+                                                           const uint16_t* __restrict__ w,
+                                                           const float* __restrict__ c1, int K, int C,
+                                                           uint16_t* __restrict__ dw) {
+  const int64_t idx = (int64_t)blockIdx.x * 256 + threadIdx.x;
+  if (idx >= (int64_t)K * C) return;
+  const int k = (int)(idx / C), c = (int)(idx - (int64_t)k * C);
+  const float* G = sums + (int64_t)K * C;
+  const uint16_t* wr = w + (int64_t)k * C;
+  float acc = 0.f;
+#pragma unroll 8
+  for (int j = 0; j < C; ++j) acc = __builtin_fmaf(bf2f(wr[j]), G[(int64_t)j * C + c], acc);
+  dw[idx] = f2bf(sums[idx] + c1[k] * acc);
+}
+
+static int fold_rows(int C, int K) { return K + (C + 127) / 128 * 128; }
+
+int conv_wgrad_fold_rows(int C, int K) { return fold_rows(C, K); }
+
+int64_t conv_wgrad_fold_workspace(int N, int H, int W, int C, int K) {
+  const WgradGeom g = plan_wgrad(N, H, W, C, K, 1, 1, H, W, 1, 0);
+  return ((int64_t)g.splits + 1) * fold_rows(C, K) * C;
+}
+
+void conv_wgrad_fold(const void* gy, const uint8_t* bits, const float* coef, const void* a, const float* a_scale,
+                     const float* a_shift, const void* w, void* dw, float* workspace, int N, int H, int W, int C,
+                     int K, hipStream_t st) {
+  if (K % 128 != 0 || C % 64 != 0) throw std::runtime_error("conv_wgrad_fold: needs K % 128 == 0 and C % 64 == 0");
+  const WgradGeom g = plan_wgrad(N, H, W, C, K, 1, 1, H, W, 1, 0);
+  const XfArgs xf{a_scale, a_shift};
+  const FoldArgs fo{bits, coef};
+  const uint16_t* d = (const uint16_t*)gy;
+  const uint16_t* xx = (const uint16_t*)a;
+  const int Kp = fold_rows(C, K);
+  auto go = [&](auto bn, auto isxf) {
+    constexpr int BN = decltype(bn)::value;
+    constexpr bool XF = decltype(isxf)::value;
+    const int nwg = (Kp / 128) * (g.ncol / BN) * g.splits;
+    conv_wgrad_k<128, BN, false, 2, false, false, XF, true><<<nwg, kWgThreads, 0, st>>>(d, xx, workspace, nullptr, g, xf, fo);
+  };
+  using std::integral_constant;
+  const bool bn128 = C % 128 == 0;
+  if (a_scale) {
+    if (bn128) go(integral_constant<int, 128>{}, std::true_type{});
+    else go(integral_constant<int, 64>{}, std::true_type{});
+  } else {
+    if (bn128) go(integral_constant<int, 128>{}, std::false_type{});
+    else go(integral_constant<int, 64>{}, std::false_type{});
+  }
+  const int64_t total = (int64_t)Kp * C;
+  float* sums = workspace + (int64_t)g.splits * total;
+  wgrad_reduce_k<float><<<cdiv(total, 4 * kRedCols), kRedCols * kRedLanes, 0, st>>>(workspace, g.splits, total, sums);
+  wgrad_fold_finish_k<<<cdiv((int64_t)K * C, 256), 256, 0, st>>>(sums, (const uint16_t*)w, coef + 2 * (int64_t)K, K, C,
+                                                               (uint16_t*)dw);
+}
+
 void conv_wgrad_set_occupancy(int o) { g_wgrad_occ = o; }
 
 int64_t conv_wgrad_split32_workspace(int N, int H, int W, int C, int K, int R, int S, int P, int Q, int stride,
diff --git a/csrc/tbamd.h b/csrc/tbamd.h
--- a/csrc/tbamd.h
+++ b/csrc/tbamd.h
@@ -60,6 +60,20 @@
 void bn_backward_apply_coef(int dt, const void* dy, const void* x, int64_t M, int C, int act, float slope,
                             const float* scale, const float* shift, const float* coef, void* dx,
                             const uint8_t* maskin, hipStream_t st);
+bool conv_bwd_fold_supported(int64_t NPQ, int C, int K, bool xf);
+bool conv_dgrad_fold_combo_supported(int add, int bnb_mode);
+int conv_fold_bnb_rows(int64_t NPQ, int C);
+void conv_bn_fold_m(const void* w, const float* coef, int K, int C, void* m, hipStream_t st);
+void conv_dgrad_fold(const void* g, const void* wt, const void* wm, void* y, const void* addend, const uint8_t* amask,
+                     int N, int H, int W, int K, int C, hipStream_t st, int bnb_mode, const void* bnb_x,
+                     const float* bnb_scale, const float* bnb_shift, const float* bnb_mean, float* bnb_part,
+                     const uint8_t* bits, const float* coef, const void* a, const float* a_scale,
+                     const float* a_shift);
+int64_t conv_wgrad_fold_workspace(int N, int H, int W, int C, int K);
+int conv_wgrad_fold_rows(int C, int K);
+void conv_wgrad_fold(const void* g, const uint8_t* bits, const float* coef, const void* a, const float* a_scale,
+                     const float* a_shift, const void* w, void* dw, float* workspace, int N, int H, int W, int C,
+                     int K, hipStream_t st);
 int bn_bwd_dsp_rows(int64_t M, int C);
 void bn_eval_coeffs(int C, const float* gamma, const float* beta, const float* rm, const float* rv,
                     float eps, float* mean, float* invstd, float* scale, float* shift, hipStream_t st);
diff --git a/torchbooster_amd/models/resnet.py b/torchbooster_amd/models/resnet.py
--- a/torchbooster_amd/models/resnet.py
+++ b/torchbooster_amd/models/resnet.py
@@ -10,7 +10,9 @@
                                        stem_supported)
 from torchbooster_amd.ops import _ext
 from torchbooster_amd.ops._ext import native, use_native
-from torchbooster_amd.ops.norm import BatchNormAct2d, BnBwdLink, BnGradXf, LazyAct, ResidualGradLink, gxf_enabled
+from torchbooster_amd.ops.conv import f32_exact
+from torchbooster_amd.ops.norm import (BatchNormAct2d, BnBwdLink, BnGradXf, LazyAct, ResidualGradLink, fold_enabled,
+                                       gxf_enabled)
 from torchbooster_amd.ops.linear import Linear
 
 __all__ = [
@@ -126,6 +128,13 @@
     return _no_hooks(tuple(m for m in tuple(convs[:3]) + tuple(bns[:3]) if m is not None) + tuple(watch))
 
 
+def _fold_ok(training: bool, convs: Sequence[Optional[nn.Conv2d]], bns: Sequence[Optional[nn.Module]],
+             watch: Sequence[nn.Module]) -> bool:
+    if not (fold_enabled() and training and bns[2].training and torch.is_grad_enabled() and not f32_exact()):
+        return False
+    return _no_hooks(tuple(m for m in tuple(convs[:3]) + tuple(bns[:3]) if m is not None) + tuple(watch))
+
+
 def _gxf_pair_ok(conv: nn.Conv2d, act: str) -> bool:
     return (act == "relu" and conv.bias is None and conv.kernel_size == (1, 1) and conv.stride == (1, 1)
             and conv.padding == (0, 0) and conv.groups == 1 and conv.weight.dtype == torch.bfloat16
@@ -157,6 +166,12 @@
     if native and _gxf_ok(training, convs, bns, watch):
         g1 = BnGradXf() if _gxf_pair_ok(convs[0], acts[0]) else None
         g3 = BnGradXf() if not has_down and link is not None and _gxf_pair_ok(convs[2], "relu") else None
+    if (g3 is None and native and not has_down and link is not None and _gxf_pair_ok(convs[2], "relu")
+            and _fold_ok(training, convs, bns, watch)):
+        c3 = convs[2]
+        npq = x.shape[0] * x.shape[2] * x.shape[3]
+        if _ext.native().conv_bwd_fold_supported(npq, c3.in_channels, c3.out_channels, z2 is not None):
+            g3 = BnGradXf(fold=True)
     h, xp = run(0, x, passthrough=True, link=link if not has_down else None,
                 bn_in=bn_in if native else None, bn_out=l1, gx=g1)
     if has_down:
diff --git a/torchbooster_amd/ops/conv.py b/torchbooster_amd/ops/conv.py
--- a/torchbooster_amd/ops/conv.py
+++ b/torchbooster_amd/ops/conv.py
@@ -294,16 +294,51 @@
     return dw
 
 
+def _fold_grads(ctx, gx, x: Tensor, w: Tensor, addend: Optional[Tensor], amask: Optional[Tensor], bn_in,
+                want_dw: bool, xf: Optional[Tuple[Tensor, Tensor]]):
+    nat = native()
+    g, _, bits, _, _, coef, _ = gx.take()
+    a_sc, a_sh = xf if xf is not None else (None, None)
+    wm = nat.conv_bn_fold_m(w, coef)
+    dw = None
+    if want_dw:
+        def run(gg, slot):
+            out = nat.conv2d_wgrad_fold(gg, bits, coef, x, a_sc, a_sh, w, slot)[0]
+            return slot_alias(slot) if slot is not None else out
+
+        dw = _wgrad_side(ctx.wparam, w, run, (g, bits, coef, x) + (tuple(xf) if xf is not None else ()), None)
+    if addend is not None:
+        addend = addend.contiguous(memory_format=torch.channels_last)
+    b = bn_in
+    dx, part = nat.conv2d_dgrad_fold(
+        g, _flipped(w, ctx.wparam), wm, bits, coef, x, a_sc, a_sh, addend, amask, b.mode if b is not None else 0,
+        b.xb if b is not None else None, b.scale if b is not None else None, b.shift if b is not None else None,
+        b.mean if b is not None else None)
+    if b is not None:
+        b.part, b.dx_ptr = part, dx.data_ptr()
+    return dx, dw
+
+
 def _deferred_apply(ctx, dy: Tensor, x: Tensor, w: Tensor, stride: int, pad: int, ok: bool,
                     addend: Optional[Tensor], amask: Optional[Tensor], want_dw: bool,
-                    wgrad: Callable[[Tensor, Optional[Tensor]], Tensor], reads: tuple):
+                    wgrad: Callable[[Tensor, Optional[Tensor]], Tensor], reads: tuple,
+                    xf: Optional[Tuple[Tensor, Tensor]] = None):
     gx, ctx.gx = ctx.gx, None
     if gx is None:
         return dy
     if not gx.ready(dy):
+        if gx.mode and gx.fold:
+            raise RuntimeError("a BatchNorm backward folded into this conv's gradients (TBAMD_BN_FOLD) received a "
+                               "gradient that is not its placeholder; run with TBAMD_BN_FOLD=0")
         return gx.materialize() if gx.mode else dy
     b = ctx.bn_in if (ctx.bn_in is not None and ctx.bn_in.ready()) else None
     add = 0 if addend is None else (2 if amask is not None else 1)
+    if gx.fold:
+        if not (ctx.needs_input_grad[0] and ok and gx.mode == 2 and _gxf_conv_ok(x, w, stride, pad)
+                and w.shape[0] % 128 == 0
+                and native().conv_dgrad_fold_combo_supported(add, b.mode if b is not None else 0)):
+            return gx.materialize()
+        return _fold_grads(ctx, gx, x, w, addend, amask, b, want_dw, xf)
     if not (ctx.needs_input_grad[0] and ok and _gxf_conv_ok(x, w, stride, pad)
             and native().conv_dgrad_gxf_supported(gx.mode, add, b.mode if b is not None else 0)):
         return gx.materialize()
@@ -433,7 +468,7 @@
             return native().conv2d_wgrad_xf(g, y, scale, shift, R, R, stride, pad)
 
         dy = _deferred_apply(ctx, dy, y, w, stride, pad, True, None, None, ctx.needs_input_grad[4], wgrad,
-                             (y, scale, shift))
+                             (y, scale, shift), xf=(scale, shift))
         if isinstance(dy, tuple):
             return dy[0], None, None, None, dy[1], None, None, None, None
         dy_in = dy
diff --git a/torchbooster_amd/ops/norm.py b/torchbooster_amd/ops/norm.py
--- a/torchbooster_amd/ops/norm.py
+++ b/torchbooster_amd/ops/norm.py
@@ -96,11 +96,12 @@
 
 class BnGradXf:
 
-    __slots__ = ("g", "xb", "bits", "scale", "shift", "coef", "mode", "ph", "restore", "__weakref__")
-
-    def __init__(self) -> None:
+    __slots__ = ("g", "xb", "bits", "scale", "shift", "coef", "mode", "ph", "restore", "fold", "__weakref__")
+
+    def __init__(self, fold: bool = False) -> None:
         self.g = self.xb = self.bits = self.scale = self.shift = self.coef = self.ph = self.restore = None
         self.mode = 0
+        self.fold = fold
 
     def ready(self, dy: Optional[Tensor]) -> bool:
         return (self.mode != 0 and dy is not None and self.ph is not None and dy.data_ptr() == self.ph.data_ptr()
@@ -125,6 +126,13 @@
 
 def gxf_enabled() -> bool:
     return _GXF
+
+
+_FOLD = os.environ.get("TBAMD_BN_FOLD", "1") == "1"
+
+
+def fold_enabled() -> bool:
+    return _FOLD
 
 
 class LazyAct:
@@ -319,7 +327,7 @@
         gx, ctx.gx = ctx.gx, None
         if part is not None and gx is not None and code == 1 and rows.shape[1] % 64 == 0:
             gmode = 0
-            if not has_res and mask is None:
+            if not has_res and mask is None and not gx.fold:
                 gmode = 1
             elif has_res and mask is not None and link is not None and not link.carrier:
                 gmode = 2
```
